# AmandineBtto/NeRAF

Measured on AMD Instinct MI355X. Metric: field-samples/sec (rays + RIR STFT bins), higher is better.
Workload: dtype f16; 1 GPU; RAF FurnishedRoom joint training step (BASELINE configs[2]): 4096 rays + 2048 RIR slices x 513 bins per GPU; radiance + grid refresh + ResNet3D + NAcF + STFT loss, backward, GradScaler + fused Adam...; rays_per_gpu=4096, slices_per_gpu=2048, global_rays=4096, global_slices=2048, parallelism=dp1, distinct_resident_batches=16, deterministic=True

## Files before the change

neraf_amd/csrc/field_bwd.hip:

```cpp
#include "field_common.h"

namespace {

constexpr int NFRAG = 24;
constexpr int NFRAG_B = 28;

struct RenderLossArgs {
  const float* density; const float* rgb_s; const float* e_bins; const float* s_bins; const float* gt;
  int R, S; float dist_mult;
  const float* up;
  float* d_rgb_s; float* d_density;
  float* d_density_dist;
  float* sums;
};

__global__ __launch_bounds__(256) void render_loss_kernel(RenderLossArgs a) {
  const int lane = threadIdx.x & 63;
  int ray = blockIdx.x * 4 + (threadIdx.x >> 6);
  const bool active = ray < a.R;
  if (!active) ray = a.R - 1;
  const int S = a.S;
  const bool on = lane < S;
  const float* eb = a.e_bins + (size_t)ray * (S + 1);
  const float* sb = a.s_bins + (size_t)ray * (S + 1);
// ... 214 lines not shown
  __syncthreads();
  const int lane = threadIdx.x & 63, wv = threadIdx.x >> 6;
  const long N = (long)a.R * a.S;
  const long nchunks = (N + 255) / 256;
  float tmass[8] = {0.f, 0.f, 0.f, 0.f, 0.f, 0.f, 0.f, 0.f};
  if (a.d32 && blockIdx.x == 0 && threadIdx.x < 2) a.one2[threadIdx.x] = 1.f;
  for (long chunk = blockIdx.x; chunk < nchunks; chunk += gridDim.x) {
    const long idx = chunk * 256 + threadIdx.x;
    const bool valid = idx < N;
    float enc[16], hpre[16], dh[16];
#pragma unroll
    for (int k = 0; k < 16; ++k) { enc[k] = 0.f; dh[k] = 0.f; hpre[k] = 0.f; }
    float x = 0.f, y = 0.f, z = 0.f, gs = 0.f;
    float xr = 0.f, yr = 0.f, zr = 0.f, tmid = 0.f; int ray_id = -1; bool sel_pt = false;
    float rgx = 0.f, rgy = 0.f, rgz = 0.f;
    if (valid) {
      const int ray = (int)(idx / a.S), s = (int)(idx % a.S);
      const float t = 0.5f * (a.e_bins[(size_t)ray * (a.S + 1) + s] + a.e_bins[(size_t)ray * (a.S + 1) + s + 1]);
      x = fmaf(a.dirs[ray * 3 + 0], t, a.origins[ray * 3 + 0]);
      y = fmaf(a.dirs[ray * 3 + 1], t, a.origins[ray * 3 + 1]);
      z = fmaf(a.dirs[ray * 3 + 2], t, a.origins[ray * 3 + 2]);
      xr = x; yr = y; zr = z; tmid = t; ray_id = ray;
      const bool sel = map_position(x, y, z, 0, nullptr);
      sel_pt = sel;
#pragma unroll
      for (int l = 0; l < 8; ++l)
        if (l < a.g.n_levels) {
          float f0, f1;
          encode_level(a.table, x, y, z, a.g.scale[l], a.g.res[l], a.g.size[l], a.g.offset[l], a.g.hashed[l], f0, f1);
          enc[2 * l] = (float)(half_t)f0; enc[2 * l + 1] = (float)(half_t)f1;
        }
      float out = 0.f;
#pragma unroll
      for (int j = 0; j < 16; ++j) {
        float h = 0.f;
#pragma unroll
        for (int k = 0; k < 16; ++k) h = fmaf(w0[j][k], enc[k], h);
        hpre[j] = h;
        out = fmaf(w1[j], fmaxf(h, 0.f), out);
      }
      gs = sel ? a.d_density[idx] * a.avg_density * __expf(fminf(fmaxf(out, -15.f), 15.f)) : 0.f;
#pragma unroll
      for (int j = 0; j < 16; ++j) dh[j] = hpre[j] > 0.f ? gs * w1[j] : 0.f;
    }
#pragma unroll
    for (int l = 0; l < 8; ++l)
      if (l < a.g.n_levels) {
        float g0 = 0.f, g1 = 0.f;
#pragma unroll
        for (int j = 0; j < 16; ++j) { g0 = fmaf(dh[j], w0[j][2 * l], g0); g1 = fmaf(dh[j], w0[j][2 * l + 1], g1); }
        if (a.d_ray && valid && sel_pt)
          encode_level_dpos(a.table, x, y, z, a.g.scale[l], a.g.res[l], a.g.size[l], a.g.offset[l], a.g.hashed[l], g0, g1, rgx, rgy, rgz);
        if (a.d32) {
          if (valid) { a.d32[(long)l * a.npad + idx] = make_float2(g0, g1); tmass[l] += fmaxf(fabsf(g0), fabsf(g1)); }
        } else {
          scatter_level_seg<64>(a.table_grad, x, y, z, a.g.scale[l], a.g.res[l], a.g.size[l], a.g.offset[l], a.g.hashed[l], g0, g1, lane);
        }
      }
    if (a.d_ray) {
      map_position_jt(xr, yr, zr, rgx, rgy, rgz);
      float g6[6] = {rgx, rgy, rgz, tmid * rgx, tmid * rgy, tmid * rgz};
      const int ray0 = __shfl(ray_id, 0);
      if (a.g6_out) {
        if (valid) {
#pragma unroll
          for (int k = 0; k < 6; ++k) a.g6_out[(size_t)idx * 6 + k] = g6[k];
        }
      } else if (__all(ray_id == ray0 || !valid)) {
#pragma unroll
        for (int k = 0; k < 6; ++k) {
          float v = valid ? g6[k] : 0.f;
#pragma unroll
          for (int o = 32; o > 0; o >>= 1) v += __shfl_xor(v, o);
          if (lane == 0 && v != 0.f && ray0 >= 0) atomicAdd(a.d_ray + (size_t)ray0 * 6 + k, v);
        }
      } else if (valid) {
#pragma unroll
        for (int k = 0; k < 6; ++k) if (g6[k] != 0.f) atomicAdd(a.d_ray + (size_t)ray_id * 6 + k, g6[k]);
      }
    }
#pragma unroll
    for (int k = 0; k < 16; ++k) { s_dh[wv][lane][k] = dh[k]; s_enc[wv][lane][k] = enc[k]; s_hr[wv][lane][k] = gs * fmaxf(hpre[k], 0.f); }
    __builtin_amdgcn_wave_barrier();
    __syncthreads();
    {
      const int j = lane >> 2, k0 = (lane & 3) * 4;
      float s[4] = {0.f, 0.f, 0.f, 0.f};
      for (int p = 0; p < 64; ++p) {
        const float d = s_dh[wv][p][j];
#pragma unroll
        for (int q = 0; q < 4; ++q) s[q] = fmaf(d, s_enc[wv][p][k0 + q], s[q]);
      }
#pragma unroll
      for (int q = 0; q < 4; ++q) acc[wv][j * 16 + k0 + q] += s[q];
      if (lane < 16) {
        float t = 0.f;
        for (int p = 0; p < 64; ++p) t += s_hr[wv][p][lane];
        acc[wv][256 + lane] += t;
      }
    }
    __syncthreads();
  }
  for (int i = threadIdx.x; i < 272; i += 256) {
    const float v = (acc[0][i] + acc[1][i]) + (acc[2][i] + acc[3][i]);
    if (a.w_part) a.w_part[(size_t)blockIdx.x * 272 + i] = v;
    else atomicAdd(a.w_grad + i, v);
  }
  if (a.d32) {
    __syncthreads();
    float* red = &s_dh[0][0][0];
#pragma unroll
    for (int l = 0; l < 8; ++l) {
      float v = tmass[l];
#pragma unroll
      for (int o = 32; o > 0; o >>= 1) v += __shfl_xor(v, o);
      if (lane == 0) red[wv * 8 + l] = v;
    }
    __syncthreads();
    if (threadIdx.x < 16)
      a.t_part[(size_t)blockIdx.x * 16 + threadIdx.x] = threadIdx.x < 8 ? (red[threadIdx.x] + red[8 + threadIdx.x]) + (red[16 + threadIdx.x] + red[24 + threadIdx.x]) : 0.f;
  }
}

__global__ __launch_bounds__(256) void prop_wgrad_fold_kernel(const float* __restrict__ part, int nblocks, float* __restrict__ w_grad,
                                                             float* __restrict__ w0_out, float* __restrict__ w1_out) {
  __shared__ float red[32][9];
  const int o = threadIdx.x & 7, sl = threadIdx.x >> 3;
  const int i = blockIdx.x * 8 + o;
  float t = 0.f, t1 = 0.f;
  if (i < 272) {
    int b = sl;
    for (; b + 32 < nblocks; b += 64) { t += part[(size_t)b * 272 + i]; t1 += part[(size_t)(b + 32) * 272 + i]; }
    for (; b < nblocks; b += 32) t += part[(size_t)b * 272 + i];
  }
  red[sl][o] = t + t1;
  __syncthreads();
  if (threadIdx.x < 8 && i < 272) {
    float s = 0.f;
#pragma unroll
    for (int r = 0; r < 32; ++r) s += red[r][threadIdx.x];
    const int k = blockIdx.x * 8 + threadIdx.x;
    if (w0_out) { if (k < 256) w0_out[k] = s; else w1_out[k - 256] = s; }
    else w_grad[k] += s;
  }
  if (w1_out && blockIdx.x == 0 && threadIdx.x >= 16) w1_out[threadIdx.x] = 0.f;
}

struct FieldBwdArgs {
  GridLayout g;
  const unsigned* table; const half8* wfrag; const half8* wfrag_b; const half_t* emb;
  const float* origins; const float* dirs; const float* e_bins; const int* cam_idx;
  int R, S; int mode; float aabb[6]; float avg_density; int avg_row;
  const float* d_rgb; const float* d_density;
  const float* scale;
  float* emb_grad;
  half_t* dump; long npad;
  unsigned* d_enc;
  float* t_part;
  int emb_det;
  float* e_part; int* e_part_row;
  float* pos;
  float* d_ray;
  float* g6_out;
  const half_t* enc_in;
  const half_t* denc_in;
};

__device__ __forceinline__ void dump_block(half_t* base, long npad, long n, int row0, const f32x4& v, float m) {
#pragma unroll
  for (int r = 0; r < 4; ++r) base[(long)(row0 + r) * npad + n] = (half_t)(v[r] * m);
}

template <bool RAYGRAD, bool SAVED>
__global__ __launch_bounds__(256) void field_backward_kernel(FieldBwdArgs a) {
  __shared__ float l_scale[MAX_LEVELS];
  __shared__ int l_res[MAX_LEVELS];
  __shared__ unsigned l_size[MAX_LEVELS], l_off[MAX_LEVELS];
  __shared__ int l_hash[MAX_LEVELS];
  if (threadIdx.x < MAX_LEVELS) {
    const int l = threadIdx.x;
    l_scale[l] = a.g.scale[l]; l_res[l] = a.g.res[l]; l_size[l] = a.g.size[l]; l_off[l] = a.g.offset[l]; l_hash[l] = a.g.hashed[l];
  }
  __syncthreads();
  __shared__ float t_sum[4][16];
  __shared__ float e_acc[32];
  __shared__ int e_blk_s;
  if (threadIdx.x < 32) e_acc[threadIdx.x] = 0.f;
  if (threadIdx.x == 0) {
    long n0 = (long)blockIdx.x * 64; const long Nn = (long)a.R * a.S;
    if (n0 >= Nn) n0 = Nn - 1;
    e_blk_s = (a.avg_row < 0 && a.cam_idx) ? a.cam_idx[n0 / a.S] : -1;
  }
  __syncthreads();
  const int e_blk = e_blk_s;
  const int lane = threadIdx.x & 63;
  const int p = lane & 15, q = lane >> 4;
  __shared__ half8 wf_s[NFRAG * 64];
  for (int i = threadIdx.x; i < NFRAG * 64; i += 256) wf_s[i] = a.wfrag[i];
  const half8* wfp = wf_s + lane;
#define wf(f) wfp[(f) * 64]
  __shared__ half8 wb_s[NFRAG_B * 64];
  for (int i = threadIdx.x; i < NFRAG_B * 64; i += 256) wb_s[i] = a.wfrag_b[i];
  __syncthreads();
  const half8* wb = wb_s + lane;
  const float gscale = a.scale[0], inv_gscale = a.scale[1];
  float tl[4] = {0.f, 0.f, 0.f, 0.f};
  const f32x4 zero = {0.f, 0.f, 0.f, 0.f};
  const long N = (long)a.R * a.S;
  const long ngroups = a.npad / 16;
  const long gstride = (long)gridDim.x * 4;
  const long MAT = 128 * a.npad;
  for (long grp = (long)blockIdx.x * 4 + (threadIdx.x >> 6); grp < ngroups; grp += gstride) {
    const long ncol = grp * 16 + p;
    long n = ncol;
    const bool valid = n < N;
    if (!valid) n = N - 1;
    const float vm = valid ? 1.f : 0.f;
    const int ray = (int)(n / a.S), s = (int)(n % a.S);
    const float t = 0.5f * (a.e_bins[(size_t)ray * (a.S + 1) + s] + a.e_bins[(size_t)ray * (a.S + 1) + s + 1]);
    const float dx = a.dirs[ray * 3 + 0], dy = a.dirs[ray * 3 + 1], dz = a.dirs[ray * 3 + 2];
    float x = fmaf(dx, t, a.origins[ray * 3 + 0]);
    float y = fmaf(dy, t, a.origins[ray * 3 + 1]);
    float z = fmaf(dz, t, a.origins[ray * 3 + 2]);
    const float xr = x, yr = y, zr = z;
    const bool sel = map_position(x, y, z, a.mode, a.aabb);
    if (a.pos && q == 0) { a.pos[ncol] = x; a.pos[a.npad + ncol] = y; a.pos[2 * a.npad + ncol] = z; }
    half8 xin;
    float dfe[RAYGRAD ? 4 : 1][2][3];
    if (SAVED) {
      xin = *reinterpret_cast<const half8*>(a.enc_in + ((size_t)n * 4 + q) * 8);
      if (RAYGRAD) {
        half8 dh[3];
        const half8* src = reinterpret_cast<const half8*>(a.denc_in + ((size_t)n * 4 + q) * 24);
        dh[0] = src[0]; dh[1] = src[1]; dh[2] = src[2];
        const half_t* dp = reinterpret_cast<const half_t*>(dh);
#pragma unroll
        for (int li = 0; li < 4; ++li)
#pragma unroll
          for (int k = 0; k < 3; ++k) { dfe[RAYGRAD ? li : 0][0][k] = (float)dp[li * 6 + k]; dfe[RAYGRAD ? li : 0][1][k] = (float)dp[li * 6 + 3 + k]; }
      }
    } else {
#pragma unroll
      for (int li = 0; li < 4; ++li) {
        const int l = 4 * q + li;
        float f0, f1;
        if (RAYGRAD) encode_level_grad(a.table, x, y, z, l_scale[l], l_res[l], l_size[l], l_off[l], l_hash[l], f0, f1, dfe[RAYGRAD ? li : 0][0], dfe[RAYGRAD ? li : 0][1]);
        else encode_level(a.table, x, y, z, l_scale[l], l_res[l], l_size[l], l_off[l], l_hash[l], f0, f1);
        xin[2 * li] = (half_t)f0; xin[2 * li + 1] = (half_t)f1;
      }
    }
    f32x4 d1[4];
#pragma unroll
    for (int ob = 0; ob < 4; ++ob) d1[ob] = __builtin_amdgcn_mfma_f32_16x16x32_f16(wf(ob), xin, zero, 0, 0, 0);
    f32x4 d2 = __builtin_amdgcn_mfma_f32_16x16x32_f16(wf(4), pack_relu(d1[0], d1[1], true), zero, 0, 0, 0);
    d2 = __builtin_amdgcn_mfma_f32_16x16x32_f16(wf(5), pack_relu(d1[2], d1[3], true), d2, 0, 0, 0);
    float sh[4];
    sh4_quarter(q, dx, dy, dz, sh);
    half8 h0;
#pragma unroll
    for (int r = 0; r < 4; ++r) { h0[r] = (half_t)d2[r]; h0[4 + r] = (half_t)sh[r]; }
    const float logit = d2[0];
    if (q == 0) h0[0] = (half_t)0.f;
    const int erow = a.avg_row >= 0 ? a.avg_row : a.cam_idx[ray];
    const half8 h1 = *reinterpret_cast<const half8*>(a.emb + (size_t)erow * 32 + 8 * q);
    f32x4 d3[4], d4[4];
#pragma unroll
    for (int ob = 0; ob < 4; ++ob) {
      d3[ob] = __builtin_amdgcn_mfma_f32_16x16x32_f16(wf(6 + ob * 2), h0, zero, 0, 0, 0);
      d3[ob] = __builtin_amdgcn_mfma_f32_16x16x32_f16(wf(7 + ob * 2), h1, d3[ob], 0, 0, 0);
    }
    const half8 a0 = pack_relu(d3[0], d3[1], true), a1 = pack_relu(d3[2], d3[3], true);
#pragma unroll
    for (int ob = 0; ob < 4; ++ob) {
      d4[ob] = __builtin_amdgcn_mfma_f32_16x16x32_f16(wf(14 + ob * 2), a0, zero, 0, 0, 0);
      d4[ob] = __builtin_amdgcn_mfma_f32_16x16x32_f16(wf(15 + ob * 2), a1, d4[ob], 0, 0, 0);
    }
    f32x4 d5 = __builtin_amdgcn_mfma_f32_16x16x32_f16(wf(22), pack_relu(d4[0], d4[1], true), zero, 0, 0, 0);
    d5 = __builtin_amdgcn_mfma_f32_16x16x32_f16(wf(23), pack_relu(d4[2], d4[3], true), d5, 0, 0, 0);
    f32x4 dy5 = zero;
    if (q == 0 && valid) {
#pragma unroll
      for (int c = 0; c < 3; ++c) {
        const float o = __builtin_amdgcn_rcpf(1.f + __expf(-d5[c]));
        dy5[c] = a.d_rgb[(size_t)n * 3 + c] * o * (1.f - o) * gscale;
      }
    }
    half_t* D = a.dump;
#pragma unroll
    for (int ob = 0; ob < 4; ++ob) {
      f32x4 r4; for (int r = 0; r < 4; ++r) r4[r] = fmaxf(d4[ob][r], 0.f);
      dump_block(D + 8 * MAT, a.npad, ncol, 16 * ob + 4 * q, r4, vm);
    }
    dump_block(D + 9 * MAT, a.npad, ncol, 4 * q, dy5, 1.f);
    f32x4 dy4[4];
    {
      const half8 b5 = pack_relu(dy5, zero, false);
#pragma unroll
      for (int ib = 0; ib < 4; ++ib) {
        dy4[ib] = __builtin_amdgcn_mfma_f32_16x16x32_f16(wb[(0 + ib) * 64], b5, zero, 0, 0, 0);
#pragma unroll
        for (int r = 0; r < 4; ++r) dy4[ib][r] = d4[ib][r] > 0.f ? dy4[ib][r] : 0.f;
      }
    }
#pragma unroll
    for (int ob = 0; ob < 4; ++ob) {
      f32x4 r3; for (int r = 0; r < 4; ++r) r3[r] = fmaxf(d3[ob][r], 0.f);
      dump_block(D + 6 * MAT, a.npad, ncol, 16 * ob + 4 * q, r3, vm);
      dump_block(D + 7 * MAT, a.npad, ncol, 16 * ob + 4 * q, dy4[ob], 1.f);
    }
    f32x4 dy3[4];
    {
      const half8 b0 = pack_relu(dy4[0], dy4[1], false), b1 = pack_relu(dy4[2], dy4[3], false);
#pragma unroll
      for (int ib = 0; ib < 4; ++ib) {
        dy3[ib] = __builtin_amdgcn_mfma_f32_16x16x32_f16(wb[(4 + ib * 2) * 64], b0, zero, 0, 0, 0);
        dy3[ib] = __builtin_amdgcn_mfma_f32_16x16x32_f16(wb[(5 + ib * 2) * 64], b1, dy3[ib], 0, 0, 0);
#pragma unroll
        for (int r = 0; r < 4; ++r) dy3[ib][r] = d3[ib][r] > 0.f ? dy3[ib][r] : 0.f;
      }
    }
    {
#pragma unroll
      for (int r = 0; r < 4; ++r) {
        D[4 * MAT + (long)(4 * q + r) * a.npad + ncol] = (half_t)(sh[r] * vm);
        const int tt = 4 * q + r;
        if (tt >= 1) D[4 * MAT + (long)(15 + tt) * a.npad + ncol] = (half_t)(d2[r] * vm);
      }
#pragma unroll
      for (int j = 0; j < 8; ++j) D[4 * MAT + (long)(31 + 8 * q + j) * a.npad + ncol] = (half_t)((float)h1[j] * vm);
      if (q == 0) D[4 * MAT + (long)63 * a.npad + ncol] = (half_t)0.f;
#pragma unroll
      for (int ob = 0; ob < 4; ++ob) dump_block(D + 5 * MAT, a.npad, ncol, 16 * ob + 4 * q, dy3[ob], 1.f);
    }
    f32x4 dbase, demb[2], dsh = zero;
    {
      const half8 b0 = pack_relu(dy3[0], dy3[1], false), b1 = pack_relu(dy3[2], dy3[3], false);
      dbase = __builtin_amdgcn_mfma_f32_16x16x32_f16(wb[12 * 64], b0, zero, 0, 0, 0);
      dbase = __builtin_amdgcn_mfma_f32_16x16x32_f16(wb[13 * 64], b1, dbase, 0, 0, 0);
      if (RAYGRAD) {
        dsh = __builtin_amdgcn_mfma_f32_16x16x32_f16(wb[26 * 64], b0, zero, 0, 0, 0);
        dsh = __builtin_amdgcn_mfma_f32_16x16x32_f16(wb[27 * 64], b1, dsh, 0, 0, 0);
      }
#pragma unroll
      for (int ib = 0; ib < 2; ++ib) {
        demb[ib] = __builtin_amdgcn_mfma_f32_16x16x32_f16(wb[(14 + ib * 2) * 64], b0, zero, 0, 0, 0);
        demb[ib] = __builtin_amdgcn_mfma_f32_16x16x32_f16(wb[(15 + ib * 2) * 64], b1, demb[ib], 0, 0, 0);
      }
    }
    if (a.emb_grad && a.avg_row < 0) {
      const int e0 = __shfl(erow, lane & 48);
      const bool uniform = __all(e0 == erow || !valid);
      const bool to_lds = uniform && __all(e0 == e_blk);
      const bool det_store = a.emb_det && uniform;
      if (a.emb_det && lane == 0) a.e_part_row[grp] = (uniform && __shfl(valid ? 1 : 0, 0)) ? e0 : -1;
#pragma unroll
      for (int ib = 0; ib < 2; ++ib)
#pragma unroll
        for (int r = 0; r < 4; ++r) {
          float v = valid ? demb[ib][r] * inv_gscale : 0.f;
          if (uniform) {
#pragma unroll
            for (int o = 1; o < 16; o <<= 1) v += __shfl_xor(v, o);
            if (det_store) {
              if (p == 0) a.e_part[grp * 32 + 16 * ib + 4 * q + r] = v;
            } else if (p == 0 && v != 0.f) {
              if (to_lds) atomicAdd(&e_acc[16 * ib + 4 * q + r], v);
              else atomicAdd(a.emb_grad + (size_t)e0 * 32 + 16 * ib + 4 * q + r, v);
            }
          } else if (valid && v != 0.f) {
            atomicAdd(a.emb_grad + (size_t)erow * 32 + 16 * ib + 4 * q + r, v);
          }
        }
    }
    f32x4 dy2 = dbase;
    if (q == 0) dy2[0] = (valid && sel) ? a.d_density[n] * a.avg_density * __expf(fminf(fmaxf(logit, -15.f), 15.f)) * gscale : 0.f;
#pragma unroll
    for (int ob = 0; ob < 4; ++ob) {
      f32x4 r1; for (int r = 0; r < 4; ++r) r1[r] = fmaxf(d1[ob][r], 0.f);
      dump_block(D + 2 * MAT, a.npad, ncol, 16 * ob + 4 * q, r1, vm);
    }
    dump_block(D + 3 * MAT, a.npad, ncol, 4 * q, dy2, vm);
    f32x4 dy1[4];
    {
      const half8 b2 = pack_relu(dy2, zero, false);
#pragma unroll
      for (int ib = 0; ib < 4; ++ib) {
        dy1[ib] = __builtin_amdgcn_mfma_f32_16x16x32_f16(wb[(18 + ib) * 64], b2, zero, 0, 0, 0);
#pragma unroll
        for (int r = 0; r < 4; ++r) dy1[ib][r] = (d1[ib][r] > 0.f && valid) ? dy1[ib][r] : 0.f;
      }
    }
#pragma unroll
    for (int j = 0; j < 8; ++j) D[0 * MAT + (long)(8 * q + j) * a.npad + ncol] = (half_t)((float)xin[j] * vm);
#pragma unroll
    for (int ob = 0; ob < 4; ++ob) dump_block(D + 1 * MAT, a.npad, ncol, 16 * ob + 4 * q, dy1[ob], 1.f);
    f32x4 de[2];
    {
      const half8 b0 = pack_relu(dy1[0], dy1[1], false), b1 = pack_relu(dy1[2], dy1[3], false);
#pragma unroll
      for (int rb = 0; rb < 2; ++rb) {
        de[rb] = __builtin_amdgcn_mfma_f32_16x16x32_f16(wb[(22 + rb * 2) * 64], b0, zero, 0, 0, 0);
        de[rb] = __builtin_amdgcn_mfma_f32_16x16x32_f16(wb[(23 + rb * 2) * 64], b1, de[rb], 0, 0, 0);
      }
    }
#pragma unroll
    for (int li = 0; li < 4; ++li) {
      const int l = 4 * q + li;
      half2v gh;
      gh[0] = (half_t)(valid ? de[li >> 1][2 * (li & 1)] : 0.f);
      gh[1] = (half_t)(valid ? de[li >> 1][2 * (li & 1) + 1] : 0.f);
      a.d_enc[(long)l * a.npad + ncol] = *reinterpret_cast<const unsigned*>(&gh);
      tl[li] += fmaxf(fabsf((float)gh[0]), fabsf((float)gh[1]));
    }
    if (RAYGRAD) {
      float px = 0.f, py = 0.f, pz = 0.f;
      if (valid && sel && a.mode == 0) {
#pragma unroll
        for (int li = 0; li < 4; ++li) {
          const float g0 = de[li >> 1][2 * (li & 1)], g1 = de[li >> 1][2 * (li & 1) + 1];
          px = fmaf(g0, dfe[RAYGRAD ? li : 0][0][0], fmaf(g1, dfe[RAYGRAD ? li : 0][1][0], px));
          py = fmaf(g0, dfe[RAYGRAD ? li : 0][0][1], fmaf(g1, dfe[RAYGRAD ? li : 0][1][1], py));
          pz = fmaf(g0, dfe[RAYGRAD ? li : 0][0][2], fmaf(g1, dfe[RAYGRAD ? li : 0][1][2], pz));
        }
      }
      px += __shfl_xor(px, 16); py += __shfl_xor(py, 16); pz += __shfl_xor(pz, 16);
      px += __shfl_xor(px, 32); py += __shfl_xor(py, 32); pz += __shfl_xor(pz, 32);
      map_position_jt(xr, yr, zr, px, py, pz);
      float sx = 0.f, sy = 0.f, sz = 0.f;
      if (valid) {
        const float g4[4] = {dsh[0], dsh[1], dsh[2], dsh[3]};
        sh4_quarter_dpos(q, dx, dy, dz, g4, sx, sy, sz);
      }
      sx += __shfl_xor(sx, 16); sy += __shfl_xor(sy, 16); sz += __shfl_xor(sz, 16);
      sx += __shfl_xor(sx, 32); sy += __shfl_xor(sy, 32); sz += __shfl_xor(sz, 32);
      float g6[6] = {px * inv_gscale, py * inv_gscale, pz * inv_gscale,
                     fmaf(t, px, sx) * inv_gscale, fmaf(t, py, sy) * inv_gscale, fmaf(t, pz, sz) * inv_gscale};
      const int ray0 = __shfl(ray, lane & 48);
      const bool one_ray = __all(ray == ray0 || !valid);
      if (a.g6_out) {
        if (valid && q == 0) {
#pragma unroll
          for (int k = 0; k < 6; ++k) a.g6_out[(size_t)n * 6 + k] = g6[k];
        }
      } else if (one_ray) {
#pragma unroll
        for (int k = 0; k < 6; ++k) {
          float v = valid ? g6[k] : 0.f;
#pragma unroll
          for (int o = 1; o < 16; o <<= 1) v += __shfl_xor(v, o);
          g6[k] = v;
        }
        if (p == 0 && q == 0) {
#pragma unroll
          for (int k = 0; k < 6; ++k) if (g6[k] != 0.f) atomicAdd(a.d_ray + (size_t)ray0 * 6 + k, g6[k]);
        }
      } else if (valid && q == 0) {
#pragma unroll
        for (int k = 0; k < 6; ++k) if (g6[k] != 0.f) atomicAdd(a.d_ray + (size_t)ray * 6 + k, g6[k]);
      }
    }
  }
#pragma unroll
  for (int li = 0; li < 4; ++li) {
    float v = tl[li];
#pragma unroll
    for (int o = 1; o < 16; o <<= 1) v += __shfl_xor(v, o);
    if (p == 0) t_sum[threadIdx.x >> 6][4 * q + li] = v;
  }
  __syncthreads();
  if (threadIdx.x < 16)
    a.t_part[(long)blockIdx.x * 16 + threadIdx.x] = t_sum[0][threadIdx.x] + t_sum[1][threadIdx.x] + t_sum[2][threadIdx.x] + t_sum[3][threadIdx.x];
  if (!a.emb_det) {
    if (threadIdx.x < 32) a.e_part[(long)blockIdx.x * 32 + threadIdx.x] = e_acc[threadIdx.x];
    if (threadIdx.x == 0) a.e_part_row[blockIdx.x] = e_blk;
  }
#undef wf
}

__global__ __launch_bounds__(256) void field_finalize_kernel(const float* __restrict__ t_part, int nblocks, float* __restrict__ lvl,
                                                            const float* __restrict__ e_part, const int* __restrict__ e_part_row,
                                                            float* __restrict__ emb_grad) {
  __shared__ float red[4];
  if (blockIdx.x < 16) {
    const int l = blockIdx.x;
    float v = 0.f;
    for (int b = threadIdx.x; b < nblocks; b += 256) v += t_part[(long)b * 16 + l];
#pragma unroll
    for (int o = 32; o > 0; o >>= 1) v += __shfl_xor(v, o);
    if ((threadIdx.x & 63) == 0) red[threadIdx.x >> 6] = v;
    __syncthreads();
    if (threadIdx.x == 0) {
      const float T = red[0] + red[1] + red[2] + red[3];
      float F = 1.f;
      if (T > 0.f && T < 3.0e38f) {
        int e = 29 - (int)ceilf(log2f(T));
        e = e > 100 ? 100 : (e < -100 ? -100 : e);
        F = exp2f((float)e);
      }
      lvl[l] = F; lvl[16 + l] = 1.f / F;
    }
    return;
  }
  if (!emb_grad) return;
  const int c = threadIdx.x & 31, sl = threadIdx.x >> 5;
  const int b0 = (blockIdx.x - 16) * 64 + sl * 8;
  int rows[8]; float vals[8];
#pragma unroll
  for (int i = 0; i < 8; ++i) {
    const int b = b0 + i;
    rows[i] = b < nblocks ? e_part_row[b] : -1;
    vals[i] = b < nblocks ? e_part[(long)b * 32 + c] : 0.f;
  }
  int cur = -1; float acc = 0.f;
#pragma unroll
  for (int i = 0; i < 8; ++i) {
    if (rows[i] != cur) {
      if (cur >= 0 && acc != 0.f) atomicAdd(emb_grad + (size_t)cur * 32 + c, acc);
      cur = rows[i]; acc = 0.f;
    }
    acc += vals[i];
  }
  if (cur >= 0 && acc != 0.f) atomicAdd(emb_grad + (size_t)cur * 32 + c, acc);
}

__global__ __launch_bounds__(256) void field_emb_fold_det_kernel(const float* __restrict__ e_part, const int* __restrict__ e_part_row,
                                                                long ngroups, float* __restrict__ emb_grad, int beta) {
  __shared__ float part[8][32];
  const int row = blockIdx.x, c = threadIdx.x & 31, q = threadIdx.x >> 5;
  float acc = 0.f;
  for (long g = q; g < ngroups; g += 8)
    if (e_part_row[g] == row) acc += e_part[g * 32 + c];
  part[q][c] = acc;
  __syncthreads();
  if (threadIdx.x < 32) {
    const float v = ((part[0][c] + part[1][c]) + (part[2][c] + part[3][c])) + ((part[4][c] + part[5][c]) + (part[6][c] + part[7][c]));
    float* dst = emb_grad + (size_t)row * 32 + c;
    *dst = beta ? *dst + v : v;
  }
}

struct FieldScatterArgs {
  GridLayout g;
  const float* origins; const float* dirs; const float* e_bins;
  int R, S; int mode; float aabb[6];
  const unsigned* d_enc; long npad;
  const float* lvl;
  unsigned long long* acc;
  int l_end;
  const float2* d_red; int run;
  long npad_r;
  const float2* d32;
};

__global__ __launch_bounds__(256) void field_runsum_kernel(const unsigned* __restrict__ d_enc, long npad, long nruns, int run,
                                                          float2* __restrict__ d_red, long npad_r) {
  const int l = blockIdx.y;
  for (long k = (long)blockIdx.x * 256 + threadIdx.x; k < nruns; k += (long)gridDim.x * 256) {
    float s0 = 0.f, s1 = 0.f;
    for (int j = 0; j < run; ++j) {
      const unsigned raw = d_enc[(long)l * npad + k * run + j];
      const half2v gh = *reinterpret_cast<const half2v*>(&raw);
      s0 += (float)gh[0]; s1 += (float)gh[1];
    }
    d_red[(long)l * npad_r + k] = make_float2(s0, s1);
  }
}

__device__ __forceinline__ long long shfl_up_i64(long long v, int o) {
  const int lo = __shfl_up((int)(v & 0xffffffffll), o), hi = __shfl_up((int)(v >> 32), o);
  return ((long long)hi << 32) | (unsigned)lo;
}

__global__ __launch_bounds__(256) void field_scatter_kernel(FieldScatterArgs a) {
  __shared__ float l_scale[MAX_LEVELS], l_fix[MAX_LEVELS];
  __shared__ int l_res[MAX_LEVELS];
  __shared__ unsigned l_size[MAX_LEVELS], l_off[MAX_LEVELS];
  __shared__ int l_hash[MAX_LEVELS];
  if (threadIdx.x < 16) {
    const int l = threadIdx.x;
    l_scale[l] = a.g.scale[l]; l_res[l] = a.g.res[l]; l_size[l] = a.g.size[l]; l_off[l] = a.g.offset[l]; l_hash[l] = a.g.hashed[l];
    l_fix[l] = a.lvl[l];
  }
  __syncthreads();
  const int lane = threadIdx.x & 63;
  const long N = a.run > 1 ? (long)a.R / a.run : (long)a.R * a.S;
  const long nwave = (N + 63) / 64;
  for (long wv = (long)blockIdx.x * 4 + (threadIdx.x >> 6); wv < nwave; wv += (long)gridDim.x * 4) {
    long n = wv * 64 + lane;
    const bool valid = n < N;
    if (!valid) n = N - 1;
    const int ray = a.run > 1 ? (int)(n * a.run) : (int)(n / a.S), sidx = a.run > 1 ? 0 : (int)(n % a.S);
    const float t = 0.5f * (a.e_bins[(size_t)ray * (a.S + 1) + sidx] + a.e_bins[(size_t)ray * (a.S + 1) + sidx + 1]);
    float x = fmaf(a.dirs[ray * 3 + 0], t, a.origins[ray * 3 + 0]);
    float y = fmaf(a.dirs[ray * 3 + 1], t, a.origins[ray * 3 + 1]);
    float z = fmaf(a.dirs[ray * 3 + 2], t, a.origins[ray * 3 + 2]);
    map_position(x, y, z, a.mode, a.aabb);
    const int l_first = gridDim.y > 1 ? (int)blockIdx.y : 0, l_last = gridDim.y > 1 ? l_first + 1 : a.l_end;
    for (int l = l_first; l < l_last; ++l) {
      const float F = l_fix[l];
      float g0, g1;
      if (a.run > 1) {
        const float2 gr = valid ? a.d_red[(long)l * a.npad_r + n] : make_float2(0.f, 0.f);
        g0 = gr.x * F; g1 = gr.y * F;
      } else if (a.d32) {
        const float2 gr = valid ? a.d32[(long)l * a.npad + n] : make_float2(0.f, 0.f);
        g0 = gr.x * F; g1 = gr.y * F;
      } else {
        const unsigned raw = valid ? a.d_enc[(long)l * a.npad + n] : 0u;
        const half2v gh = *reinterpret_cast<const half2v*>(&raw);
        g0 = (float)gh[0] * F; g1 = (float)gh[1] * F;
      }
      const float scale = l_scale[l];
      const int res = l_res[l]; const unsigned size = l_size[l], offset = l_off[l]; const int hashed = l_hash[l];
      const float px = fmaf(scale, x, 0.5f), py = fmaf(scale, y, 0.5f), pz = fmaf(scale, z, 0.5f);
      const float flx = floorf(px), fly = floorf(py), flz = floorf(pz);
      const float wx = px - flx, wy = py - fly, wz = pz - flz;
      const unsigned ix = (unsigned)(int)flx, iy = (unsigned)(int)fly, iz = (unsigned)(int)flz;
#pragma unroll
      for (int c = 0; c < 8; ++c) {
        const unsigned cx = ix + (c & 1), cy = iy + ((c >> 1) & 1), cz = iz + ((c >> 2) & 1);
        const float w = ((c & 1) ? wx : 1.f - wx) * ((c & 2) ? wy : 1.f - wy) * ((c & 4) ? wz : 1.f - wz);
        unsigned idx;
        if (hashed) idx = (cx ^ (cy * 2654435761u) ^ (cz * 805459861u)) & (size - 1u);
        else {
          idx = cx + cy * (unsigned)res + cz * (unsigned)res * (unsigned)res;
          if (idx >= size) idx -= size;
        }
        const int q0 = __float2int_rn(w * g0), q1 = __float2int_rn(w * g1);
        long long v = ((long long)q1 << 32) + (long long)q0;
        const unsigned prev = __shfl_up(idx, 1);
        const unsigned next = __shfl_down(idx, 1);
        int head = (lane == 0 || prev != idx) ? 1 : 0;
        const bool tail = (lane == 63) || next != idx;
        if (__any(!head)) {
#pragma unroll
// ... 78 lines not shown
  for (unsigned i = tid; i < NENT; i += OWN_THREADS) own[i] = 0ull;
  __syncthreads();
  const float scale = a.g.scale[l], F = a.lvl[l];
  const int res = a.g.res[l]; const unsigned size = a.g.size[l]; const int hashed = a.g.hashed[l];
  const unsigned mask = size - 1u;
  const unsigned nsl_mask = (size >> OWN_SLICE_LOG2) - 1u;
  const uint4* ids = reinterpret_cast<const uint4*>(a.ids + (long)l * a.npad);
  const unsigned* genc = a.d_enc + (long)l * a.npad;
  const float* xs = a.pos; const float* ys = a.pos + a.npad; const float* zs = a.pos + 2 * a.npad;

  auto expand = [&](unsigned head, int cnt) {
    if (lane < cnt) {
      const long n = (long)queue[(head + lane) & (OWN_QUEUE - 1)];
      const unsigned raw = genc[n];
      const float x = xs[n], y = ys[n], z = zs[n];
      const half2v gh = *reinterpret_cast<const half2v*>(&raw);
      const float g0 = (float)gh[0] * F, g1 = (float)gh[1] * F;
      const float px = fmaf(scale, x, 0.5f), py = fmaf(scale, y, 0.5f), pz = fmaf(scale, z, 0.5f);
      const float flx = floorf(px), fly = floorf(py), flz = floorf(pz);
      const float wx = px - flx, wy = py - fly, wz = pz - flz;
      const unsigned ix = (unsigned)(int)flx, iy = (unsigned)(int)fly, iz = (unsigned)(int)flz;
      auto add = [&](unsigned idx, float w) {
        const int q0 = __float2int_rn(w * g0), q1 = __float2int_rn(w * g1);
        const long long v = ((long long)q1 << 32) + (long long)q0;
        if (v != 0) atomicAdd(&own[idx & (NENT - 1u)], (unsigned long long)v);
      };
      if (hashed) {
        unsigned m4 = 0u;
#pragma unroll
        for (int k = 0; k < 4; ++k) {
          const unsigned t = ((iy + (k & 1)) * HASH_P1) ^ ((iz + (k >> 1)) * HASH_P2);
          if (((t >> OWN_SLICE_LOG2) & nsl_mask) == slice) m4 |= 1u << k;
        }
        while (m4) {
          const int k = __builtin_ctz(m4);
          m4 &= m4 - 1u;
          const int kb = k & 1, kc = k >> 1;
          const unsigned t = ((iy + kb) * HASH_P1) ^ ((iz + kc) * HASH_P2);
          const float wyv = kb ? wy : 1.f - wy, wzv = kc ? wz : 1.f - wz;
#pragma unroll
          for (int ka = 0; ka < 2; ++ka)
            add(((ix + ka) ^ t) & mask, ((ka ? wx : 1.f - wx) * wyv) * wzv);
        }
      } else {
#pragma unroll
        for (int c = 0; c < 8; ++c) {
          const unsigned idx = corner_index(ix + (c & 1), iy + ((c >> 1) & 1), iz + ((c >> 2) & 1), res, size, 0);
          if ((idx >> OWN_SLICE_LOG2) != slice) continue;
          add(idx, ((c & 1) ? wx : 1.f - wx) * ((c & 2) ? wy : 1.f - wy) * ((c & 4) ? wz : 1.f - wz));
        }
      }
    }
  };

  unsigned head = 0; int qcount = 0;
  const long step = (long)(OWN_THREADS / 64) * 256;
  long base = n_begin + (long)wave * 256;
  const uint4 none = make_uint4(0u, 0u, 0u, 0u);
  uint4 cur = (base < n_end && base + lane * 4 < a.npad) ? ids[(base >> 2) + lane] : none;
  for (; base < n_end; base += step) {
    const long nb = base + step;
    const uint4 nxt = (nb < n_end && nb + lane * 4 < a.npad) ? ids[(nb >> 2) + lane] : none;
    const unsigned wv[4] = {cur.x, cur.y, cur.z, cur.w};
#pragma unroll
    for (int j = 0; j < 4; ++j) {
      const bool has = (wv[j] >> slice) & 1u;
      const unsigned long long b = __ballot(has);
      if (b == 0ull) continue;
      if (has) {
        const int at = qcount + __builtin_amdgcn_mbcnt_hi((unsigned)(b >> 32), __builtin_amdgcn_mbcnt_lo((unsigned)b, 0));
        queue[(head + at) & (OWN_QUEUE - 1)] = (unsigned)(base + lane * 4 + j);
      }
      qcount += __popcll(b);
      __builtin_amdgcn_wave_barrier();
      if (qcount >= 64) { expand(head, 64); head += 64; qcount -= 64; __builtin_amdgcn_wave_barrier(); }
    }
    cur = nxt;
  }
  if (qcount > 0) expand(head, qcount);
  __syncthreads();
  const size_t e0 = (size_t)slice * NENT;
  unsigned long long* dst = a.acc + a.g.offset[l] + e0;
  if (nrep == 1 && a.dst) {
    const float m = a.lvl[16 + l] * a.scale[1];
    float2* out = a.dst + a.g.offset[l] + e0;
    for (unsigned i = tid; i < NENT; i += OWN_THREADS) {
      if (e0 + i >= size) continue;
      const long long v = (long long)own[i];
      if (v == 0) {
        if (!a.beta) out[i] = make_float2(0.f, 0.f);
        continue;
      }
      const int lo = (int)(v & 0xffffffffll);
      const int hi = (int)((v - (long long)lo) >> 32);
      float2 o = make_float2((float)lo * m, (float)hi * m);
      if (a.beta) { const float2 old = out[i]; o.x += old.x; o.y += old.y; }
      out[i] = o;
    }
  } else if (nrep == 1) {
    for (unsigned i = tid; i < NENT; i += OWN_THREADS)
      if (e0 + i < size) dst[i] = own[i];
  } else {
    for (unsigned i = tid; i < NENT; i += OWN_THREADS) {
      const unsigned long long v = own[i];
      if (v != 0ull && e0 + i < size) atomicAdd(dst + i, v);
    }
  }
}

__global__ __launch_bounds__(256) void field_unpack_grad_kernel(GridLayout g, const float* __restrict__ lvl, const float* __restrict__ scale,
                                                               unsigned long long* __restrict__ acc, float2* __restrict__ dst, int beta,
                                                               unsigned skip_levels = 0u) {
  const int l = blockIdx.y;
  if ((skip_levels >> l) & 1u) return;
  const float m = lvl[16 + l] * scale[1];
  const unsigned size = g.size[l], off = g.offset[l];
  const bool inplace = reinterpret_cast<void*>(dst) == reinterpret_cast<void*>(acc);
  for (unsigned i = blockIdx.x * 256 + threadIdx.x; i < size; i += gridDim.x * 256) {
    const long long v = (long long)acc[off + i];
    if (v == 0) {
      if (!inplace && !beta) dst[off + i] = make_float2(0.f, 0.f);
      continue;
    }
    const int lo = (int)(v & 0xffffffffll);
    const int hi = (int)((v - (long long)lo) >> 32);
    float2 o = make_float2((float)lo * m, (float)hi * m);
    if (!inplace) {
      acc[off + i] = 0ull;
      if (beta) { const float2 old = dst[off + i]; o.x += old.x; o.y += old.y; }
    }
    dst[off + i] = o;
  }
}

__global__ __launch_bounds__(256) void field_amax_kernel(const float* __restrict__ d_rgb, const float* __restrict__ d_density,
                                                        const float* __restrict__ density, long N, float avg_density,
                                                        unsigned* __restrict__ amax_bits, float* __restrict__ zero_p, long zero_n) {
  for (long i = (long)blockIdx.x * 256 + threadIdx.x; i < zero_n; i += (long)gridDim.x * 256) zero_p[i] = 0.f;
  const float dlo = avg_density * 3.0590232e-7f, dhi = avg_density * 3269017.4f;
  float m = 0.f;
  for (long i = (long)blockIdx.x * 256 + threadIdx.x; i < N; i += (long)gridDim.x * 256) {
    float v = fmaxf(fabsf(d_rgb[i * 3]), fmaxf(fabsf(d_rgb[i * 3 + 1]), fabsf(d_rgb[i * 3 + 2]))) * 0.25f;
    v = fmaxf(v, fabsf(d_density[i]) * fminf(fmaxf(density[i], dlo), dhi));
    m = (v == v && v > m) ? v : m;
  }
#pragma unroll
  for (int o = 32; o > 0; o >>= 1) m = fmaxf(m, __shfl_xor(m, o));
  __shared__ float sh[4];
  if ((threadIdx.x & 63) == 0) sh[threadIdx.x >> 6] = m;
  __syncthreads();
  if (threadIdx.x == 0) atomicMax(amax_bits, __float_as_uint(fmaxf(fmaxf(sh[0], sh[1]), fmaxf(sh[2], sh[3]))));
}

__global__ void field_make_scale_kernel(float* __restrict__ scale) {
  if (threadIdx.x == 0 && blockIdx.x == 0) {
    const float amax = __uint_as_float(reinterpret_cast<unsigned*>(scale)[2]);
    reinterpret_cast<unsigned*>(scale)[2] = 0u;
    float S = 1.f;
    if (amax > 0.f && amax < 3.0e38f) {
      int e = 6 - (int)floorf(log2f(amax));
      e = e > 100 ? 100 : (e < -100 ? -100 : e);
      S = exp2f((float)e);
    }
    scale[0] = S; scale[1] = 1.f / S;
  }
}

}

extern "C" int neraf_render_loss(neraf_ctx* ctx, const float* density, const float* rgb_s, const float* e_bins,
                                 const float* s_bins, const float* gt_rgb, int R, int S, float distortion_mult, const float* up3,
                                 float* d_rgb_s, float* d_density, float* d_density_dist, float* sums, neraf_stream_t stream) {
  if (R <= 0 || S <= 0 || S > 64 || !density || !rgb_s || !e_bins || !s_bins || !gt_rgb || !sums || (up3 && (!d_rgb_s || !d_density)) ||
      (!up3 && d_rgb_s && (!d_density || !d_density_dist)))
    return neraf_fail(ctx, NERAF_EINVAL, "render_loss: bad arguments (S <= 64)");
  RenderLossArgs a{density, rgb_s, e_bins, s_bins, gt_rgb, R, S, distortion_mult, up3, d_rgb_s, d_density, d_density_dist, sums};
  hipLaunchKernelGGL(render_loss_kernel, dim3((R + 3) / 4), dim3(256), 0, (hipStream_t)stream, a);
  NERAF_HIP_CHECK(ctx, hipGetLastError());
  return NERAF_OK;
}

extern "C" int neraf_interlevel_loss(neraf_ctx* ctx, const float* c_bins, const float* w_fine, int S2, const float* p_bins,
                                     const float* p_ebins, const float* p_density, int Sp, int R, float mult, const float* up3,
                                     float* d_density, float* sums, neraf_stream_t stream) {
  if (R <= 0 || S2 <= 0 || S2 > IL_MAX_S2 || Sp <= 0 || Sp > IL_MAX_SP || !c_bins || !w_fine || !p_bins || !p_ebins || !p_density ||
      !sums || (up3 && !d_density))
    return neraf_fail(ctx, NERAF_EINVAL, "interlevel_loss: bad arguments (S2 <= 64, Sp <= 256)");
  InterlevelArgs a{c_bins, w_fine, S2, p_bins, p_ebins, p_density, Sp, R, mult, up3, d_density, sums};
  hipLaunchKernelGGL(interlevel_kernel, dim3((R + 3) / 4), dim3(256), 0, (hipStream_t)stream, a);
  NERAF_HIP_CHECK(ctx, hipGetLastError());
  return NERAF_OK;
}

static int proposal_backward_impl(neraf_ctx* ctx, const neraf_grid_desc* g, const void* table_f16, const void* mlp_f16,
                                  const float* origins, const float* dirs, const float* e_bins, const float* d_density,
                                  int R, int S, float avg_density, float* table_grad, float* w_grad, void* scratch,
                                  size_t scratch_bytes, float* d_rays, float* w0_out, float* w1_out, void* acc_scratch,
                                  neraf_stream_t stream);

extern "C" size_t neraf_proposal_backward_scratch_bytes(int R, int S, int n_levels) {
  const size_t npad = ((size_t)R * S + 63) / 64 * 64;
  return (size_t)2048 * 272 * sizeof(float) + (size_t)2048 * 16 * sizeof(float) + 64 * sizeof(float) + (size_t)n_levels * npad * sizeof(float2) +
         (neraf_deterministic() ? npad * 6 * sizeof(float) : 0);
}

extern "C" int neraf_proposal_backward(neraf_ctx* ctx, const neraf_grid_desc* g, const void* table_f16, const void* mlp_f16,
                                       const float* origins, const float* dirs, const float* e_bins, const float* d_density,
                                       int R, int S, float avg_density, float* table_grad, float* w_grad, void* scratch,
                                       size_t scratch_bytes, neraf_stream_t stream) {
  return proposal_backward_impl(ctx, g, table_f16, mlp_f16, origins, dirs, e_bins, d_density, R, S, avg_density, table_grad, w_grad,
                                scratch, scratch_bytes, nullptr, nullptr, nullptr, nullptr, stream);
}

extern "C" int neraf_proposal_backward_ex(neraf_ctx* ctx, const neraf_grid_desc* g, const void* table_f16, const void* mlp_f16,
                                          const float* origins, const float* dirs, const float* e_bins, const float* d_density,
                                          int R, int S, float avg_density, float* table_grad, float* w0_grad, float* w1_grad,
                                          void* scratch, size_t scratch_bytes, void* acc_scratch, float* d_rays,
                                          neraf_stream_t stream) {
  if (!w0_grad || !w1_grad || !acc_scratch || !scratch || scratch_bytes < neraf_proposal_backward_scratch_bytes(R, S, g ? g->n_levels : 0))
    return neraf_fail(ctx, NERAF_EINVAL, "proposal_backward_ex: w0_grad, w1_grad, acc_scratch and the full scratch are required");
  return proposal_backward_impl(ctx, g, table_f16, mlp_f16, origins, dirs, e_bins, d_density, R, S, avg_density, table_grad, w0_grad,
                                scratch, scratch_bytes, d_rays, w0_grad, w1_grad, acc_scratch, stream);
}

extern "C" int neraf_proposal_backward_rays(neraf_ctx* ctx, const neraf_grid_desc* g, const void* table_f16, const void* mlp_f16,
                                            const float* origins, const float* dirs, const float* e_bins, const float* d_density,
                                            int R, int S, float avg_density, float* table_grad, float* w_grad, void* scratch,
                                            size_t scratch_bytes, float* d_rays, neraf_stream_t stream) {
  if (!d_rays) return neraf_fail(ctx, NERAF_EINVAL, "proposal_backward_rays: d_rays required");
  return proposal_backward_impl(ctx, g, table_f16, mlp_f16, origins, dirs, e_bins, d_density, R, S, avg_density, table_grad, w_grad,
                                scratch, scratch_bytes, d_rays, nullptr, nullptr, nullptr, stream);
}

static int proposal_backward_impl(neraf_ctx* ctx, const neraf_grid_desc* g, const void* table_f16, const void* mlp_f16,
                                  const float* origins, const float* dirs, const float* e_bins, const float* d_density,
                                  int R, int S, float avg_density, float* table_grad, float* w_grad, void* scratch,
                                  size_t scratch_bytes, float* d_rays, float* w0_out, float* w1_out, void* acc_scratch,
                                  neraf_stream_t stream) {
  PropBwdArgs a{};
  if (make_grid_layout(g, &a.g) || a.g.n_levels > 8) return neraf_fail(ctx, NERAF_EINVAL, "proposal_backward: bad grid (<= 8 levels)");
  if (R <= 0 || S <= 0 || !table_f16 || !mlp_f16 || !origins || !dirs || !e_bins || !d_density || !table_grad || !w_grad)
    return neraf_fail(ctx, NERAF_EINVAL, "proposal_backward: bad arguments");
  a.table = (const unsigned*)table_f16; a.w = (const half_t*)mlp_f16; a.origins = origins; a.dirs = dirs; a.e_bins = e_bins;
  a.d_density = d_density; a.R = R; a.S = S; a.avg_density = avg_density; a.table_grad = table_grad; a.w_grad = w_grad; a.d_ray = d_rays;
  const long n = (long)R * S;
  long blocks = (n + 255) / 256;
  if (blocks > 2048) blocks = 2048;
  a.w_part = (scratch && scratch_bytes >= (size_t)blocks * 272 * sizeof(float)) ? (float*)scratch : nullptr;
  constexpr int packed_on = 1;
  const long npad = (n + 63) / 64 * 64;
  float* lvl = nullptr;
  if (packed_on && a.w_part && scratch_bytes >= neraf_proposal_backward_scratch_bytes(R, S, a.g.n_levels)) {
    char* sp = (char*)scratch + (size_t)2048 * 272 * sizeof(float);
    a.t_part = (float*)sp; sp += (size_t)2048 * 16 * sizeof(float);
    lvl = (float*)sp; sp += 32 * sizeof(float);
    a.one2 = (float*)sp; sp += 32 * sizeof(float);
    a.d32 = (float2*)sp; a.npad = npad;
    sp += (size_t)a.g.n_levels * npad * sizeof(float2);
    if (neraf_deterministic() && d_rays) a.g6_out = (float*)sp;
  }
  hipStream_t st = (hipStream_t)stream;
  {
    ProfScope prof(ctx, st, PROF_PROP_BWD, (double)n * a.g.n_levels * 8 * 8);
    hipLaunchKernelGGL(proposal_backward_kernel, dim3((unsigned)blocks), dim3(256), 0, st, a);
    if (a.g6_out) hipLaunchKernelGGL(ray_fold_kernel, dim3((R + 3) / 4), dim3(256), 0, st, a.g6_out, R, S, d_rays);
    if (a.d32) {
      hipLaunchKernelGGL(field_finalize_kernel, dim3(16), dim3(256), 0, st, a.t_part, (int)blocks, lvl, nullptr, nullptr, nullptr);
      FieldScatterArgs sa{};
      sa.g = a.g; sa.origins = origins; sa.dirs = dirs; sa.e_bins = e_bins; sa.R = R; sa.S = S; sa.mode = 0;
      sa.npad = npad; sa.lvl = lvl; sa.acc = reinterpret_cast<unsigned long long*>(acc_scratch ? acc_scratch : (void*)table_grad);
      sa.l_end = a.g.n_levels; sa.run = 1;
      sa.d32 = a.d32;
      long sblocks = ((n + 63) / 64 + 3) / 4;
      const long cap = (long)(ctx ? ctx->num_cus : 256) * 8;
      if (sblocks > cap) sblocks = cap;
      hipLaunchKernelGGL(field_scatter_kernel, dim3((unsigned)sblocks, 1), dim3(256), 0, st, sa);
      unsigned maxsize = 0;
      for (int l = 0; l < a.g.n_levels; ++l) maxsize = a.g.size[l] > maxsize ? a.g.size[l] : maxsize;
      hipLaunchKernelGGL(field_unpack_grad_kernel, dim3((maxsize + 1023) / 1024, a.g.n_levels), dim3(256), 0, st, a.g, lvl, a.one2,
                         sa.acc, reinterpret_cast<float2*>(table_grad), 0);
    } else if (acc_scratch) return neraf_fail(ctx, NERAF_EINVAL, "proposal_backward_ex: packed table gradient unavailable");
  }
  if (a.w_part) hipLaunchKernelGGL(prop_wgrad_fold_kernel, dim3(34), dim3(256), 0, st, a.w_part, (int)blocks, w_grad, w0_out, w1_out);
  NERAF_HIP_CHECK(ctx, hipGetLastError());
  return NERAF_OK;
}

extern "C" size_t neraf_field_backward_dump_bytes(int R, int S) {
  const long npad = ((long)R * S + 63) / 64 * 64;
  return (size_t)10 * 128 * npad * 2 + 256 + (neraf_deterministic() ? (size_t)npad * 6 * sizeof(float) : 0);
}

static int field_backward_impl(neraf_ctx* ctx, const neraf_grid_desc* g, const void* table_f16, const void* wfrag_f16,
                               const void* wfrag_bwd_f16, const void* emb_f16, const float* origins, const float* dirs,
                               const float* e_bins, const int32_t* cam_idx, int R, int S, int mode, const float* aabb_host,
                               float avg_density, int avg_row, const float* density, const float* d_rgb,
                               const float* d_density, float* table_grad, float* emb_grad, float* const* w_grads, void* dump,
                               void* splitk_ws, size_t splitk_bytes, int pos_run, float* d_rays, const void* enc_in, const void* denc_in,
                               void* acc_scratch, int accumulate, int emb_rows, neraf_stream_t stream);

extern "C" int neraf_field_backward(neraf_ctx* ctx, const neraf_grid_desc* g, const void* table_f16, const void* wfrag_f16,
                                    const void* wfrag_bwd_f16, const void* emb_f16, const float* origins, const float* dirs,
                                    const float* e_bins, const int32_t* cam_idx, int R, int S, int mode, const float* aabb_host,
                                    float avg_density, int avg_row, const float* density, const float* d_rgb, const float* d_density,
                                    float* table_grad, float* emb_grad, float* const* w_grads, void* dump, void* splitk_ws,
                                    size_t splitk_bytes, neraf_stream_t stream) {
  return field_backward_impl(ctx, g, table_f16, wfrag_f16, wfrag_bwd_f16, emb_f16, origins, dirs, e_bins, cam_idx, R, S, mode,
                             aabb_host, avg_density, avg_row, density, d_rgb, d_density, table_grad, emb_grad, w_grads, dump,
                             splitk_ws, splitk_bytes, 1, nullptr, nullptr, nullptr, nullptr, 0, 0, stream);
}

extern "C" int neraf_field_backward_runs(neraf_ctx* ctx, const neraf_grid_desc* g, const void* table_f16, const void* wfrag_f16,
                                         const void* wfrag_bwd_f16, const void* emb_f16, const float* origins, const float* dirs,
                                         const float* e_bins, const int32_t* cam_idx, int R, int S, int mode, const float* aabb_host,
                                         float avg_density, int avg_row, const float* density, const float* d_rgb,
                                         const float* d_density, float* table_grad, float* emb_grad, float* const* w_grads, void* dump,
                                         void* splitk_ws, size_t splitk_bytes, int pos_run, neraf_stream_t stream) {
  return field_backward_impl(ctx, g, table_f16, wfrag_f16, wfrag_bwd_f16, emb_f16, origins, dirs, e_bins, cam_idx, R, S, mode,
                             aabb_host, avg_density, avg_row, density, d_rgb, d_density, table_grad, emb_grad, w_grads, dump,
                             splitk_ws, splitk_bytes, pos_run, nullptr, nullptr, nullptr, nullptr, 0, 0, stream);
}

extern "C" int neraf_field_backward_rays(neraf_ctx* ctx, const neraf_grid_desc* g, const void* table_f16, const void* wfrag_f16,
                                         const void* wfrag_bwd_f16, const void* emb_f16, const float* origins, const float* dirs,
                                         const float* e_bins, const int32_t* cam_idx, int R, int S, int mode, const float* aabb_host,
                                         float avg_density, int avg_row, const float* density, const float* d_rgb,
                                         const float* d_density, float* table_grad, float* emb_grad, float* const* w_grads, void* dump,
                                         void* splitk_ws, size_t splitk_bytes, float* d_rays, neraf_stream_t stream) {
  if (!d_rays) return neraf_fail(ctx, NERAF_EINVAL, "field_backward_rays: d_rays required");
  return field_backward_impl(ctx, g, table_f16, wfrag_f16, wfrag_bwd_f16, emb_f16, origins, dirs, e_bins, cam_idx, R, S, mode,
                             aabb_host, avg_density, avg_row, density, d_rgb, d_density, table_grad, emb_grad, w_grads, dump,
                             splitk_ws, splitk_bytes, 1, d_rays, nullptr, nullptr, nullptr, 0, 0, stream);
}

extern "C" int neraf_field_backward_ex(neraf_ctx* ctx, const neraf_grid_desc* g, const void* table_f16, const void* wfrag_f16,
                                      const void* wfrag_bwd_f16, const void* emb_f16, const float* origins, const float* dirs,
                                      const float* e_bins, const int32_t* cam_idx, int R, int S, int mode, const float* aabb_host,
                                      float avg_density, int avg_row, const float* density, const float* d_rgb,
                                      const float* d_density, float* table_grad, float* emb_grad, float* const* w_grads, void* dump,
                                      void* splitk_ws, size_t splitk_bytes, int pos_run, float* d_rays, const void* enc_saved,
                                      const void* denc_saved, void* acc_scratch, int accumulate, int emb_rows, neraf_stream_t stream) {
  if (d_rays && pos_run != 1) return neraf_fail(ctx, NERAF_EINVAL, "field_backward_ex: ray gradients need pos_run == 1");
  return field_backward_impl(ctx, g, table_f16, wfrag_f16, wfrag_bwd_f16, emb_f16, origins, dirs, e_bins, cam_idx, R, S, mode,
                             aabb_host, avg_density, avg_row, density, d_rgb, d_density, table_grad, emb_grad, w_grads, dump,
                             splitk_ws, splitk_bytes, pos_run, d_rays, enc_saved, denc_saved, acc_scratch, accumulate, emb_rows, stream);
}

static int field_backward_impl(neraf_ctx* ctx, const neraf_grid_desc* g, const void* table_f16, const void* wfrag_f16,
                               const void* wfrag_bwd_f16, const void* emb_f16, const float* origins, const float* dirs,
                               const float* e_bins, const int32_t* cam_idx, int R, int S, int mode, const float* aabb_host,
                               float avg_density, int avg_row, const float* density, const float* d_rgb,
                               const float* d_density, float* table_grad, float* emb_grad, float* const* w_grads, void* dump,
                               void* splitk_ws, size_t splitk_bytes, int pos_run, float* d_rays, const void* enc_in, const void* denc_in,
                               void* acc_scratch, int accumulate, int emb_rows, neraf_stream_t stream) {
  if (accumulate && !acc_scratch)
    return neraf_fail(ctx, NERAF_EINVAL, "field_backward: accumulate needs acc_scratch (the gradient buffer cannot double as the accumulator)");
  if (pos_run < 1 || (pos_run > 1 && (S != 1 || R % pos_run != 0)))
    return neraf_fail(ctx, NERAF_EINVAL, "field_backward_runs: pos_run > 1 needs S == 1 and R a multiple of pos_run");
  FieldBwdArgs a{};
  if (make_grid_layout(g, &a.g) || a.g.n_levels != 16) return neraf_fail(ctx, NERAF_EINVAL, "field_backward: grid must have 16 levels");
  if (R <= 0 || S <= 0 || !table_f16 || !wfrag_f16 || !wfrag_bwd_f16 || !emb_f16 || !origins || !dirs || !e_bins || !density ||
      !d_rgb || !d_density || !table_grad || !w_grads || !dump || (avg_row < 0 && !cam_idx) || (mode != 0 && !aabb_host))
    return neraf_fail(ctx, NERAF_EINVAL, "field_backward: bad arguments");
  hipStream_t st = (hipStream_t)stream;
  const long N = (long)R * S;
  const long npad = (N + 63) / 64 * 64;
  a.table = (const unsigned*)table_f16; a.wfrag = (const half8*)wfrag_f16; a.wfrag_b = (const half8*)wfrag_bwd_f16;
  a.emb = (const half_t*)emb_f16; a.origins = origins; a.dirs = dirs; a.e_bins = e_bins; a.cam_idx = cam_idx;
  a.R = R; a.S = S; a.mode = mode;
  for (int i = 0; i < 6; ++i) a.aabb[i] = aabb_host ? aabb_host[i] : 0.f;
  a.avg_density = avg_density; a.avg_row = avg_row; a.d_rgb = d_rgb; a.d_density = d_density;
  a.emb_grad = emb_grad;
  a.dump = (half_t*)dump; a.npad = npad;
  a.d_enc = reinterpret_cast<unsigned*>((half_t*)dump + (size_t)64 * npad);
  a.t_part = reinterpret_cast<float*>((half_t*)dump + (size_t)128 * npad + (size_t)64 * npad);
  a.e_part = reinterpret_cast<float*>((half_t*)dump + (size_t)2 * 128 * npad + (size_t)64 * npad);
  a.e_part_row = reinterpret_cast<int*>((half_t*)dump + (size_t)3 * 128 * npad + (size_t)64 * npad);
  float* scale = (float*)((char*)dump + (size_t)10 * 128 * npad * 2);
  a.scale = scale;
  if (neraf_deterministic() && d_rays) a.g6_out = (float*)((char*)dump + (size_t)10 * 128 * npad * 2 + 256);
  constexpr int kOwnLds = (1 << OWN_SLICE_LOG2) * 8 + (OWN_THREADS / 64) * OWN_QUEUE * 4;
  const char* own_e = getenv("NERAF_FIELD_OWNER_SCATTER");
  const int own_env = own_e ? atoi(own_e) : 1;
  bool use_owner = own_env && pos_run == 1 && (N >= 131072 || own_env == 2) && N < (1l << 30);
  int own_blk[MAX_LEVELS + 1] = {0};
  unsigned char own_rep[MAX_LEVELS] = {0};
  for (int l = 0; l < 16 && use_owner; ++l) {
    const unsigned sz = a.g.size[l];
    const unsigned nsl = (sz + (1u << OWN_SLICE_LOG2) - 1u) >> OWN_SLICE_LOG2;
    use_owner = nsl <= 32 && a.g.res[l] + 1 < (1 << OWN_SLICE_LOG2) &&
                (!a.g.hashed[l] || ((sz & (sz - 1)) == 0 && sz >= (2u << OWN_SLICE_LOG2)));
    int rep = a.g.hashed[l] ? 1 : (int)((10 + nsl / 2) / nsl);
    rep = rep < 1 ? 1 : (rep > 12 ? 12 : rep);
    own_rep[l] = (unsigned char)rep;
    own_blk[l + 1] = own_blk[l] + (int)nsl * rep;
  }
  if (use_owner) {
    static bool attr_set = false;
    if (!attr_set) {
      NERAF_HIP_CHECK(ctx, hipFuncSetAttribute(reinterpret_cast<const void*>(&field_scatter_owner_kernel),
                                               hipFuncAttributeMaxDynamicSharedMemorySize, kOwnLds));
      attr_set = true;
    }
    a.pos = reinterpret_cast<float*>((half_t*)dump + (size_t)4 * 128 * npad + (size_t)64 * npad);
  }
  {
    long blocks = (N + 1023) / 1024; if (blocks > 256) blocks = 256;
    a.emb_det = (neraf_deterministic() && acc_scratch && emb_grad && avg_row < 0 && emb_rows > 0) ? 1 : 0;
    const bool zero_emb = acc_scratch && !accumulate && emb_grad && avg_row < 0 && emb_rows > 0;
    hipLaunchKernelGGL(field_amax_kernel, dim3((unsigned)blocks), dim3(256), 0, st, d_rgb, d_density, density, N, avg_density,
                       reinterpret_cast<unsigned*>(scale) + 2, zero_emb ? emb_grad : nullptr, zero_emb ? (long)emb_rows * 32 : 0l);
    hipLaunchKernelGGL(field_make_scale_kernel, dim3(1), dim3(64), 0, st, scale);
  }
  {
    const long groups = npad / 16;
    long blocks = (groups + 3) / 4;
    const long cap = (long)(ctx ? ctx->num_cus : 256) * 8;
    if (blocks > cap) blocks = cap;
    {
      ProfScope prof(ctx, st, PROF_FIELD_BWD, (double)N * 16 * 8 * 4);
      a.d_ray = d_rays; a.enc_in = (const half_t*)enc_in; a.denc_in = (const half_t*)denc_in;
      if (d_rays && enc_in && denc_in) hipLaunchKernelGGL((field_backward_kernel<true, true>), dim3((unsigned)blocks), dim3(256), 0, st, a);
      else if (d_rays) hipLaunchKernelGGL((field_backward_kernel<true, false>), dim3((unsigned)blocks), dim3(256), 0, st, a);
      else if (enc_in) hipLaunchKernelGGL((field_backward_kernel<false, true>), dim3((unsigned)blocks), dim3(256), 0, st, a);
      else hipLaunchKernelGGL((field_backward_kernel<false, false>), dim3((unsigned)blocks), dim3(256), 0, st, a);
      if (a.g6_out) hipLaunchKernelGGL(ray_fold_kernel, dim3((R + 3) / 4), dim3(256), 0, st, a.g6_out, R, S, d_rays);
    }
    NERAF_HIP_CHECK(ctx, hipGetLastError());
    float* lvl = scale + 8;
    const bool fold_emb = avg_row < 0 && emb_grad && !a.emb_det;
    if (a.emb_det)
      hipLaunchKernelGGL(field_emb_fold_det_kernel, dim3((unsigned)emb_rows), dim3(256), 0, st, a.e_part, a.e_part_row, npad / 16, emb_grad, 1);
    hipLaunchKernelGGL(field_finalize_kernel, dim3(16 + (fold_emb ? (unsigned)((blocks + 63) / 64) : 0u)), dim3(256), 0, st, a.t_part,
                       (int)blocks, lvl, a.e_part, a.e_part_row, fold_emb ? emb_grad : nullptr);
    FieldScatterArgs sa{};
    sa.g = a.g; sa.origins = origins; sa.dirs = dirs; sa.e_bins = e_bins; sa.R = R; sa.S = S; sa.mode = mode;
    for (int i = 0; i < 6; ++i) sa.aabb[i] = a.aabb[i];
    sa.d_enc = a.d_enc; sa.npad = npad; sa.lvl = lvl;
    sa.acc = reinterpret_cast<unsigned long long*>(acc_scratch ? acc_scratch : (void*)table_grad);
    sa.l_end = 16;
    sa.run = pos_run;
    long sblocks = ((N + 63) / 64 + 3) / 4;
    if (pos_run > 1) {
      const long nruns = N / pos_run;
      sa.npad_r = (nruns + 63) / 64 * 64;
      float2* d_red = reinterpret_cast<float2*>((half_t*)dump + (size_t)5 * 128 * npad + (size_t)64 * npad);
      sa.d_red = d_red;
      long rb = (nruns + 255) / 256; if (rb > 256) rb = 256;
      hipLaunchKernelGGL(field_runsum_kernel, dim3((unsigned)rb, 16), dim3(256), 0, st, a.d_enc, npad, nruns, pos_run, d_red, sa.npad_r);
      sblocks = ((nruns + 63) / 64 + 3) / 4;
    }
    if (sblocks > cap) sblocks = cap;
    unsigned direct_levels = 0u;
    {
      ProfScope prof(ctx, st, PROF_FIELD_SCATTER, (double)N * 16 * 8 * 8);
      if (!use_owner) hipLaunchKernelGGL(field_scatter_kernel, dim3((unsigned)sblocks, pos_run > 1 ? 16 : 1), dim3(256), 0, st, sa);
      else {
        FieldOwnerArgs oa{};
        oa.g = a.g; oa.pos = a.pos; oa.npad = npad; oa.N = N; oa.d_enc = a.d_enc; oa.lvl = lvl; oa.acc = sa.acc;
        oa.ids = reinterpret_cast<unsigned*>(a.pos + 3 * npad);
        for (int l = 0; l <= 16; ++l) oa.blk_begin[l] = own_blk[l];
        for (int l = 0; l < 16; ++l) oa.rep[l] = own_rep[l];
        static const int direct_on = [] { const char* e = getenv("NERAF_OWNER_DIRECT"); return e ? atoi(e) : 1; }();
        if (acc_scratch && direct_on) {
          oa.dst = reinterpret_cast<float2*>(table_grad); oa.beta = accumulate; oa.scale = scale;
          for (int l = 0; l < 16; ++l) if (own_rep[l] == 1) direct_levels |= 1u << l;
        }
        long iblocks = (npad + 255) / 256; if (iblocks > 512) iblocks = 512;
        hipLaunchKernelGGL(field_slice_ids_kernel, dim3((unsigned)iblocks, 16), dim3(256), 0, st, oa);
        hipLaunchKernelGGL(field_scatter_owner_kernel, dim3(own_blk[16]), dim3(OWN_THREADS), kOwnLds, st, oa);
      }
    }
    unsigned maxsize = 0;
    for (int l = 0; l < 16; ++l) maxsize = a.g.size[l] > maxsize ? a.g.size[l] : maxsize;
    hipLaunchKernelGGL(field_unpack_grad_kernel, dim3((maxsize + 1023) / 1024, 16), dim3(256), 0, st, a.g, lvl, scale,
                       sa.acc, reinterpret_cast<float2*>(table_grad), accumulate, direct_levels);
    NERAF_HIP_CHECK(ctx, hipGetLastError());
  }
  const int outs[5] = {64, 16, 64, 64, 16}, ins[5] = {32, 64, 64, 64, 64};
  GemmParams gp{};
  gp.lda = (int)npad; gp.ldb = (int)npad; gp.K = (int)npad; gp.Mpad = 64; gp.Npad = 64; gp.alpha = 1.f; gp.alpha_dev = scale + 1;
  gp.splitk_ws = (float*)splitk_ws; gp.splitk_ws_bytes = splitk_bytes;
  gp.ngroups = 5;
  gp.c32_beta = accumulate;
  for (int l = 0; l < 5; ++l) {
    gp.grp[l].A = (const half_t*)dump + (size_t)(2 * l + 1) * 128 * npad;
    gp.grp[l].B = (const half_t*)dump + (size_t)(2 * l) * 128 * npad;
    gp.grp[l].M = outs[l]; gp.grp[l].N = ins[l]; gp.grp[l].C32 = w_grads[l]; gp.grp[l].ldc32 = ins[l];
  }
  gp.A = gp.grp[0].A; gp.B = gp.grp[0].B; gp.M = 64; gp.N = 64; gp.C32 = w_grads[0]; gp.ldc32 = ins[0];
  if (int e = launch_gemm_f16(ctx, gp, st)) return e;
  return NERAF_OK;
}
```

neraf_amd/csrc/nacf.hip:

```cpp
#include "common.h"
#include <algorithm>

namespace {

constexpr int TRUNK[5] = {5096, 2048, 1024, 1024, 0};
constexpr int KQ_PAD = 192;
constexpr int QT_ROWS = 256;

struct Dims {
  int n[6];
  int np[6];
  int k[6];
  int kp[6];
  int kdense, kdense_p;
};

Dims make_dims(const neraf_nacf_desc* d) {
  Dims D{};
  for (int i = 0; i < 4; ++i) D.n[i] = TRUNK[i];
  D.n[4] = d->W;
  D.n[5] = d->C * d->F;
  for (int i = 0; i < 6; ++i) D.np[i] = round_up(D.n[i], 128);
  D.k[0] = d->n_query; D.kp[0] = KQ_PAD;
  for (int i = 1; i < 6; ++i) { D.k[i] = D.n[i - 1]; D.kp[i] = D.np[i - 1]; }
  D.kdense = d->n_feat + d->n_query;
  D.kdense_p = round_up(D.kdense, 128);
  return D;
}

struct PackLayout {
  size_t w[6], wt[6];
  size_t w0d, w0dt;
  size_t bias[6];
  size_t total;
};

PackLayout make_pack_layout(const neraf_nacf_desc* d, const Dims& D) {
  PackLayout L{};
  size_t off = 0;
  auto take = [&](size_t bytes) { size_t o = off; off += round_up_sz(bytes, 256); return o; };
  for (int l = 0; l < 6; ++l) {
    L.w[l] = take((size_t)D.np[l] * D.kp[l] * 2);
    L.wt[l] = (l == 0) ? 0 : take((size_t)round_up(D.kp[l], 128) * D.np[l] * 2);
  }
  if (d->dense_l0) {
    L.w0d = take((size_t)D.np[0] * D.kdense_p * 2);
    L.w0dt = take((size_t)D.kdense_p * D.np[0] * 2);
  }
  for (int l = 0; l < 6; ++l) L.bias[l] = take((size_t)D.np[l] * 4);
  L.total = off;
  return L;
}

struct WsLayout {
  int Mpad;
  size_t q, qT;
  size_t hd, hdT;
  size_t h[5], hT[5];
  size_t bias0;
  size_t dz[2], dzT[2];
  size_t colsum[6];
  size_t scale;
  size_t dfeat_part;
  int col_slots;
  size_t total;
};

WsLayout make_ws_layout(const neraf_nacf_desc* d, const Dims& D, int B, int training) {
  WsLayout L{};
  static const int kAlign = [] { const char* e = getenv("NERAF_NACF_MALIGN"); const int v = e ? atoi(e) : 128; return (v == 256 || v == 512) ? v : 128; }();
  L.Mpad = round_up(B, kAlign);
  size_t off = 0;
  auto take = [&](size_t bytes) { size_t o = off; off += round_up_sz(bytes, 256); return o; };
  const size_t M = L.Mpad;
  L.q = take(M * KQ_PAD * 2);
  L.qT = take((size_t)QT_ROWS * M * 2);
  if (d->dense_l0) {
    L.hd = take(M * D.kdense_p * 2);
    L.hdT = take((size_t)D.kdense_p * M * 2);
  }
  for (int l = 0; l < 5; ++l) {
    L.h[l] = take(M * D.np[l] * 2);
    L.hT[l] = training ? take((size_t)D.np[l] * M * 2) : 0;
  }
  L.bias0 = take((size_t)D.np[0] * 4);
  if (training) {
    int maxw = 0;
    for (int l = 0; l < 6; ++l) maxw = D.np[l] > maxw ? D.np[l] : maxw;
    for (int i = 0; i < 2; ++i) {
      L.dz[i] = take(M * maxw * 2);
      L.dzT[i] = take((size_t)(maxw + 128) * M * 2);
    }
    L.col_slots = neraf_deterministic() ? L.Mpad / 32 : 1;
    for (int l = 0; l < 6; ++l) L.colsum[l] = take((size_t)L.col_slots * D.np[l] * 4);
    L.scale = take(256);
    if (neraf_deterministic()) L.dfeat_part = take((size_t)64 * (d->n_feat > 0 ? d->n_feat : 1) * 4);
  }
  L.total = off;
  return L;
}


__global__ __launch_bounds__(256) void cvt_pad_transpose_kernel(
    const float* __restrict__ src, const float* __restrict__ aux, const float* __restrict__ scale, int ld, int R, int Cc,
    int mode, half_t* __restrict__ dst, int ld_dst, int Rpad, int Cpad,
    half_t* __restrict__ dstT, int ld_dstT, int RpadT, int CpadT, float* __restrict__ colsum, int colsum_slot_stride) {
  __shared__ float tile[32][33];
  const int tx = threadIdx.x & 31, ty = threadIdx.x >> 5;
  const int c0 = blockIdx.x * 32, r0 = blockIdx.y * 32;
  const float sc = scale ? scale[0] : 1.f;
#pragma unroll
  for (int i = 0; i < 4; ++i) {
    const int r = r0 + ty + i * 8, c = c0 + tx;
    float v = 0.f;
    if (r < R && c < Cc) {
      v = src[(size_t)r * ld + c];
      if (mode == 1) {
        const float o = aux[(size_t)r * ld + c];
        v *= (10.f - o * o * 0.1f) * sc;
      }
    }
    tile[ty + i * 8][tx] = v;
    if (dst && r < Rpad && c < Cpad) dst[(size_t)r * ld_dst + c] = (half_t)v;
  }
  __syncthreads();
  if (dstT) {
#pragma unroll
    for (int i = 0; i < 4; ++i) {
      const int c = c0 + ty + i * 8, r = r0 + tx;
      if (c < CpadT && r < RpadT) dstT[(size_t)c * ld_dstT + r] = (half_t)tile[tx][ty + i * 8];
    }
  }
  if (colsum && ty == 0) {
    float s = 0.f;
#pragma unroll 8
    for (int i = 0; i < 32; ++i) s += (float)(half_t)tile[i][tx];
    const int c = c0 + tx;
    if (c < Cpad) {
      if (colsum_slot_stride > 0) colsum[(size_t)blockIdx.y * colsum_slot_stride + c] = s;
      else atomicAdd(colsum + c, s);
    }
  }
}

__global__ void pad_copy_f32_kernel(const float* __restrict__ src, int n, float* __restrict__ dst, int npad) {
  const int i = blockIdx.x * blockDim.x + threadIdx.x;
  if (i < npad) dst[i] = (i < n) ? src[i] : 0.f;
}

struct CvtJob {
  const float* src; half_t* dst; half_t* dstT;
  int ld, R, Cc, ld_dst, Rpad, Cpad, ld_dstT, RpadT, CpadT;
  int tiles_x, tile_begin;
};
constexpr int kMaxCvtJobs = 10;
struct CvtTable { int n; int total; CvtJob j[kMaxCvtJobs]; };

__global__ __launch_bounds__(256) void cvt_pad_transpose_grouped_kernel(CvtTable t) {
  __shared__ float tile[32][33];
  int ji = 0;
  while (ji + 1 < t.n && (int)blockIdx.x >= t.j[ji + 1].tile_begin) ++ji;
  const CvtJob& J = t.j[ji];
  const int b = blockIdx.x - J.tile_begin;
  const int tx = threadIdx.x & 31, ty = threadIdx.x >> 5;
  const int c0 = (b % J.tiles_x) * 32, r0 = (b / J.tiles_x) * 32;
#pragma unroll
  for (int i = 0; i < 4; ++i) {
    const int r = r0 + ty + i * 8, c = c0 + tx;
    float v = 0.f;
    if (r < J.R && c < J.Cc) v = J.src[(size_t)r * J.ld + c];
    tile[ty + i * 8][tx] = v;
    if (J.dst && r < J.Rpad && c < J.Cpad) J.dst[(size_t)r * J.ld_dst + c] = (half_t)v;
  }
  __syncthreads();
  if (J.dstT) {
#pragma unroll
    for (int i = 0; i < 4; ++i) {
      const int c = c0 + ty + i * 8, r = r0 + tx;
      if (c < J.CpadT && r < J.RpadT) J.dstT[(size_t)c * J.ld_dstT + r] = (half_t)tile[tx][ty + i * 8];
    }
  }
}

struct SegCopyTable { int n; int begin[17]; const float* src[16]; float* dst[16]; int len[16]; int npad[16]; int stride[16]; const float* mul;
                      int nslots; };

__global__ __launch_bounds__(256) void seg_copy_kernel(SegCopyTable t) {
  int si = 0;
  while (si + 1 < t.n && (int)blockIdx.x >= t.begin[si + 1]) ++si;
  const int i = (blockIdx.x - t.begin[si]) * 256 + threadIdx.x;
  if (i >= t.npad[si]) return;
  float v = 0.f;
  if (i < t.len[si]) {
    if (t.nslots > 1) {
      float a = 0.f, b = 0.f, c = 0.f, e = 0.f;
      int sl = 0;
      for (; sl + 4 <= t.nslots; sl += 4) {
        a += t.src[si][(size_t)sl * t.stride[si] + i]; b += t.src[si][(size_t)(sl + 1) * t.stride[si] + i];
        c += t.src[si][(size_t)(sl + 2) * t.stride[si] + i]; e += t.src[si][(size_t)(sl + 3) * t.stride[si] + i];
      }
      for (; sl < t.nslots; ++sl) a += t.src[si][(size_t)sl * t.stride[si] + i];
      v = (a + b) + (c + e);
    } else {
      v = t.src[si][i];
    }
    v *= t.mul ? t.mul[0] : 1.f;
  }
  t.dst[si][i] = v;
}

static void seg_copy_add(SegCopyTable& t, float* dst, const float* src, int n, int npad, int stride = 0) {
  const int k = t.n++;
  t.src[k] = src; t.dst[k] = dst; t.len[k] = n; t.npad[k] = npad; t.stride[k] = stride;
  t.begin[k + 1] = t.begin[k] + (npad + 255) / 256;
}

__global__ __launch_bounds__(256) void feat_gemv_kernel(const float* __restrict__ W0, int ldw, const float* __restrict__ b0,
                                                       const float* __restrict__ feat, int n_feat, int N, int Npad,
                                                       float* __restrict__ out) {
  const int lane = threadIdx.x & 63;
  const int n = blockIdx.x * 4 + (threadIdx.x >> 6);
  if (n >= Npad) return;
  float s = 0.f;
  if (n < N) {
    const float* w = W0 + (size_t)n * ldw;
    for (int k = lane; k < n_feat; k += 64) s += w[k] * feat[k];
  }
#pragma unroll
  for (int o = 32; o > 0; o >>= 1) s += __shfl_xor(s, o);
  if (lane == 0) out[n] = (n < N) ? s + b0[n] : 0.f;
}

__global__ __launch_bounds__(256) void dfeat_kernel(const float* __restrict__ W0, int ldw, const float* __restrict__ db0,
                                                   int N, int n_feat, float* __restrict__ dfeat, float* __restrict__ part) {
  const int k = blockIdx.x * 256 + threadIdx.x;
  const int per = (N + gridDim.y - 1) / gridDim.y;
  const int n0 = blockIdx.y * per, n1 = min(N, n0 + per);
  if (k >= n_feat) return;
  float s = 0.f, s1 = 0.f, s2 = 0.f, s3 = 0.f;
  int n = n0;
  for (; n + 8 <= n1; n += 8) {
    float w[8];
#pragma unroll
    for (int u = 0; u < 8; ++u) w[u] = W0[(size_t)(n + u) * ldw + k];
    s += db0[n] * w[0] + db0[n + 4] * w[4]; s1 += db0[n + 1] * w[1] + db0[n + 5] * w[5];
    s2 += db0[n + 2] * w[2] + db0[n + 6] * w[6]; s3 += db0[n + 3] * w[3] + db0[n + 7] * w[7];
  }
  for (; n < n1; ++n) s += db0[n] * W0[(size_t)n * ldw + k];
  if (part) part[(size_t)blockIdx.y * n_feat + k] = (s + s1) + (s2 + s3);
  else atomicAdd(dfeat + k, (s + s1) + (s2 + s3));
}

__global__ __launch_bounds__(256) void dfeat_fold_kernel(const float* __restrict__ part, int nsplit, int n_feat, float* __restrict__ dfeat) {
  const int k = blockIdx.x * 256 + threadIdx.x;
  if (k >= n_feat) return;
  float a = 0.f, b = 0.f, c = 0.f, e = 0.f;
  int sl = 0;
  for (; sl + 4 <= nsplit; sl += 4) {
    a += part[(size_t)sl * n_feat + k]; b += part[(size_t)(sl + 1) * n_feat + k];
    c += part[(size_t)(sl + 2) * n_feat + k]; e += part[(size_t)(sl + 3) * n_feat + k];
  }
  for (; sl < nsplit; ++sl) a += part[(size_t)sl * n_feat + k];
  dfeat[k] = (a + b) + (c + e);
}

__global__ __launch_bounds__(256) void outer_kernel(const float* __restrict__ db0, const float* __restrict__ feat, int N,
                                                   int n_feat, float* __restrict__ dW0, int ldw, float* __restrict__ zero_nfeat) {
  const int k = blockIdx.x * 256 + threadIdx.x;
  const int n = blockIdx.y;
  if (k < n_feat && n < N) dW0[(size_t)n * ldw + k] = db0[n] * feat[k];
  if (zero_nfeat && n == 0 && k < n_feat) zero_nfeat[k] = 0.f;
}

struct EncodeArgs {
  const int64_t* tq; const double* mic; const double* src; const double* rot;
  float aabb[6]; float inv_tmax; int B, Mpad;
  half_t* q; half_t* qT;
  int pstride;
};

__global__ __launch_bounds__(256) void encode_queries_kernel(EncodeArgs a, int tmajor) {
  const long idx = (long)blockIdx.x * 256 + threadIdx.x;
  int row, col;
  if (tmajor) {
    if (idx >= (long)QT_ROWS * a.Mpad) return;
    col = (int)(idx / a.Mpad); row = (int)(idx % a.Mpad);
  } else {
    if (idx >= (long)a.Mpad * KQ_PAD) return;
    row = (int)(idx / KQ_PAD); col = (int)(idx % KQ_PAD);
  }
  float v = 0.f;
  if (row < a.B && col < 163) {
    const double TWO_PI = 6.283185307179586476925286766559;
    const double HALF_PI = 1.5707963267948966192313216916398;
    if (col < 21) {
      const float t = (float)a.tq[row] * a.inv_tmax;
      if (col == 20) v = t;
      else {
        const int k = col % 10;
        const float f = exp2f((float)k * (8.0f / 9.0f));
        const float s = (6.283185307179586f * t) * f;
        v = (col < 10) ? (float)sin((double)s) : (float)sin((double)(s + 1.5707963267948966f));
      }
    } else if (col < 147) {
      const bool is_mic = col < 84;
      const double* P = (is_mic ? a.mic : a.src) + (size_t)row * a.pstride;
      const int c = is_mic ? col - 21 : col - 84;
      double xn[3];
      bool inside = true;
#pragma unroll
      for (int d = 0; d < 3; ++d) {
        xn[d] = (P[d] - (double)a.aabb[d]) / ((double)a.aabb[3 + d] - (double)a.aabb[d]);
        inside = inside && (xn[d] > 0.0) && (xn[d] < 1.0);
      }
      if (!inside) { xn[0] = xn[1] = xn[2] = 0.0; }
      if (c >= 60) v = (float)xn[c - 60];
      else {
        const int cc = c < 30 ? c : c - 30;
        const int d = cc / 10, k = cc % 10;
        const double f = (double)exp2f((float)k * (8.0f / 9.0f));
        const double s = TWO_PI * xn[d] * f;
        v = (float)sin(c < 30 ? s : s + HALF_PI);
      }
    } else {
      const double* R = a.rot + (size_t)row * a.pstride;
      const float x = (float)R[0] * 2.f - 1.f, y = (float)R[1] * 2.f - 1.f, z = (float)R[2] * 2.f - 1.f;
      const float xy = x * y, xz = x * z, yz = y * z, x2 = x * x, y2 = y * y, z2 = z * z;
      switch (col - 147) {
        case 0: v = 0.28209479177387814f; break;
        case 1: v = -0.48860251190291987f * y; break;
        case 2: v = 0.48860251190291987f * z; break;
        case 3: v = -0.48860251190291987f * x; break;
        case 4: v = 1.0925484305920792f * xy; break;
        case 5: v = -1.0925484305920792f * yz; break;
        case 6: v = 0.94617469575755997f * z2 - 0.31539156525251999f; break;
        case 7: v = -1.0925484305920792f * xz; break;
        case 8: v = 0.54627421529603959f * x2 - 0.54627421529603959f * y2; break;
        case 9: v = 0.59004358992664352f * y * (-3.0f * x2 + y2); break;
        case 10: v = 2.8906114426405538f * xy * z; break;
        case 11: v = 0.45704579946446572f * y * (1.0f - 5.0f * z2); break;
        case 12: v = 0.3731763325901154f * z * (5.0f * z2 - 3.0f); break;
        case 13: v = 0.45704579946446572f * x * (1.0f - 5.0f * z2); break;
        case 14: v = 1.4453057213202769f * z * (x2 - y2); break;
        default: v = 0.59004358992664352f * x * (-x2 + 3.0f * y2); break;
      }
    }
  }
  if (tmajor) a.qT[(size_t)col * a.Mpad + row] = (half_t)v;
  else a.q[(size_t)row * KQ_PAD + col] = (half_t)v;
}

__global__ __launch_bounds__(256) void amax_dz5_kernel(const float* __restrict__ dout, const float* __restrict__ out, size_t n,
                                                      unsigned* __restrict__ amax_bits) {
  float m = 0.f;
  for (size_t i = (size_t)blockIdx.x * 256 + threadIdx.x; i < n; i += (size_t)gridDim.x * 256) {
    const float o = out[i];
    const float v = fabsf(dout[i] * (10.f - o * o * 0.1f));
    m = (v == v && v > m) ? v : m;
  }
#pragma unroll
  for (int o = 32; o > 0; o >>= 1) m = fmaxf(m, __shfl_xor(m, o));
  __shared__ float sh[4];
  if ((threadIdx.x & 63) == 0) sh[threadIdx.x >> 6] = m;
  __syncthreads();
  if (threadIdx.x == 0) atomicMax(amax_bits, __float_as_uint(fmaxf(fmaxf(sh[0], sh[1]), fmaxf(sh[2], sh[3]))));
}

__global__ void make_scale_kernel(float* __restrict__ scale) {
  if (threadIdx.x == 0 && blockIdx.x == 0) {
    const float amax = __uint_as_float(reinterpret_cast<unsigned*>(scale)[2]);
    float S = 1.f;
    if (amax > 0.f && amax < 3.0e38f) {
      int e = 8 - (int)floorf(log2f(amax));
      e = e > 100 ? 100 : (e < -100 ? -100 : e);
      S = exp2f((float)e);
    }
    scale[0] = S;
    scale[1] = 1.f / S;
  }
}

__global__ void scale_copy_kernel(float* __restrict__ dst, const float* __restrict__ src, int n, const float* __restrict__ mul) {
  const int i = blockIdx.x * blockDim.x + threadIdx.x;
  if (i < n) dst[i] = src[i] * mul[0];
}

__global__ __launch_bounds__(256) void stft_loss_sums_kernel(const float* __restrict__ x, const float* __restrict__ y,
                                                            size_t n, int l1, float* __restrict__ part) {
  float s0 = 0.f, s1 = 0.f, s2 = 0.f;
  for (size_t i = (size_t)blockIdx.x * 256 + threadIdx.x; i < n; i += (size_t)gridDim.x * 256) {
    const float xv = x[i], yv = y[i];
    const float xm = expf(xv) - 1e-3f, ym = expf(yv) - 1e-3f;
    const float dm = ym - xm, dl = xv - yv;
    s0 += dm * dm; s1 += ym * ym; s2 += l1 ? fabsf(dl) : dl * dl;
  }
#pragma unroll
  for (int o = 32; o > 0; o >>= 1) { s0 += __shfl_xor(s0, o); s1 += __shfl_xor(s1, o); s2 += __shfl_xor(s2, o); }
  __shared__ float sh[3][4];
  const int lane = threadIdx.x & 63, w = threadIdx.x >> 6;
  if (lane == 0) { sh[0][w] = s0; sh[1][w] = s1; sh[2][w] = s2; }
  __syncthreads();
  if (threadIdx.x < 3) part[(size_t)blockIdx.x * 4 + threadIdx.x] = (sh[threadIdx.x][0] + sh[threadIdx.x][1]) + (sh[threadIdx.x][2] + sh[threadIdx.x][3]);
}

__global__ __launch_bounds__(64) void stft_sums_fold_kernel(const float* __restrict__ part, int nblocks, float* __restrict__ sums) {
  const int lane = threadIdx.x;
  float v[3] = {0.f, 0.f, 0.f};
  for (int b = lane; b < nblocks; b += 64)
#pragma unroll
    for (int k = 0; k < 3; ++k) v[k] += part[(size_t)b * 4 + k];
#pragma unroll
  for (int k = 0; k < 3; ++k) {
#pragma unroll
    for (int o = 32; o > 0; o >>= 1) v[k] += __shfl_xor(v[k], o);
  }
  if (lane < 3) sums[lane] = v[lane];
  if (lane == 3) sums[3] = 0.f;
}

__global__ void stft_loss_final_kernel(const float* __restrict__ sums, float inv_n, const float* __restrict__ weights,
                                       float* __restrict__ losses) {
  if (threadIdx.x == 0 && blockIdx.x == 0) {
    const float sc = sqrtf(sums[0]) / sqrtf(sums[1]);
    const float mag = sums[2] * inv_n;
    losses[0] = weights ? sc * weights[0] : sc;
    losses[1] = weights ? mag * weights[1] : mag;
  }
}

__global__ __launch_bounds__(256) void stft_loss_bwd_kernel(const float* __restrict__ x, const float* __restrict__ y, size_t n,
                                                           size_t n_total, int l1, const float* __restrict__ sums, const float* g_sc,
                                                           const float* g_mag, const float* __restrict__ weights, float extra,
                                                           float* __restrict__ dx) {
  const float w0 = (g_sc ? *g_sc : 0.f) * (weights ? weights[0] : 1.f) * extra;
  const float w1 = (g_mag ? *g_mag : 0.f) * (weights ? weights[1] : 1.f) * extra;
  const float inv_den = w0 / (sqrtf(sums[0]) * sqrtf(sums[1]));
  const float wm = w1 / (float)n_total;
  for (size_t i = (size_t)blockIdx.x * 256 + threadIdx.x; i < n; i += (size_t)gridDim.x * 256) {
    const float xv = x[i], yv = y[i];
    const float ex = expf(xv);
    const float xm = ex - 1e-3f, ym = expf(yv) - 1e-3f;
    const float dl = xv - yv;
    const float gm = l1 ? (dl > 0.f ? 1.f : (dl < 0.f ? -1.f : 0.f)) : 2.f * dl;
    dx[i] = (xm - ym) * ex * inv_den + gm * wm;
  }
}

int cvt_pad_transpose(neraf_ctx* ctx, hipStream_t st, const float* src, const float* aux, const float* scale, int ld, int R,
                      int Cc, int mode,
                      half_t* dst, int ld_dst, int Rpad, int Cpad, half_t* dstT, int ld_dstT, int RpadT, int CpadT,
                      float* colsum, int colsum_slot_stride = 0) {
  int rmax = Rpad, cmax = Cpad;
  if (dstT) { rmax = RpadT > rmax ? RpadT : rmax; cmax = CpadT > cmax ? CpadT : cmax; }
  if (!dst) { rmax = RpadT; cmax = CpadT; }
  dim3 grid((cmax + 31) / 32, (rmax + 31) / 32);
  hipLaunchKernelGGL(cvt_pad_transpose_kernel, grid, dim3(256), 0, st, src, aux, scale, ld, R, Cc, mode, dst, ld_dst,
                     dst ? Rpad : 0, dst ? Cpad : 0, dstT, ld_dstT, RpadT, CpadT, colsum, colsum_slot_stride);
  NERAF_HIP_CHECK(ctx, hipGetLastError());
  return NERAF_OK;
}

inline const float* Wptr(const float* const* w, int l) { return w[2 * l]; }
inline const float* Bptr(const float* const* w, int l) { return w[2 * l + 1]; }

}

extern "C" size_t neraf_nacf_packed_bytes(const neraf_nacf_desc* d) {
  const Dims D = make_dims(d);
  return make_pack_layout(d, D).total;
}

extern "C" size_t neraf_nacf_workspace_bytes(const neraf_nacf_desc* d, int B, int training) {
  const Dims D = make_dims(d);
  return make_ws_layout(d, D, B, training).total;
}

static int check_desc(neraf_ctx* ctx, const neraf_nacf_desc* d) {
  if (!d || d->n_query != 163 || d->W <= 0 || d->C < 1 || d->C > 8 || d->F <= 0 || d->n_feat < 0)
    return neraf_fail(ctx, NERAF_EINVAL, "nacf: unsupported descriptor (n_query must be 163)");
  return NERAF_OK;
}

extern "C" int neraf_nacf_pack_weights(neraf_ctx* ctx, const neraf_nacf_desc* d, const float* const* w, void* packed,
                                       neraf_stream_t stream) {
  if (int e = check_desc(ctx, d)) return e;
  if (d->C + 6 > kMaxCvtJobs || d->C + 5 > 16) return neraf_fail(ctx, NERAF_EINVAL, "nacf_pack_weights: too many heads");
  hipStream_t st = (hipStream_t)stream;
  const Dims D = make_dims(d);
  const PackLayout L = make_pack_layout(d, D);
  char* P = (char*)packed;
  const int ld0 = D.kdense;
  CvtTable t{};
  auto add = [&](const float* src, int ld, int R, int Cc, half_t* dst, int ld_dst, int Rpad, int Cpad, half_t* dstT, int ld_dstT,
                 int RpadT, int CpadT) {
    CvtJob& J = t.j[t.n++];
    J.src = src; J.dst = dst; J.dstT = dstT; J.ld = ld; J.R = R; J.Cc = Cc; J.ld_dst = ld_dst; J.Rpad = Rpad; J.Cpad = Cpad;
    J.ld_dstT = ld_dstT; J.RpadT = RpadT; J.CpadT = CpadT;
    const int rows = std::max(dst ? Rpad : 0, dstT ? RpadT : 0), cols = std::max(dst ? Cpad : 0, dstT ? CpadT : 0);
    J.tiles_x = (cols + 31) / 32;
    J.tile_begin = t.total;
    t.total += J.tiles_x * ((rows + 31) / 32);
  };
  add(Wptr(w, 0) + d->n_feat, ld0, D.n[0], D.k[0], (half_t*)(P + L.w[0]), D.kp[0], D.np[0], D.kp[0], nullptr, 0, 0, 0);
  if (d->dense_l0)
    add(Wptr(w, 0), ld0, D.n[0], D.kdense, (half_t*)(P + L.w0d), D.kdense_p, D.np[0], D.kdense_p, (half_t*)(P + L.w0dt), D.np[0], D.np[0],
        D.kdense_p);
  for (int l = 1; l < 5; ++l)
    add(Wptr(w, l), D.k[l], D.n[l], D.k[l], (half_t*)(P + L.w[l]), D.kp[l], D.np[l], D.kp[l], (half_t*)(P + L.wt[l]), D.np[l], D.np[l],
        round_up(D.kp[l], 128));
  const int kt5 = round_up(D.kp[5], 128);
  for (int c = 0; c < d->C; ++c) {
    const bool last = c == d->C - 1;
    const int rows = last ? D.np[5] - c * d->F : d->F;
    add(w[2 * (5 + c)], d->W, d->F, d->W, (half_t*)(P + L.w[5]) + (size_t)c * d->F * D.kp[5], D.kp[5], rows, D.kp[5],
        (half_t*)(P + L.wt[5]) + (size_t)c * d->F, D.np[5], rows, kt5);
  }
  hipLaunchKernelGGL(cvt_pad_transpose_grouped_kernel, dim3(t.total), dim3(256), 0, st, t);
  SegCopyTable sc{};
  for (int c = 0; c < d->C; ++c) {
    const bool last = c == d->C - 1;
    seg_copy_add(sc, (float*)(P + L.bias[5]) + (size_t)c * d->F, w[2 * (5 + c) + 1], d->F, last ? D.np[5] - c * d->F : d->F);
  }
  for (int l = 0; l < 5; ++l) seg_copy_add(sc, (float*)(P + L.bias[l]), Bptr(w, l), D.n[l], D.np[l]);
  hipLaunchKernelGGL(seg_copy_kernel, dim3(sc.begin[sc.n]), dim3(256), 0, st, sc);
  NERAF_HIP_CHECK(ctx, hipGetLastError());
  return NERAF_OK;
}

extern "C" int neraf_nacf_encode_queries(neraf_ctx* ctx, const neraf_nacf_desc* d, const int64_t* time_query,
                                         const double* mic_pose, const double* source_pose, const double* rot,
                                         const float* aabb_host, int max_len, int B, void* workspace, int training,
                                         neraf_stream_t stream) {
  return neraf_nacf_encode_queries_ex(ctx, d, time_query, mic_pose, source_pose, rot, B, aabb_host, max_len, B, workspace, training, stream);
}

extern "C" int neraf_nacf_encode_queries_ex(neraf_ctx* ctx, const neraf_nacf_desc* d, const int64_t* time_query,
                                            const double* mic_pose, const double* source_pose, const double* rot, int pose_rows,
                                            const float* aabb_host, int max_len, int B, void* workspace, int training,
                                            neraf_stream_t stream) {
  if (int e = check_desc(ctx, d)) return e;
  if (B <= 0 || max_len < 2) return neraf_fail(ctx, NERAF_EINVAL, "encode_queries: B>0 and max_len>=2 required");
  if (pose_rows != B && pose_rows != 1) return neraf_fail(ctx, NERAF_EINVAL, "encode_queries: pose_rows is B or 1");
  const Dims D = make_dims(d);
  const WsLayout L = make_ws_layout(d, D, B, training);
  EncodeArgs a{};
  a.tq = time_query; a.mic = mic_pose; a.src = source_pose; a.rot = rot;
  for (int i = 0; i < 6; ++i) a.aabb[i] = aabb_host[i];
  a.inv_tmax = 1.0f / (float)(max_len - 1.0);
  a.B = B; a.Mpad = L.Mpad; a.pstride = pose_rows == B ? 3 : 0;
  a.q = (half_t*)((char*)workspace + L.q);
  a.qT = (half_t*)((char*)workspace + L.qT);
  hipStream_t st = (hipStream_t)stream;
  long n = (long)L.Mpad * KQ_PAD;
  hipLaunchKernelGGL(encode_queries_kernel, dim3((unsigned)((n + 255) / 256)), dim3(256), 0, st, a, 0);
  if (training) {
    n = (long)QT_ROWS * L.Mpad;
    hipLaunchKernelGGL(encode_queries_kernel, dim3((unsigned)((n + 255) / 256)), dim3(256), 0, st, a, 1);
  }
  NERAF_HIP_CHECK(ctx, hipGetLastError());
  return NERAF_OK;
}

static int nacf_fwd_tail(neraf_ctx* ctx, const neraf_nacf_desc* d, const Dims& D, const PackLayout& PL, const WsLayout& WL,
                         const char* P, char* ws, int B, float* out, int training, hipStream_t st) {
  for (int l = 1; l < 5; ++l) {
    GemmParams g{};
    g.A = (const half_t*)(ws + WL.h[l - 1]); g.lda = D.np[l - 1];
    g.B = (const half_t*)(P + PL.w[l]); g.ldb = D.kp[l];
    g.M = B; g.N = D.n[l]; g.K = D.kp[l]; g.Mpad = WL.Mpad; g.Npad = D.np[l]; g.alpha = 1.f;
    g.bias = (const float*)(P + PL.bias[l]); g.act = ACT_LEAKY;
    g.C16 = (half_t*)(ws + WL.h[l]); g.ldc16 = D.np[l];
    if (training) { g.C16T = (half_t*)(ws + WL.hT[l]); g.ldc16t = WL.Mpad; }
    if (int e = launch_gemm_f16(ctx, g, st)) return e;
  }
  GemmParams g{};
  g.A = (const half_t*)(ws + WL.h[4]); g.lda = D.np[4];
  g.B = (const half_t*)(P + PL.w[5]); g.ldb = D.kp[5];
  g.M = B; g.N = D.n[5]; g.K = D.kp[5]; g.Mpad = WL.Mpad; g.Npad = D.np[5]; g.alpha = 1.f;
  g.bias = (const float*)(P + PL.bias[5]); g.act = ACT_TANH10;
  g.C32 = out; g.ldc32 = D.n[5];
  return launch_gemm_f16(ctx, g, st);
}

extern "C" int neraf_nacf_fwd(neraf_ctx* ctx, const neraf_nacf_desc* d, const void* packed, const float* const* w,
                              const float* feat, int B, float* out, void* workspace, int training,
                              neraf_stream_t stream) {
  if (int e = check_desc(ctx, d)) return e;
  if (B <= 0) return neraf_fail(ctx, NERAF_EINVAL, "nacf_fwd: B must be positive");
  if (d->n_feat > 0 && !feat) return neraf_fail(ctx, NERAF_EINVAL, "nacf_fwd: feat is null");
  hipStream_t st = (hipStream_t)stream;
  const Dims D = make_dims(d);
  const PackLayout PL = make_pack_layout(d, D);
  const WsLayout WL = make_ws_layout(d, D, B, training);
  const char* P = (const char*)packed;
  char* ws = (char*)workspace;
  float* bias0 = (float*)(ws + WL.bias0);
  hipLaunchKernelGGL(feat_gemv_kernel, dim3(D.np[0] / 4), dim3(256), 0, st, Wptr(w, 0), D.kdense, Bptr(w, 0), feat,
                     d->n_feat, D.n[0], D.np[0], bias0);
  NERAF_HIP_CHECK(ctx, hipGetLastError());
  GemmParams g{};
  g.A = (const half_t*)(ws + WL.q); g.lda = KQ_PAD;
  g.B = (const half_t*)(P + PL.w[0]); g.ldb = D.kp[0];
  g.M = B; g.N = D.n[0]; g.K = D.kp[0]; g.Mpad = WL.Mpad; g.Npad = D.np[0]; g.alpha = 1.f;
  g.bias = bias0; g.act = ACT_LEAKY;
  g.C16 = (half_t*)(ws + WL.h[0]); g.ldc16 = D.np[0];
  if (training) { g.C16T = (half_t*)(ws + WL.hT[0]); g.ldc16t = WL.Mpad; }
  if (int e = launch_gemm_f16(ctx, g, st)) return e;
  return nacf_fwd_tail(ctx, d, D, PL, WL, P, ws, B, out, training, st);
}

extern "C" int neraf_nacf_fwd_dense(neraf_ctx* ctx, const neraf_nacf_desc* d, const void* packed, const float* h, int B,
                                    float* out, void* workspace, int training, neraf_stream_t stream) {
  if (int e = check_desc(ctx, d)) return e;
  if (!d->dense_l0) return neraf_fail(ctx, NERAF_EINVAL, "nacf_fwd_dense: descriptor was created without dense_l0");
  if (B <= 0) return neraf_fail(ctx, NERAF_EINVAL, "nacf_fwd_dense: B must be positive");
  hipStream_t st = (hipStream_t)stream;
  const Dims D = make_dims(d);
  const PackLayout PL = make_pack_layout(d, D);
  const WsLayout WL = make_ws_layout(d, D, B, training);
  const char* P = (const char*)packed;
  char* ws = (char*)workspace;
  if (int e = cvt_pad_transpose(ctx, st, h, nullptr, nullptr, D.kdense, B, D.kdense, 0, (half_t*)(ws + WL.hd), D.kdense_p, WL.Mpad,
                                D.kdense_p, training ? (half_t*)(ws + WL.hdT) : nullptr, WL.Mpad, WL.Mpad, D.kdense_p,
                                nullptr))
    return e;
  GemmParams g{};
  g.A = (const half_t*)(ws + WL.hd); g.lda = D.kdense_p;
  g.B = (const half_t*)(P + PL.w0d); g.ldb = D.kdense_p;
  g.M = B; g.N = D.n[0]; g.K = D.kdense_p; g.Mpad = WL.Mpad; g.Npad = D.np[0]; g.alpha = 1.f;
  g.bias = (const float*)(P + PL.bias[0]); g.act = ACT_LEAKY;
  g.C16 = (half_t*)(ws + WL.h[0]); g.ldc16 = D.np[0];
  if (training) { g.C16T = (half_t*)(ws + WL.hT[0]); g.ldc16t = WL.Mpad; }
  if (int e = launch_gemm_f16(ctx, g, st)) return e;
  return nacf_fwd_tail(ctx, d, D, PL, WL, P, ws, B, out, training, st);
}

static int nacf_bwd_body(neraf_ctx* ctx, const neraf_nacf_desc* d, const Dims& D, const PackLayout& PL, const WsLayout& WL,
                         const char* P, char* ws, int B, const float* out, const float* dout, float* const* grads,
                         int* slot0, hipStream_t st) {
  const int M = WL.Mpad;
  neraf_zero_async(st, ws + WL.colsum[0], WL.scale + 256 - WL.colsum[0]);
  float* scale = (float*)(ws + WL.scale);
  const float* inv_scale = scale + 1;
  {
    const size_t n = (size_t)B * D.n[5];
    int blocks = (int)((n + 1023) / 1024);
    if (blocks > 256) blocks = 256;
    hipLaunchKernelGGL(amax_dz5_kernel, dim3(blocks), dim3(256), 0, st, dout, out, n, reinterpret_cast<unsigned*>(scale) + 2);
    hipLaunchKernelGGL(make_scale_kernel, dim3(1), dim3(64), 0, st, scale);
  }
  SegCopyTable outs{};
  outs.mul = inv_scale;
  const bool det = WL.col_slots > 1;
  outs.nslots = WL.col_slots;
  auto copy_out = [&](float* dst, const float* src, int n, int np) { seg_copy_add(outs, dst, src, n, n, np); };
  int cur = 0;
  half_t* dz = (half_t*)(ws + WL.dz[cur]);
  half_t* dzT = (half_t*)(ws + WL.dzT[cur]);
  if (int e = cvt_pad_transpose(ctx, st, dout, out, scale, D.n[5], B, D.n[5], 1, dz, D.np[5], M, D.np[5], dzT, M, M, D.np[5] + 128,
                                (float*)(ws + WL.colsum[5]), det ? D.np[5] : 0))
    return e;
  for (int c = 0; c < d->C; ++c) {
    GemmParams g{};
    g.A = dzT + (size_t)c * d->F * M; g.lda = M;
    g.B = (const half_t*)(ws + WL.hT[4]); g.ldb = M;
    g.M = d->F; g.N = D.n[4]; g.K = M; g.Mpad = round_up(d->F, 128); g.Npad = D.np[4]; g.alpha = 1.f;
    g.alpha_dev = inv_scale;
    g.C32 = grads[2 * (5 + c)]; g.ldc32 = D.n[4];
    if (int e = launch_gemm_f16(ctx, g, st)) return e;
    copy_out(grads[2 * (5 + c) + 1], (const float*)(ws + WL.colsum[5]) + (size_t)c * d->F, d->F, D.np[5]);
  }
  for (int l = 5; l >= 1; --l) {
    const int nxt = cur ^ 1;
    half_t* dzn = (half_t*)(ws + WL.dz[nxt]);
    half_t* dznT = (half_t*)(ws + WL.dzT[nxt]);
    GemmParams g{};
    g.A = (const half_t*)(ws + WL.dz[cur]); g.lda = D.np[l];
    g.B = (const half_t*)(P + PL.wt[l]); g.ldb = D.np[l];
    g.M = B; g.N = D.n[l - 1]; g.K = D.np[l]; g.Mpad = M; g.Npad = D.np[l - 1]; g.alpha = 1.f;
    g.lmask = (const half_t*)(ws + WL.h[l - 1]); g.ldmask = D.np[l - 1]; g.mask_slope = 0.1f;
    g.C16 = dzn; g.ldc16 = D.np[l - 1];
    g.C16T = dznT; g.ldc16t = M;
    g.colsum = (float*)(ws + WL.colsum[l - 1]);
    if (det) { g.stat_det = 1; g.stat_stride = D.np[l - 1]; }
    if (int e = launch_gemm_f16(ctx, g, st)) return e;
    cur = nxt;
    if (l - 1 >= 1) {
      GemmParams w{};
      w.A = dznT; w.lda = M;
      w.B = (const half_t*)(ws + WL.hT[l - 2]); w.ldb = M;
      w.M = D.n[l - 1]; w.N = D.k[l - 1]; w.K = M; w.Mpad = D.np[l - 1]; w.Npad = D.kp[l - 1]; w.alpha = 1.f;
      w.alpha_dev = inv_scale;
      w.C32 = grads[2 * (l - 1)]; w.ldc32 = D.k[l - 1];
      if (int e = launch_gemm_f16(ctx, w, st)) return e;
      copy_out(grads[2 * (l - 1) + 1], (const float*)(ws + WL.colsum[l - 1]), D.n[l - 1], D.np[l - 1]);
    }
  }
  copy_out(grads[1], (const float*)(ws + WL.colsum[0]), D.n[0], D.np[0]);
  hipLaunchKernelGGL(seg_copy_kernel, dim3(outs.begin[outs.n]), dim3(256), 0, st, outs);
  NERAF_HIP_CHECK(ctx, hipGetLastError());
  *slot0 = cur;
  return NERAF_OK;
}

extern "C" int neraf_nacf_bwd(neraf_ctx* ctx, const neraf_nacf_desc* d, const void* packed, const float* const* w,
                              const float* feat, int B, const float* out, const float* dout, float* const* grads,
                              float* dfeat, void* workspace, neraf_stream_t stream) {
  if (int e = check_desc(ctx, d)) return e;
  if (B <= 0 || !out || !dout || !grads) return neraf_fail(ctx, NERAF_EINVAL, "nacf_bwd: bad arguments");
  hipStream_t st = (hipStream_t)stream;
  const Dims D = make_dims(d);
  const PackLayout PL = make_pack_layout(d, D);
  const WsLayout WL = make_ws_layout(d, D, B, 1);
  const char* P = (const char*)packed;
  char* ws = (char*)workspace;
  int s0 = 0;
  if (int e = nacf_bwd_body(ctx, d, D, PL, WL, P, ws, B, out, dout, grads, &s0, st)) return e;
  const int M = WL.Mpad;
  GemmParams g{};
  g.A = (const half_t*)(ws + WL.dzT[s0]); g.lda = M;
  g.B = (const half_t*)(ws + WL.qT); g.ldb = M;
  g.M = D.n[0]; g.N = D.k[0]; g.K = M; g.Mpad = D.np[0]; g.Npad = QT_ROWS; g.alpha = 1.f;
  g.alpha_dev = (const float*)(ws + WL.scale) + 1;
  g.C32 = grads[0] + d->n_feat; g.ldc32 = D.kdense;
  if (int e = launch_gemm_f16(ctx, g, st)) return e;
  const float* db0 = grads[1];
  if (d->n_feat > 0) {
    hipLaunchKernelGGL(outer_kernel, dim3((d->n_feat + 255) / 256, D.n[0]), dim3(256), 0, st, db0, feat, D.n[0], d->n_feat,
                       grads[0], D.kdense, dfeat);
    if (dfeat) {
      float* part = WL.col_slots > 1 ? (float*)(ws + WL.dfeat_part) : nullptr;
      hipLaunchKernelGGL(dfeat_kernel, dim3((d->n_feat + 255) / 256, 64), dim3(256), 0, st, Wptr(w, 0), D.kdense, db0,
                         D.n[0], d->n_feat, dfeat, part);
      if (part) hipLaunchKernelGGL(dfeat_fold_kernel, dim3((d->n_feat + 255) / 256), dim3(256), 0, st, part, 64, d->n_feat, dfeat);
    }
  }
  NERAF_HIP_CHECK(ctx, hipGetLastError());
  return NERAF_OK;
}

extern "C" int neraf_nacf_bwd_dense(neraf_ctx* ctx, const neraf_nacf_desc* d, const void* packed, int B, const float* out,
                                    const float* dout, float* const* grads, float* dh, void* workspace,
                                    neraf_stream_t stream) {
  if (int e = check_desc(ctx, d)) return e;
  if (!d->dense_l0) return neraf_fail(ctx, NERAF_EINVAL, "nacf_bwd_dense: descriptor was created without dense_l0");
  if (B <= 0 || !out || !dout || !grads) return neraf_fail(ctx, NERAF_EINVAL, "nacf_bwd_dense: bad arguments");
  hipStream_t st = (hipStream_t)stream;
  const Dims D = make_dims(d);
  const PackLayout PL = make_pack_layout(d, D);
  const WsLayout WL = make_ws_layout(d, D, B, 1);
  const char* P = (const char*)packed;
  char* ws = (char*)workspace;
  int s0 = 0;
  if (int e = nacf_bwd_body(ctx, d, D, PL, WL, P, ws, B, out, dout, grads, &s0, st)) return e;
  const int M = WL.Mpad;
  GemmParams g{};
  g.A = (const half_t*)(ws + WL.dzT[s0]); g.lda = M;
  g.B = (const half_t*)(ws + WL.hdT); g.ldb = M;
  g.M = D.n[0]; g.N = D.kdense; g.K = M; g.Mpad = D.np[0]; g.Npad = D.kdense_p; g.alpha = 1.f;
  g.alpha_dev = (const float*)(ws + WL.scale) + 1;
  g.C32 = grads[0]; g.ldc32 = D.kdense;
  if (int e = launch_gemm_f16(ctx, g, st)) return e;
  if (dh) {
    GemmParams x{};
    x.A = (const half_t*)(ws + WL.dz[s0]); x.lda = D.np[0];
    x.B = (const half_t*)(P + PL.w0dt); x.ldb = D.np[0];
    x.M = B; x.N = D.kdense; x.K = D.np[0]; x.Mpad = M; x.Npad = D.kdense_p; x.alpha = 1.f;
    x.alpha_dev = (const float*)(ws + WL.scale) + 1;
    x.C32 = dh; x.ldc32 = D.kdense;
    if (int e = launch_gemm_f16(ctx, x, st)) return e;
  }
  return NERAF_OK;
}

extern "C" int neraf_stft_loss_sums(neraf_ctx* ctx, const float* pred, const float* gt, size_t n, int loss_type,
                                    float* sums, neraf_stream_t stream) {
  if (!pred || !gt || !sums || n == 0) return neraf_fail(ctx, NERAF_EINVAL, "stft_loss_sums: bad arguments");
  hipStream_t st = (hipStream_t)stream;
  int blocks = (int)((n + 1023) / 1024);
  if (blocks > 256) blocks = 256;
  hipLaunchKernelGGL(stft_loss_sums_kernel, dim3(blocks), dim3(256), 0, st, pred, gt, n, loss_type, sums + 4);
  hipLaunchKernelGGL(stft_sums_fold_kernel, dim3(1), dim3(64), 0, st, sums + 4, blocks, sums);
  NERAF_HIP_CHECK(ctx, hipGetLastError());
  return NERAF_OK;
}

extern "C" int neraf_stft_loss_finalize(neraf_ctx* ctx, const float* sums, size_t n_total, const float* weights, float* losses,
                                        neraf_stream_t stream) {
  if (!sums || !losses || n_total == 0) return neraf_fail(ctx, NERAF_EINVAL, "stft_loss_finalize: bad arguments");
  hipLaunchKernelGGL(stft_loss_final_kernel, dim3(1), dim3(64), 0, (hipStream_t)stream, sums, 1.0f / (float)n_total, weights, losses);
  NERAF_HIP_CHECK(ctx, hipGetLastError());
  return NERAF_OK;
}

extern "C" int neraf_stft_loss_fwd(neraf_ctx* ctx, const float* pred, const float* gt, size_t n, int loss_type,
                                   float* sums, float* losses, neraf_stream_t stream) {
  if (int e = neraf_stft_loss_sums(ctx, pred, gt, n, loss_type, sums, stream)) return e;
  return neraf_stft_loss_finalize(ctx, sums, n, nullptr, losses, stream);
}

extern "C" int neraf_stft_loss_bwd(neraf_ctx* ctx, const float* pred, const float* gt, size_t n, size_t n_total,
                                   int loss_type, const float* sums, const float* g_sc, const float* g_mag, const float* weights,
                                   float extra, float* dpred, neraf_stream_t stream) {
  if (!pred || !gt || !sums || !dpred || n == 0 || n_total < n)
    return neraf_fail(ctx, NERAF_EINVAL, "stft_loss_bwd: bad arguments");
  hipStream_t st = (hipStream_t)stream;
  int blocks = (int)((n + 255) / 256);
  if (blocks > 2048) blocks = 2048;
  hipLaunchKernelGGL(stft_loss_bwd_kernel, dim3(blocks), dim3(256), 0, st, pred, gt, n, n_total, loss_type, sums, g_sc, g_mag, weights, extra, dpred);
  NERAF_HIP_CHECK(ctx, hipGetLastError());
  return NERAF_OK;
}
```

neraf_amd/csrc/resnet3d.hip:

```cpp
#include "resnet3d_common.h"
#include <algorithm>

namespace {

__global__ __launch_bounds__(256) void grid_to_ndhwc8_kernel(const float* __restrict__ grid, size_t nvox, half_t* __restrict__ out) {
  const size_t v = (size_t)blockIdx.x * 256 + threadIdx.x;
  if (v >= nvox) return;
  half8 h;
#pragma unroll
  for (int c = 0; c < 7; ++c) h[c] = (half_t)grid[c * nvox + v];
  h[7] = (half_t)0.f;
  reinterpret_cast<half8*>(out)[v] = h;
}

__global__ __launch_bounds__(256) void grid_window_to_ndhwc8_kernel(const float* __restrict__ grid, size_t nvox, const unsigned long long* start,
                                                                   int n, half_t* __restrict__ out) {
  const int t = blockIdx.x * 256 + threadIdx.x;
  if (t >= n) return;
  const size_t v = (size_t)*start + t;
  if (v >= nvox) return;
  half8 h;
#pragma unroll
  for (int c = 0; c < 7; ++c) h[c] = (half_t)grid[c * nvox + v];
  h[7] = (half_t)0.f;
  reinterpret_cast<half8*>(out)[v] = h;
}

__global__ void set_u64_fwd_kernel(unsigned long long* p, unsigned long long v) { if (threadIdx.x == 0 && blockIdx.x == 0) p[0] = v; }

struct RunTable {
  int n;
  int begin[kMaxConv + 1];
  unsigned long long stat_off[kMaxConv];
  int cpad[kMaxConv];
  float unbias[kMaxConv];
  float* rmean[kMaxConv]; float* rvar[kMaxConv];
  long long* nbt[kMaxConv];
};

__global__ __launch_bounds__(256) void bn_update_running_all_kernel(RunTable t, const char* __restrict__ ws, float mom) {
  if (blockIdx.x == 0 && (int)threadIdx.x < t.n && t.nbt[threadIdx.x]) *t.nbt[threadIdx.x] += 1;
  const int idx = blockIdx.x * 256 + threadIdx.x;
  if (idx >= t.begin[t.n]) return;
  int lo = 0, hi = t.n - 1;
  while (lo < hi) { const int mid = (lo + hi + 1) >> 1; if (t.begin[mid] <= idx) lo = mid; else hi = mid - 1; }
  const int i = lo, c = idx - t.begin[i];
  const float* fin = reinterpret_cast<const float*>(ws + t.stat_off[i]);
  const float mean = fin[c], var = fin[t.cpad[i] + c];
  t.rmean[i][c] = (1.f - mom) * t.rmean[i][c] + mom * mean;
  t.rvar[i][c] = (1.f - mom) * t.rvar[i][c] + mom * var * t.unbias[i];
}

__global__ __launch_bounds__(256) void bn_relu_maxpool_kernel(BnSrc s, int din, int dout, size_t m_in, half_t* __restrict__ out,
                                                             unsigned char* __restrict__ arg) {
  __shared__ float sc[64], sh[64];
  if (threadIdx.x < 64) bn_scale_shift(s, threadIdx.x, 1.f / (float)m_in, sc[threadIdx.x], sh[threadIdx.x]);
  __syncthreads();
  const size_t total = cube(dout) * 8;
  const size_t idx = (size_t)blockIdx.x * 256 + threadIdx.x;
  if (idx >= total) return;
  const size_t vox = idx >> 3; const int c0 = (int)(idx & 7) * 8;
  const int x = (int)(vox % dout), y = (int)((vox / dout) % dout), z = (int)(vox / ((size_t)dout * dout));
  float best[8]; int at[8];
#pragma unroll
  for (int j = 0; j < 8; ++j) { best[j] = -3.0e38f; at[j] = 255; }
  for (int dz = -1; dz <= 1; ++dz) {
    const int iz = 2 * z + dz; if ((unsigned)iz >= (unsigned)din) continue;
    for (int dy = -1; dy <= 1; ++dy) {
      const int iy = 2 * y + dy; if ((unsigned)iy >= (unsigned)din) continue;
      for (int dx = -1; dx <= 1; ++dx) {
        const int ix = 2 * x + dx; if ((unsigned)ix >= (unsigned)din) continue;
        const half8 v = *reinterpret_cast<const half8*>(s.x + (((size_t)iz * din + iy) * din + ix) * 64 + c0);
        const int tap = (dz + 1) * 9 + (dy + 1) * 3 + (dx + 1);
#pragma unroll
        for (int j = 0; j < 8; ++j) {
          const float a = fmaxf(fmaf((float)v[j], sc[c0 + j], sh[c0 + j]), 0.f);
          if (a > best[j]) { best[j] = a; at[j] = tap; }
        }
      }
    }
  }
  if (arg) {
    unsigned long long packed = 0ull;
#pragma unroll
    for (int j = 0; j < 8; ++j) packed |= (unsigned long long)(best[j] > 0.f ? at[j] : 255) << (8 * j);
    *reinterpret_cast<unsigned long long*>(arg + vox * 64 + c0) = packed;
  }
  half8 o;
#pragma unroll
  for (int j = 0; j < 8; ++j) o[j] = (half_t)best[j];
  *reinterpret_cast<half8*>(out + vox * 64 + c0) = o;
}

__global__ __launch_bounds__(256) void avgpool_kernel(const half_t* __restrict__ x, int M, int C, float* __restrict__ feat) {
  __shared__ float part[32][65];
  const int chunk = threadIdx.x & 7, grp = threadIdx.x >> 3;
  const int c0 = blockIdx.x * 64 + chunk * 8;
  float s[8] = {0.f, 0.f, 0.f, 0.f, 0.f, 0.f, 0.f, 0.f};
  for (int r = grp; r < M; r += 32) {
    const half8 v = *reinterpret_cast<const half8*>(x + (size_t)r * C + c0);
#pragma unroll
    for (int j = 0; j < 8; ++j) s[j] += (float)v[j];
  }
#pragma unroll
  for (int j = 0; j < 8; ++j) part[grp][chunk * 8 + j] = s[j];
  __syncthreads();
  if (threadIdx.x < 64) {
    float v[32];
#pragma unroll
    for (int k = 0; k < 32; ++k) v[k] = part[k][threadIdx.x];
#pragma unroll
    for (int w = 1; w < 32; w <<= 1)
#pragma unroll
      for (int k = 0; k < 32; k += 2 * w) v[k] += v[k + w];
    feat[blockIdx.x * 64 + threadIdx.x] = v[0] * (1.f / (float)M);
  }
}

}

extern "C" int neraf_resnet3d_num_convs(const neraf_resnet3d_desc* d) {
  Arch A;
  if (make_arch(d, &A)) return -1;
  return A.nconv;
}

extern "C" size_t neraf_resnet3d_packed_bytes(const neraf_resnet3d_desc* d) {
  Arch A; Layout L;
  if (make_arch(d, &A)) return 0;
  make_layout(A, &L);
  return L.packed_total;
}

extern "C" size_t neraf_resnet3d_workspace_bytes(const neraf_resnet3d_desc* d) {
  Arch A; Layout L;
  if (make_arch(d, &A)) return 0;
  make_layout(A, &L);
  return L.total;
}

extern "C" double neraf_resnet3d_forward_flops(const neraf_resnet3d_desc* d) {
  Arch A;
  if (make_arch(d, &A)) return -1.0;
  double f = 0.0;
  for (int i = 0; i < A.nconv; ++i) {
    const ConvSpec& c = A.conv[i];
    f += 2.0 * (double)cube(c.dout) * (c.k * c.k * c.k) * c.cin_real * c.cout;
  }
  return f;
}

extern "C" int neraf_resnet3d_debug_locate(const neraf_resnet3d_desc* d, int kind, int index, size_t* offset, int* rows, int* cols) {
  Arch A; Layout L;
  if (make_arch(d, &A) || !offset || !rows || !cols) return NERAF_EINVAL;
  make_layout(A, &L);
  if (kind >= 0 && kind <= 2) {
    if (index < 0 || index >= A.nblock) return NERAF_EINVAL;
    const ConvSpec& c = A.conv[A.block[index].conv[kind]];
    *offset = kind == 0 ? L.a1[index] : kind == 1 ? L.a2[index] : L.out[index];
    *rows = (int)cube(c.dout); *cols = c.cout;
    return NERAF_OK;
  }
  if (kind == 7) { *offset = L.x0; *rows = (int)cube(A.S); *cols = 8; return NERAF_OK; }
  if (kind == 3) { *offset = L.act_pool; *rows = (int)cube(A.pooled); *cols = 64; return NERAF_OK; }
  if (kind == 4) { *offset = L.pool_arg; *rows = (int)cube(A.pooled); *cols = 64; return NERAF_OK; }
  if (kind == 5 || kind == 6) {
    if (index < 0 || index >= A.nconv) return NERAF_EINVAL;
    const ConvSpec& c = A.conv[index];
    if (kind == 5) { *offset = L.pre[index]; *rows = (int)cube(c.dout); *cols = c.cout; }
    else { *offset = L.fin[index]; *rows = 2; *cols = round_up(c.cout, 128); }
    return NERAF_OK;
  }
  return NERAF_EINVAL;
}

extern "C" int neraf_resnet3d_pack_weights(neraf_ctx* ctx, const neraf_resnet3d_desc* d, const float* const* conv_w, void* packed,
                                           neraf_stream_t stream) {
  Arch A; Layout L;
  if (make_arch(d, &A) || !conv_w || !packed) return neraf_fail(ctx, NERAF_EINVAL, "resnet3d_pack_weights: bad arguments");
  make_layout(A, &L);
  hipStream_t st = (hipStream_t)stream;
  PackTable t{};
  BrickTable bt{};
  unsigned long long acc = 0;
  int tiles = 0, max_run = 0;
  for (int i = 0; i < A.nconv; ++i) {
    const ConvSpec& c = A.conv[i];
    const int taps = c.k * c.k * c.k;
    if (brick_packable(c) && conv_kpad(c) == taps * c.cin && conv_npad(c) == c.cout) {
      const int j = bt.n++;
      int cob, cib;
      brick_shape(c, 0, &cob, &cib);
      bt.src[j] = conv_w[i]; bt.tile_begin[j] = tiles; bt.dst_off[j] = L.w[i];
      bt.cout[j] = c.cout; bt.cin[j] = c.cin; bt.taps[j] = taps; bt.cib[j] = cib; bt.cob[j] = cob;
      tiles += (c.cout / cob) * (c.cin / cib);
      max_run = std::max(max_run, cob * (cib * taps + 2));
      continue;
    }
    const int j = t.n++;
    t.src[j] = conv_w[i]; t.begin[j] = acc; t.dst_off[j] = L.w[i];
    t.cout[j] = c.cout; t.cin_real[j] = c.cin_real; t.cin[j] = c.cin; t.taps[j] = taps;
    t.kpad[j] = conv_kpad(c);
    acc += (unsigned long long)conv_npad(c) * conv_kpad(c);
  }
  t.begin[t.n] = acc;
  bt.tile_begin[bt.n] = tiles;
  if (t.n > 0) hipLaunchKernelGGL(pack_all_conv_weights_kernel, dim3((unsigned)((acc + 255) / 256)), dim3(256), 0, st, t, (char*)packed);
  if (bt.n > 0) {
    const size_t lds = brick_lds_bytes(max_run);
    static size_t attr_lds = 0;
    if (lds > attr_lds) {
      NERAF_HIP_CHECK(ctx, hipFuncSetAttribute(reinterpret_cast<const void*>(&pack_bricks_kernel<0>),
                                               hipFuncAttributeMaxDynamicSharedMemorySize, (int)lds));
      attr_lds = lds;
    }
    hipLaunchKernelGGL(pack_bricks_kernel<0>, dim3((unsigned)tiles), dim3(256), lds, st, bt, (char*)packed);
  }
  NERAF_HIP_CHECK(ctx, hipGetLastError());
  return NERAF_OK;
}

static int resnet3d_fwd_body(neraf_ctx* ctx, const Arch& A, const Layout& L, const char* packed, const float* const* bn, const float* grid,
                             char* ws, float* feat, int use_batch_stats, int win_cells, hipStream_t st) {
  neraf_zero3_async(st, ws + L.zero_page, 256, ws + L.stats_begin, L.stats_bytes, feat, (size_t)A.n_features * sizeof(float));
  neraf_node(ctx, "neraf_zero3_kernel | statistics accumulators", 0.0, 0.0, 256.0 + (double)L.stats_bytes + 4096.0);
  const size_t nvox = cube(A.S);
  const bool training = use_batch_stats != 0;
  if (win_cells > 0) {
    hipLaunchKernelGGL(grid_window_to_ndhwc8_kernel, dim3((unsigned)((win_cells + 255) / 256)), dim3(256), 0, st, grid, nvox,
                       reinterpret_cast<const unsigned long long*>(ws + L.win), win_cells, (half_t*)(ws + L.x0));
    neraf_node(ctx, "grid_window_to_ndhwc8_kernel | refresh window -> fp16 channels-last", 0.0, win_cells * 28.0, win_cells * 16.0);
  } else {
    hipLaunchKernelGGL(grid_to_ndhwc8_kernel, dim3((unsigned)((nvox + 255) / 256)), dim3(256), 0, st, grid, nvox, (half_t*)(ws + L.x0));
    neraf_node(ctx, "grid_to_ndhwc8_kernel | grid -> fp16 channels-last", 0.0, (double)nvox * 28.0, (double)nvox * 16.0);
  }
  if (int e = run_conv(ctx, st, A, L, 0, packed, ws, (const half_t*)(ws + L.x0))) return e;
  {
    const ConvSpec& c = A.conv[0];
    BnSrc s = bn_src_fwd(A, L, ws, bn, 0, use_batch_stats);
    const size_t total = cube(A.pooled) * 8;
    hipLaunchKernelGGL(bn_relu_maxpool_kernel, dim3((unsigned)((total + 255) / 256)), dim3(256), 0, st, s, c.dout, A.pooled,
                       cube(c.dout), (half_t*)(ws + L.act_pool), training ? (unsigned char*)(ws + L.pool_arg) : nullptr);
    NERAF_HIP_CHECK(ctx, hipGetLastError());
    neraf_node(ctx, "bn_relu_maxpool_kernel | stem BatchNorm + ReLU + 3x3x3/2 max-pool", 0.0, (double)cube(c.dout) * 64 * 2.0,
               (double)cube(A.pooled) * 64 * (training ? 3.0 : 2.0));
  }
  const half_t* x = (const half_t*)(ws + L.act_pool);
  for (int b = 0; b < A.nblock; ++b) {
    const BlockSpec& B = A.block[b];
    const int i0 = B.conv[0], i1 = B.conv[1], i2 = B.conv[2];
    const ConvSpec &c0 = A.conv[i0], &c1 = A.conv[i1], &c2 = A.conv[i2];
    if (int e = run_conv(ctx, st, A, L, i0, packed, ws, x)) return e;
    BnApplyArgs a{};
    a.a = bn_src_fwd(A, L, ws, bn, i0, use_batch_stats);
    a.M = (int)cube(c0.dout); a.Mpad = (int)rows_pad(c0.dout); a.C = c0.cout; a.relu = 1; a.out = (half_t*)(ws + L.a1[b]);
    if (int e = run_bn_apply(ctx, st, a)) return e;
    if (int e = run_conv(ctx, st, A, L, i1, packed, ws, (const half_t*)(ws + L.a1[b]))) return e;
    BnApplyArgs a2{};
    a2.a = bn_src_fwd(A, L, ws, bn, i1, use_batch_stats);
    a2.M = (int)cube(c1.dout); a2.Mpad = (int)rows_pad(c1.dout); a2.C = c1.cout; a2.relu = 1; a2.out = (half_t*)(ws + L.a2[b]);
    static const int skip_small = [] { const char* e = getenv("NERAF_SKIP_SMALL_BN"); return e ? atoi(e) : 0; }();
    if (!(skip_small && cube(c1.dout) <= 4096))
    if (int e = run_bn_apply(ctx, st, a2)) return e;
    if (int e = run_conv(ctx, st, A, L, i2, packed, ws, (const half_t*)(ws + L.a2[b]))) return e;
    BnApplyArgs a3{};
    a3.a = bn_src_fwd(A, L, ws, bn, i2, use_batch_stats);
    if (B.ds >= 0) {
      if (int e = run_conv(ctx, st, A, L, B.ds, packed, ws, x)) return e;
      a3.r = bn_src_fwd(A, L, ws, bn, B.ds, use_batch_stats);
    } else {
      a3.res = x;
    }
    a3.M = (int)cube(c2.dout); a3.Mpad = (int)rows_pad(c2.dout); a3.C = c2.cout; a3.relu = 1; a3.out = (half_t*)(ws + L.out[b]);
    if (int e = run_bn_apply(ctx, st, a3)) return e;
    x = (const half_t*)(ws + L.out[b]);
  }
  {
    const int M = (int)cube(A.final_edge), C = A.n_features;
    hipLaunchKernelGGL(avgpool_kernel, dim3(C / 64), dim3(256), 0, st, x, M, C, feat);
    NERAF_HIP_CHECK(ctx, hipGetLastError());
    neraf_node(ctx, "avgpool_kernel | mean over the voxels", 0.0, (double)M * C * 2.0, C * 4.0);
  }
  return NERAF_OK;
}

extern "C" int neraf_resnet3d_fwd(neraf_ctx* ctx, const neraf_resnet3d_desc* d, const void* packed_, const float* const* bn,
                                  const float* grid, void* workspace, float* feat, int use_batch_stats, size_t win_start, int win_cells,
                                  neraf_stream_t stream) {
  Arch A; Layout L;
  if (make_arch(d, &A) || !packed_ || !bn || !grid || !workspace || !feat || win_cells < 0 ||
      (win_cells > 0 && win_start + (size_t)win_cells > cube(d->grid_size)))
    return neraf_fail(ctx, NERAF_EINVAL, "resnet3d_fwd: bad arguments (grid_size 64|128|256, in_channels 7, n_features 1024|2048, window inside the grid)");
  make_layout(A, &L);
  if (win_cells > 0)
    hipLaunchKernelGGL(set_u64_fwd_kernel, dim3(1), dim3(64), 0, (hipStream_t)stream,
                       reinterpret_cast<unsigned long long*>((char*)workspace + L.win), (unsigned long long)win_start);
  ArgHash k;
  k.add(0x66776431u); k.add(d->grid_size); k.add(packed_); k.ptrs((const void* const*)bn, 4 * A.nconv); k.add(grid); k.add(workspace);
  k.add(feat); k.add(use_batch_stats); k.add(win_cells);
  return neraf_run_graphed(ctx, (hipStream_t)stream, k.h, [&](hipStream_t st) {
    return resnet3d_fwd_body(ctx, A, L, (const char*)packed_, bn, grid, (char*)workspace, feat, use_batch_stats, win_cells, st);
  });
}

extern "C" int neraf_resnet3d_update_running_stats(neraf_ctx* ctx, const neraf_resnet3d_desc* d, const void* workspace,
                                                   float* const* bn, float momentum, int64_t* const* num_batches_tracked,
                                                   neraf_stream_t stream) {
  Arch A; Layout L;
  if (make_arch(d, &A) || !workspace || !bn) return neraf_fail(ctx, NERAF_EINVAL, "resnet3d_update_running_stats: bad arguments");
  make_layout(A, &L);
  const char* ws = (const char*)workspace;
  RunTable t{};
  t.n = A.nconv;
  int acc = 0;
  for (int i = 0; i < A.nconv; ++i) {
    const ConvSpec& c = A.conv[i];
    const float m = (float)cube(c.dout);
    t.begin[i] = acc; t.stat_off[i] = L.fin[i]; t.cpad[i] = round_up(c.cout, 128);
    t.unbias[i] = m / (m - 1.f);
    t.rmean[i] = bn[4 * i + 2]; t.rvar[i] = bn[4 * i + 3];
    t.nbt[i] = num_batches_tracked ? (long long*)num_batches_tracked[i] : nullptr;
    acc += c.cout;
  }
  t.begin[A.nconv] = acc;
  hipLaunchKernelGGL(bn_update_running_all_kernel, dim3((acc + 255) / 256), dim3(256), 0, (hipStream_t)stream, t, ws, momentum);
  NERAF_HIP_CHECK(ctx, hipGetLastError());
  return NERAF_OK;
}
```

neraf_amd/csrc/resnet3d_bwd.hip:

```cpp
#include "resnet3d_common.h"
#include <algorithm>
#include <mutex>
#include <stddef.h>
#include <stdlib.h>
#include <string.h>
#include <unordered_map>

namespace {

struct PackTTable {
  int n;
  const float* src[kMaxConv];
  int tile_begin[kMaxConv + 1];
  unsigned long long dst_off[kMaxConv];
  int cout[kMaxConv], cin[kMaxConv], taps[kMaxConv], kcols[kMaxConv], nrows[kMaxConv];
};

__global__ __launch_bounds__(256) void pack_dgrad_weights_kernel(PackTTable t, char* __restrict__ packed) {
  extern __shared__ half_t brick[];
  int lo = 0, hi = t.n - 1;
  const int bid = blockIdx.x;
  while (lo < hi) { const int mid = (lo + hi + 1) >> 1; if (t.tile_begin[mid] <= bid) lo = mid; else hi = mid - 1; }
  const int i = lo;
  const int tile = bid - t.tile_begin[i];
// ... 67 lines not shown
  r.x = *reinterpret_cast<const half8*>(p.s.x + off);
  if (p.g16) r.g16 = *reinterpret_cast<const half8*>(p.g16 + off);
  else { r.g0 = *reinterpret_cast<const f32x4*>(p.g32 + off); r.g1 = *reinterpret_cast<const f32x4*>(p.g32 + off + 4); }
  if (p.act) r.act = *reinterpret_cast<const half8*>(p.act + off);
}
__device__ __forceinline__ void bn_bwd_finish(const BnBwdArgs& p, const BnBwdRaw& r, float (&xv)[8], float (&g)[8]) {
#pragma unroll
  for (int j = 0; j < 8; ++j) xv[j] = (float)r.x[j];
  if (p.g16) {
#pragma unroll
    for (int j = 0; j < 8; ++j) g[j] = (float)r.g16[j];
  } else {
#pragma unroll
    for (int j = 0; j < 4; ++j) { g[j] = r.g0[j]; g[4 + j] = r.g1[j]; }
  }
  if (p.act) {
#pragma unroll
    for (int j = 0; j < 8; ++j) if (!((float)r.act[j] > 0.f)) g[j] = 0.f;
  }
}
__device__ __forceinline__ void bn_bwd_load(const BnBwdArgs& p, size_t off, float (&xv)[8], float (&g)[8]) {
  BnBwdRaw r;
  bn_bwd_issue(p, off, r);
  bn_bwd_finish(p, r, xv, g);
}

__global__ __launch_bounds__(256) void bn_bwd_reduce_kernel(BnBwdArgs p) {
  __shared__ float mean[64], rstd[64];
  __shared__ float red[2][32][65];
  const int c_base = blockIdx.y * 64;
  const int tid = threadIdx.x;
  const int ch = tid & 7, rsub = tid >> 3;
  const int r_begin = blockIdx.x * p.rows_per_block;
  const int r_end = min(p.M, r_begin + p.rows_per_block);
  BnBwdRaw first;
  const bool has_first = r_begin + rsub < r_end;
  if (has_first) bn_bwd_issue(p, (size_t)(r_begin + rsub) * p.C + c_base + ch * 8, first);
  if (tid < 64) { float m, v; bn_mean_var(p.s, c_base + tid, 0.f, m, v); mean[tid] = m; rstd[tid] = rsqrtf(v + 1e-5f); }
  __syncthreads();
  float s1[8], s2[8];
#pragma unroll
  for (int j = 0; j < 8; ++j) { s1[j] = 0.f; s2[j] = 0.f; }
  for (int row = r_begin + rsub; row < r_end; row += 32) {
    float xv[8], g[8];
    if (row == r_begin + rsub) bn_bwd_finish(p, first, xv, g);
    else bn_bwd_load(p, (size_t)row * p.C + c_base + ch * 8, xv, g);
#pragma unroll
    for (int j = 0; j < 8; ++j) {
      s1[j] += g[j];
      s2[j] += g[j] * (xv[j] - mean[ch * 8 + j]) * rstd[ch * 8 + j];
    }
  }
#pragma unroll
  for (int j = 0; j < 8; ++j) { red[0][rsub][ch * 8 + j] = s1[j]; red[1][rsub][ch * 8 + j] = s2[j]; }
  __syncthreads();
  if (tid < 128) {
    const int which = tid >> 6, col = tid & 63;
    float acc = 0.f;
#pragma unroll 8
    for (int r = 0; r < 32; ++r) acc += red[which][r][col];
    if (p.det) {
      p.sums[(size_t)(blockIdx.x * (p.rows_per_block >> 5)) * (2 * p.s.cpad) + which * p.s.cpad + c_base + col] = acc;
    } else {
      const int rep = p.rep > 1 ? (blockIdx.x & (p.rep - 1)) * kStatStride : 0;
      atomicAdd(p.sums + rep + which * p.s.cpad + c_base + col, acc);
    }
  }
}

__global__ __launch_bounds__(256) void bn_bwd_apply_kernel(BnBwdArgs p) {
  __shared__ float mean[64], rstd[64], k1[64], k2[64], k3[64];
  __shared__ float part[2][4][64];
  const int c_base = blockIdx.y * 64, m0 = blockIdx.x * 64;
  const int tid = threadIdx.x;
  const float inv_m = 1.f / (float)p.M;
  BnBwdRaw raw[2];
  size_t offs[2];
  bool in[2];
#pragma unroll
  for (int it = 0; it < 2; ++it) {
    const int e = it * 256 + tid, row = e >> 3, ch = e & 7;
    const int m = m0 + row;
    offs[it] = (size_t)m * p.C + c_base + ch * 8;
    in[it] = m < p.M;
    if (in[it]) bn_bwd_issue(p, offs[it], raw[it]);
  }
  float fm = 0.f, fv = 0.f, gam = 0.f;
  const float isc = p.isc ? p.isc[0] : 1.f;
  const float rsc = p.osc ? p.osc[0] / isc : 1.f, rmk = p.msc ? p.msc[0] / isc : 1.f;
  if (tid < 64) { bn_mean_var(p.s, c_base + tid, 0.f, fm, fv); gam = p.s.gamma[c_base + tid]; }
  {
    const int c = c_base + (tid & 63), q = tid >> 6;
    float db = 0.f, dg = 0.f;
    for (int r = q; r < p.rep; r += 4) {
      db += stat_ld(p.sums + r * kStatStride + c, p.s.read_mode); dg += stat_ld(p.sums + r * kStatStride + p.s.cpad + c, p.s.read_mode);
    }
    part[0][q][tid & 63] = db; part[1][q][tid & 63] = dg;
  }
  __syncthreads();
  if (tid < 64) {
    const int c = c_base + tid;
    const float rs = rsqrtf(fv + 1e-5f);
    const float dbeta = (part[0][0][tid] + part[0][1][tid]) + (part[0][2][tid] + part[0][3][tid]);
    const float dgamma = (part[1][0][tid] + part[1][1][tid]) + (part[1][2][tid] + part[1][3][tid]);
    mean[tid] = fm; rstd[tid] = rs;
    k1[tid] = gam * rs * rsc; k2[tid] = dbeta * inv_m; k3[tid] = dgamma * inv_m;
    if (blockIdx.x == 0 && p.dgamma) { p.dgamma[c] = dgamma * p.inv_scale[0]; p.dbeta[c] = dbeta * p.inv_scale[0]; }
  }
  __syncthreads();
  float am = 0.f, am_in = 0.f;
  half8 o[2], om[2];
#pragma unroll
  for (int it = 0; it < 2; ++it) {
    const int ch = (it * 256 + tid) & 7;
    if (in[it]) {
      float xv[8], g[8];
      bn_bwd_finish(p, raw[it], xv, g);
#pragma unroll
      for (int j = 0; j < 8; ++j) {
        const int c = ch * 8 + j;
        const float xh = (xv[j] - mean[c]) * rstd[c];
        const float v = k1[c] * (g[j] - k2[c] - xh * k3[c]);
        am = fmaxf(am, fabsf(v));
        am_in = fmaxf(am_in, fabsf(g[j]));
        o[it][j] = (half_t)v;
        om[it][j] = (half_t)(g[j] * rmk);
      }
    } else {
#pragma unroll
      for (int j = 0; j < 8; ++j) { o[it][j] = (half_t)0.f; om[it][j] = (half_t)0.f; }
    }
  }
  if (p.amax_out) {
    __shared__ float wmax[2][4];
#pragma unroll
    for (int o2 = 32; o2 > 0; o2 >>= 1) { am = fmaxf(am, __shfl_xor(am, o2)); am_in = fmaxf(am_in, __shfl_xor(am_in, o2)); }
    if ((tid & 63) == 0) { wmax[0][tid >> 6] = am; wmax[1][tid >> 6] = am_in; }
    __syncthreads();
    if (tid < 2) {
      const float m4 = fmaxf(fmaxf(wmax[tid][0], wmax[tid][1]), fmaxf(wmax[tid][2], wmax[tid][3]));
      unsigned* dst = tid == 0 ? p.amax_out : p.amax_in;
      if (dst && m4 > 0.f) atomicMax(dst + ((blockIdx.x * 3u + blockIdx.y) & (kAmaxRep - 1)) * kAmaxStride, __float_as_uint(m4));
    }
  }
#pragma unroll
  for (int it = 0; it < 2; ++it) {
    *reinterpret_cast<half8*>(p.dx + offs[it]) = o[it];
    if (p.dy_masked) *reinterpret_cast<half8*>(p.dy_masked + offs[it]) = om[it];
  }
}

__global__ __launch_bounds__(256) void bwd_prologue_kernel(const float* __restrict__ dfeat, float* __restrict__ scale, int target_log2, int M,
                                                          int Mpad, int C, half_t* __restrict__ g, ChainState* __restrict__ cs,
                                                          unsigned* __restrict__ amax, int n_groups, ChainParents par) {
  __shared__ float red[4];
  __shared__ unsigned s_am[kChainMax];
  __shared__ ChainParents s_par;
  constexpr int kWords = kChainMax * kAmaxRep / 256;
  unsigned v[kWords];
  unsigned magic = 0u, passes_in = 0u;
  int e_in = 0;
  if (blockIdx.x == 0) {
#pragma unroll
    for (int k = 0; k < kWords; ++k) {
      const int i = threadIdx.x + k * 256;
      v[k] = i < n_groups * kAmaxRep ? __hip_atomic_load(amax + (size_t)i * kAmaxStride, __ATOMIC_RELAXED, __HIP_MEMORY_SCOPE_SYSTEM) : 0u;
    }
    magic = cs->magic; passes_in = cs->passes;
    if ((int)threadIdx.x < n_groups) e_in = cs->e[threadIdx.x];
  }
  float df[8];
#pragma unroll
  for (int k = 0; k < 8; ++k) df[k] = (int)(threadIdx.x + k * 256) < C ? fabsf(dfeat[threadIdx.x + k * 256]) : 0.f;
  float m = 0.f;
  int nan_seen = 0;
#pragma unroll
  for (int k = 0; k < 8; ++k) { m = (df[k] == df[k] && df[k] > m) ? df[k] : m; nan_seen |= df[k] != df[k]; }
#pragma unroll
  for (int o = 32; o > 0; o >>= 1) m = fmaxf(m, __shfl_xor(m, o));
  if ((threadIdx.x & 63) == 0) red[threadIdx.x >> 6] = m;
  __syncthreads();
  const float amx = fmaxf(fmaxf(red[0], red[1]), fmaxf(red[2], red[3]));
  int es = 0;
  if (amx > 0.f && amx < 3.0e38f) {
    es = target_log2 - (int)floorf(log2f(amx));
    es = es > 100 ? 100 : (es < -100 ? -100 : es);
  }
  const float S = exp2f((float)es);
  if (blockIdx.x == 0) {
    const int dfeat_bad = __syncthreads_or(nan_seen) || !(amx < 3.0e38f);
    if (threadIdx.x == 0) { scale[0] = S; scale[1] = 1.f / S; }
    if ((int)threadIdx.x < kChainMax) { s_par.p[threadIdx.x] = par.p[threadIdx.x]; s_am[threadIdx.x] = 0u; }
    const bool valid = magic == kChainMagic;
    __syncthreads();
    bool any = false;
#pragma unroll
    for (int k = 0; k < kWords; ++k) {
      const int i = threadIdx.x + k * 256;
      if (i < n_groups * kAmaxRep && v[k]) { amax[(size_t)i * kAmaxStride] = 0u; if (valid) atomicMax(&s_am[i / kAmaxRep], v[k]); any = true; }
    }
    const int recorded = __syncthreads_or(any ? 1 : 0);
    if (threadIdx.x < 64) {
      const int lane = threadIdx.x;
      const bool in = lane < n_groups;
      const unsigned mx = in ? s_am[lane] : 0u;
      const int p = (in && lane > 0) ? s_par.p[lane] : 0;
      const int eo = (in && valid) ? e_in : 0;
      const int eo_p = __shfl(eo, p);
      int ok = (lane == 0 || !in) ? 1 : (mx < 0x477fe000u ? 1 : 0);
      int anc = p;
#pragma unroll
      for (int r = 0; r < 6; ++r) { ok &= __shfl(ok, anc); anc = __shfl(anc, anc); }
      const int okp = __shfl(ok, p);
      const bool measured = okp && mx > 0u && mx < 0x7f800000u;
      const bool blind = okp && in && lane > 0 && mx >= 0x7f800000u;
      int done = (lane == 0 || !in || measured || blind) ? 1 : 0;
      int acc = (lane == 0 || !in) ? 0 : (measured ? eo + kChainTarget - ((int)(mx >> 23) - 127) : (blind ? eo - kChainOverflowStep : eo - eo_p));
      int link = done ? lane : p;
#pragma unroll
      for (int r = 0; r < 6; ++r) {
        const int a2 = __shfl(acc, link), d2 = __shfl(done, link), l2 = __shfl(link, link);
        if (!done) { acc += a2; done = d2; link = l2; }
      }
      const int lim_lo = max(-100, -120 - es), lim_hi = min(100, 120 - es);
      const int e = acc < lim_lo ? lim_lo : (acc > lim_hi ? lim_hi : acc);
      const unsigned long long bad = __ballot(in && !ok);
      if (in) { cs->e[lane] = e; cs->pow2[lane] = exp2f((float)e); cs->inv[lane] = exp2f((float)(-es - e)); }
      if (lane == 0) {
        if (!valid) cs->unsettled = (unsigned)n_groups;
        else if (recorded) cs->unsettled = (unsigned)__popcll(bad);
        cs->passes = valid ? passes_in + 1u : 1u;
        cs->dfeat_bad = dfeat_bad ? 1u : 0u;
        cs->magic = kChainMagic;
      }
    }
  }
  const float k = S / (float)M;
  const size_t total = (size_t)Mpad * C;
  for (size_t idx = (size_t)blockIdx.x * 256 + threadIdx.x; idx < total; idx += (size_t)gridDim.x * 256) {
    const int row = (int)(idx / C), c = (int)(idx % C);
    g[idx] = (half_t)(row < M ? dfeat[c] * k : 0.f);
  }
}

__global__ __launch_bounds__(256) void maxpool_bwd_gather_kernel(const unsigned char* __restrict__ arg, int din, int dout,
                                                                const half_t* __restrict__ g, half_t* __restrict__ dpost, size_t rows_pad_in) {
  const size_t idx = (size_t)blockIdx.x * 256 + threadIdx.x;
  if (idx >= rows_pad_in * 8) return;
  const size_t vox = idx >> 3; const int c0 = (int)(idx & 7) * 8;
  float acc[8];
#pragma unroll
  for (int j = 0; j < 8; ++j) acc[j] = 0.f;
  if (vox < cube(din)) {
    const int ix = (int)(vox % din), iy = (int)((vox / din) % din), iz = (int)(vox / ((size_t)din * din));
    int oz[2], tz[2], oy[2], ty[2], ox[2], tx[2];
    auto wins = [&](int i, int (&o)[2], int (&tp)[2]) {
      if ((i & 1) == 0) { o[0] = i >> 1; tp[0] = 1; return 1; }
      o[0] = (i - 1) >> 1; tp[0] = 2;
      if (((i + 1) >> 1) < dout) { o[1] = (i + 1) >> 1; tp[1] = 0; return 2; }
      return 1;
    };
    const int nz = wins(iz, oz, tz), ny = wins(iy, oy, ty), nx = wins(ix, ox, tx);
    for (int a = 0; a < nz; ++a)
      for (int b = 0; b < ny; ++b)
        for (int c = 0; c < nx; ++c) {
          const size_t ov = ((size_t)oz[a] * dout + oy[b]) * dout + ox[c];
          const unsigned tap = (unsigned)(tz[a] * 9 + ty[b] * 3 + tx[c]);
          const unsigned long long am = *reinterpret_cast<const unsigned long long*>(arg + ov * 64 + c0);
          const half8 gv = *reinterpret_cast<const half8*>(g + ov * 64 + c0);
#pragma unroll
          for (int j = 0; j < 8; ++j)
            if (((am >> (8 * j)) & 0xffu) == tap) acc[j] += (float)gv[j];
        }
  }
  half8 o;
#pragma unroll
  for (int j = 0; j < 8; ++j) o[j] = (half_t)acc[j];
  *reinterpret_cast<half8*>(dpost + vox * 64 + c0) = o;
}

__global__ void set_f32x2_kernel(float* p, float a, float b) { if (threadIdx.x == 0 && blockIdx.x == 0) { p[0] = a; p[1] = b; } }
__global__ void set_u64_kernel(unsigned long long* p, unsigned long long v) { if (threadIdx.x == 0 && blockIdx.x == 0) p[0] = v; }

__global__ __launch_bounds__(256) void stem_w_relayout_kernel(const float* __restrict__ W, float* __restrict__ Wt) {
  const int idx = blockIdx.x * 256 + threadIdx.x;
  if (idx >= 125 * 8 * 64) return;
  const int co = idx & 63, c = (idx >> 6) & 7, tap = idx >> 9;
  Wt[idx] = c < 7 ? W[((size_t)co * 7 + c) * 125 + tap] : 0.f;
}

__global__ __launch_bounds__(256) void stem_dgrid_kernel(const half_t* __restrict__ dy, const float* __restrict__ Wt, int S, int dout,
                                                        const unsigned long long* __restrict__ start_dev, int n, int nch,
                                                        const float* __restrict__ inv_scale, float* __restrict__ dgrid) {
  const int lane = threadIdx.x & 63;
  const int i = blockIdx.x * 4 + (threadIdx.x >> 6);
  if (i >= n) return;
  const size_t cell = (size_t)start_dev[0] + i;
  const int x = (int)(cell % S), y = (int)((cell / S) % S), z = (int)(cell / ((size_t)S * S));
  float acc[7] = {0.f, 0.f, 0.f, 0.f, 0.f, 0.f, 0.f};
  for (int dz = 0; dz < 5; ++dz) {
    const int nz = z + 2 - dz; if (nz < 0 || (nz & 1) || (nz >> 1) >= dout) continue;
    for (int dyy = 0; dyy < 5; ++dyy) {
      const int ny = y + 2 - dyy; if (ny < 0 || (ny & 1) || (ny >> 1) >= dout) continue;
      for (int dx = 0; dx < 5; ++dx) {
        const int nx = x + 2 - dx; if (nx < 0 || (nx & 1) || (nx >> 1) >= dout) continue;
        const float d = (float)dy[((size_t)((nz >> 1) * dout + (ny >> 1)) * dout + (nx >> 1)) * 64 + lane];
        const float* w = Wt + (size_t)((dz * 5 + dyy) * 5 + dx) * 512 + lane;
#pragma unroll
        for (int c = 0; c < 7; ++c) if (c < nch) acc[c] = fmaf(d, w[c * 64], acc[c]);
      }
    }
  }
#pragma unroll
  for (int c = 0; c < 7; ++c) {
    if (c >= nch) break;
    float v = acc[c];
#pragma unroll
    for (int o = 32; o > 0; o >>= 1) v += __shfl_xor(v, o);
    if (lane == 0) dgrid[(size_t)c * n + i] = v * inv_scale[0];
  }
}

__global__ void f16_to_f32_kernel(const half_t* __restrict__ a, size_t n, const float* __restrict__ mul, float* __restrict__ o) {
  const size_t i = (size_t)blockIdx.x * blockDim.x + threadIdx.x;
  if (i < n) o[i] = (float)a[i] * mul[0];
}

struct BwdLayout {
  size_t wt[64];
  size_t packed_total;
  size_t scale;
  size_t chain, amax;
  size_t sums[64];
  size_t sums_fin[64];
  size_t sums_begin, sums_bytes;
  size_t g[2];
  size_t dy[64];
  size_t gm, da;
  size_t dpost;
  size_t wtmp;
  size_t splitk; size_t splitk_bytes;
  size_t total;
};

inline int bwd_rows_per_block(const ConvSpec& c) {
  static const int min_rows = [] { const char* e = getenv("NERAF_BN_BWD_MIN_ROWS"); return e ? atoi(e) : 32; }();
  static const int max_blocks = [] { const char* e = getenv("NERAF_BN_BWD_MAX_BLOCKS"); return e ? atoi(e) : 512; }();
  const int M = (int)cube(c.dout);
  return std::max(min_rows, round_up((M + max_blocks - 1) / max_blocks, 32));
}
inline int bwd_stat_rep(const ConvSpec& c) {
  if (2 * round_up(c.cout, 128) > kStatStride) return 1;
  const int M = (int)cube(c.dout), rpb = bwd_rows_per_block(c);
  const int nrb = (M + rpb - 1) / rpb;
  int r = 1;
  while (r < 16 && r * 8 < nrb) r <<= 1;
  return r;
}

void make_bwd_layout(const Arch& A, BwdLayout* L) {
  size_t off = 0;
  auto take = [&](size_t bytes) { size_t o = off; off += round_up_sz(bytes, 256); return o; };
  for (int i = 0; i < A.nconv; ++i) {
    const ConvSpec& c = A.conv[i];
    const int nrows = c.cin == 64 || c.cin == 8 ? 64 : round_up(c.cin, 128);
    L->wt[i] = take((size_t)nrows * c.k * c.k * c.k * c.cout * 2);
  }
  L->packed_total = off;
  off = 0;
  L->scale = take(256);
  L->chain = take(sizeof(ChainState));
  L->amax = take((size_t)kChainMax * kAmaxRep * kAmaxStride * 4);
  L->sums_begin = off;
  for (int i = 0; i < A.nconv; ++i) {
    const int rep = bwd_stat_rep(A.conv[i]);
    if (neraf_deterministic()) L->sums[i] = take(det_slots(A.conv[i]) * 2 * round_up(A.conv[i].cout, 128) * 4);
    else L->sums[i] = take(rep > 1 ? (size_t)rep * kStatStride * 4 : (size_t)2 * round_up(A.conv[i].cout, 128) * 4);
  }
  L->sums_bytes = off - L->sums_begin;
  for (int i = 0; i < A.nconv; ++i) L->sums_fin[i] = take((size_t)2 * round_up(A.conv[i].cout, 128) * 4);
  size_t max_act = 0, max_wtmp = 0;
  for (int i = 0; i < A.nconv; ++i) {
    const ConvSpec& c = A.conv[i];
    const size_t rows_out = rows_pad(c.dout), rows_in = rows_pad(c.din);
    if (i > 0) {
      max_act = std::max(max_act, rows_out * c.cout * 2);
      max_act = std::max(max_act, rows_in * c.cin * 2);
    }
    max_wtmp = std::max(max_wtmp, (size_t)125 * 8 * 64 * 4);
  }
  for (int i = 0; i < 2; ++i) L->g[i] = take(max_act);
  for (int i = 0; i < A.nconv; ++i) L->dy[i] = take(rows_pad(A.conv[i].dout) * A.conv[i].cout * 2);
  L->gm = take(max_act); L->da = take(max_act);
  L->dpost = take(cube(A.conv[0].dout) * 64 * 4);
  L->wtmp = take(max_wtmp);
  L->splitk_bytes = (size_t)192 << 20;
  L->splitk = take(L->splitk_bytes);
  L->total = off;
}

struct Ctx {
  neraf_ctx* ctx; hipStream_t st; const Arch* A; const Layout* L; const BwdLayout* B;
  const char* packed_t; char* ws; char* bws; const float* const* bn; float* const* w_grads; float* const* bn_grads;
  const float* pow2(int t) const { return reinterpret_cast<const ChainState*>(bws + B->chain)->pow2 + t; }
  const float* inv(int t) const { return reinterpret_cast<const ChainState*>(bws + B->chain)->inv + t; }
  const float* inv_base() const { return reinterpret_cast<const ChainState*>(bws + B->chain)->inv; }
  bool track = true;
  unsigned* amax(int t) const { return track ? reinterpret_cast<unsigned*>(bws + B->amax) + (size_t)t * kAmaxRep * kAmaxStride : nullptr; }
};

int bn_backward(const Ctx& c, int ci, const half_t* g16, const float* g32, const half_t* act, half_t* dx, half_t* dy_masked,
                int k_in, int k_out, int k_mask, bool sums_done = false) {
  const ConvSpec& cs = c.A->conv[ci];
  BnBwdArgs p{};
  p.s = bn_src_bwd(*c.A, *c.L, c.ws, c.bn, ci);
  p.g16 = g16; p.g32 = g32; p.act = act;
  p.M = (int)cube(cs.dout); p.Mpad = (int)rows_pad(cs.dout); p.C = cs.cout;
  p.rows_per_block = bwd_rows_per_block(cs);
  p.sums = (float*)(c.bws + c.B->sums[ci]); p.rep = bwd_stat_rep(cs);
  p.dx = dx; p.dy_masked = dy_masked;
  p.dgamma = c.bn_grads[2 * ci]; p.dbeta = c.bn_grads[2 * ci + 1]; p.inv_scale = c.inv(k_in);
  p.osc = c.pow2(k_out); p.isc = c.pow2(k_in); p.msc = dy_masked ? c.pow2(k_mask) : nullptr;
  p.amax_out = c.amax(k_out); p.amax_in = g16 ? c.amax(k_in) : nullptr;
  const int nrb = (p.M + p.rows_per_block - 1) / p.rows_per_block;
  p.det = neraf_deterministic() ? 1 : 0;
  if (!sums_done) hipLaunchKernelGGL(bn_bwd_reduce_kernel, dim3(nrb, p.C / 64), dim3(256), 0, c.st, p);
  if (c.ctx && c.ctx->manifest) {
    char nm[96];
    const double elems = (double)p.M * p.C;
    if (!sums_done) {
      snprintf(nm, sizeof(nm), "bn_bwd_reduce_kernel | M=%d C=%d", p.M, p.C);
      neraf_node(c.ctx, nm, 0.0, elems * (2.0 + (g16 ? 2.0 : 4.0) + (act ? 2.0 : 0.0)), 0.0);
    }
    snprintf(nm, sizeof(nm), "bn_bwd_apply_kernel | M=%d C=%d%s", p.M, p.C, dy_masked ? " + masked copy" : "");
    neraf_node(c.ctx, nm, 0.0, elems * (2.0 + (g16 ? 2.0 : 4.0) + (act ? 2.0 : 0.0)), (double)p.Mpad * p.C * 2.0 * (dy_masked ? 2 : 1));
  }
  static const int skip_small = [] { const char* e = getenv("NERAF_SKIP_SMALL_BN"); return e ? atoi(e) : 0; }();
  if (skip_small >= 2 && cube(cs.dout) <= 4096 && cs.k == 1) return NERAF_OK;
  if (p.det) {
    float* fin = (float*)(c.bws + c.B->sums_fin[ci]);
    run_slot_sum(c.st, p.sums, det_slots(cs), p.s.cpad, 0.f, 0, fin);
    p.sums = fin; p.rep = 1;
  }
  hipLaunchKernelGGL(bn_bwd_apply_kernel, dim3(p.Mpad / 64, p.C / 64), dim3(256), 0, c.st, p);
  NERAF_HIP_CHECK(c.ctx, hipGetLastError());
  return NERAF_OK;
}

inline WgradItem wgrad_item(const Ctx& c, int ci, const half_t* dy, const half_t* x_in, int t_dy) {
  const ConvSpec& cs = c.A->conv[ci];
  WgradItem it{};
  it.dy = dy; it.x = x_in; it.out = c.w_grads[ci];
  it.cout = cs.cout; it.cin = cs.cin; it.cin_real = cs.cin_real; it.ksize = cs.k; it.stride = cs.stride; it.pad = cs.pad;
  it.din = cs.din; it.dout = cs.dout; it.K = (int)rows_pad(cs.dout);
  it.alpha_idx = t_dy;
  return it;
}

int conv_wgrad(const Ctx& c, int ci, const half_t* dy, const half_t* x_in, int t_dy) {
  const WgradItem it = wgrad_item(c, ci, dy, x_in, t_dy);
  return launch_wgrad_grouped(c.ctx, &it, 1, (const half_t*)(c.ws + c.L->zero_page), (float*)(c.bws + c.B->splitk), c.B->splitk_bytes,
                              c.inv_base(), c.st);
}

inline bool fuse_bn_sums(const ConvSpec& bn_conv) {
  static const int on = [] { const char* e = getenv("NERAF_BN_FUSE_SUMS"); return e ? atoi(e) : 1; }();
  static const long max_vox = [] { const char* e = getenv("NERAF_BN_FUSE_MAX_VOX"); return e ? atol(e) : 4096l; }();
  return on && (long)cube(bn_conv.dout) <= max_vox && (bn_conv.cout % 64) == 0;
}

int conv_dgrad(const Ctx& c, int ci, const half_t* dy, const half_t* add16, half_t* dx, int bn_ci = -1, const half_t* bn_act = nullptr) {
  const ConvSpec& cs = c.A->conv[ci];
  GemmParams g{};
  const int taps = cs.k * cs.k * cs.k;
  g.A = (const half_t*)dy; g.lda = cs.cout;
  g.B = (const half_t*)(c.packed_t + c.B->wt[ci]); g.ldb = taps * cs.cout;
  g.M = (int)cube(cs.din); g.N = cs.cin; g.K = taps * cs.cout; g.Mpad = (int)rows_pad(cs.din);
  g.Npad = cs.cin == 64 ? 64 : round_up(cs.cin, 128); g.tile_n = cs.cin == 64 ? 64 : 0; g.alpha = 1.f;
  g.alg_flops = 2.0 * (double)cube(cs.dout) * taps * cs.cin_real * cs.cout;
  g.add16 = (const half_t*)add16; g.ldadd = cs.cin;
  g.C16 = (half_t*)dx; g.ldc16 = cs.cin;
  g.splitk_ws = (float*)(c.bws + c.B->splitk); g.splitk_ws_bytes = c.B->splitk_bytes;
  if (bn_ci >= 0) {
    const ConvSpec& bs = c.A->conv[bn_ci];
    float* sums = (float*)(c.bws + c.B->sums[bn_ci]);
    g.colsum = sums; g.colsumsq = sums + round_up(bs.cout, 128);
    g.stat_rep = bwd_stat_rep(bs); g.stat_stride = kStatStride;
    if (neraf_deterministic()) { g.stat_det = 1; g.stat_rep = 0; g.stat_stride = 2 * round_up(bs.cout, 128); }
    g.bnb_x = (const half_t*)(c.ws + c.L->pre[bn_ci]); g.ldbnb = bs.cout; g.bnb_mask = (const half_t*)bn_act;
    g.bnb_fin = (const float*)(c.ws + c.L->fin[bn_ci]); g.bnb_cpad = round_up(bs.cout, 128);
  }
  if (cs.k == 1 && cs.stride == 1) {
    g.conv.loader = 0;
  } else {
    g.conv.loader = 1; g.conv.cin = cs.cout; g.conv.din = cs.dout; g.conv.dout = cs.din; g.conv.stride = 1; g.conv.pad = -cs.pad;
    g.conv.ksize = cs.k; g.conv.tflip = 1; g.conv.tstride = cs.stride;
    g.conv.zero_page = (const half_t*)(c.ws + c.L->zero_page);
  }
  return launch_gemm_f16(c.ctx, g, c.st);
}

}

extern "C" size_t neraf_resnet3d_bwd_packed_bytes(const neraf_resnet3d_desc* d) {
  Arch A; BwdLayout B;
  if (make_arch(d, &A)) return 0;
  make_bwd_layout(A, &B);
  return B.packed_total;
}

extern "C" size_t neraf_resnet3d_bwd_workspace_bytes(const neraf_resnet3d_desc* d) {
  Arch A; BwdLayout B;
  if (make_arch(d, &A)) return 0;
  make_bwd_layout(A, &B);
  return B.total;
}

extern "C" int neraf_resnet3d_pack_weights_bwd(neraf_ctx* ctx, const neraf_resnet3d_desc* d, const float* const* conv_w, void* packed_t,
                                               neraf_stream_t stream) {
  Arch A; BwdLayout B;
  if (make_arch(d, &A) || !conv_w || !packed_t) return neraf_fail(ctx, NERAF_EINVAL, "resnet3d_pack_weights_bwd: bad arguments");
  make_bwd_layout(A, &B);
  hipStream_t st = (hipStream_t)stream;
  PackTTable t{};
  BrickTable bt{};
  int acc = 0, max_taps = 1, tiles = 0, max_run = 0;
  for (int i = 1; i < A.nconv; ++i) {
    const ConvSpec& c = A.conv[i];
    const int taps = c.k * c.k * c.k;
    const int nrows = c.cin == 64 || c.cin == 8 ? 64 : round_up(c.cin, 128);
    if (brick_packable(c) && nrows == c.cin) {
      const int j = bt.n++;
      int cob, cib;
      brick_shape(c, 1, &cob, &cib);
      bt.src[j] = conv_w[i]; bt.tile_begin[j] = tiles; bt.dst_off[j] = B.wt[i];
      bt.cout[j] = c.cout; bt.cin[j] = c.cin; bt.taps[j] = taps; bt.cib[j] = cib; bt.cob[j] = cob;
      tiles += (c.cout / cob) * (c.cin / cib);
      max_run = std::max(max_run, cob * (cib * taps + 2));
      continue;
    }
    const int j = t.n++;
    t.src[j] = conv_w[i]; t.tile_begin[j] = acc; t.dst_off[j] = B.wt[i];
    t.cout[j] = c.cout; t.cin[j] = c.cin_real; t.taps[j] = taps; t.kcols[j] = taps * c.cout; t.nrows[j] = nrows;
    acc += (c.cout / 32) * (nrows / 32);
    max_taps = std::max(max_taps, taps);
  }
  t.tile_begin[t.n] = acc;
  bt.tile_begin[bt.n] = tiles;
  if (t.n > 0)
    if (int e = launch_pack_dgrad(ctx, t, acc, max_taps, (char*)packed_t, st)) return e;
  if (bt.n > 0) {
    const size_t lds = brick_lds_bytes(max_run);
    static size_t attr_lds = 0;
    if (lds > attr_lds) {
      NERAF_HIP_CHECK(ctx, hipFuncSetAttribute(reinterpret_cast<const void*>(&pack_bricks_kernel<1>),
                                               hipFuncAttributeMaxDynamicSharedMemorySize, (int)lds));
      attr_lds = lds;
    }
    hipLaunchKernelGGL(pack_bricks_kernel<1>, dim3((unsigned)tiles), dim3(256), lds, st, bt, (char*)packed_t);
    NERAF_HIP_CHECK(ctx, hipGetLastError());
  }
  return NERAF_OK;
}

static int resnet3d_bwd_body(neraf_ctx* ctx, const Arch& A, const Layout& L, const BwdLayout& B, const void* packed_t,
                             const float* const* conv_w, const float* const* bn, char* ws, char* bws, const float* dfeat,
                             float* const* w_grads, float* const* bn_grads, int n_cells, int n_ch, float* dgrid_cells, hipStream_t st,
                             bool track) {
  float* scale = (float*)(bws + B.scale);
  neraf_zero_async(st, bws + B.sums_begin, B.sums_bytes);
  neraf_node(ctx, "neraf_zero_kernel | BatchNorm-backward accumulators", 0.0, 0.0, (double)B.sums_bytes);
  const int Mlast = (int)cube(A.final_edge);
  Ctx c{ctx, st, &A, &L, &B, (const char*)packed_t, ws, bws, bn, w_grads, bn_grads};
  c.track = track;
  half_t* g = (half_t*)(bws + B.g[0]);
  half_t* g_next = (half_t*)(bws + B.g[1]);
  ChainParents par{};
  int n_k = 0;
  auto new_k = [&](int parent) { par.p[n_k] = (unsigned char)parent; return n_k++; };
  int k_g = new_k(0);
  const int total_k = 1 + 3 * A.nblock + 1;
  if (total_k > kChainMax) return neraf_fail(ctx, NERAF_EINVAL, "resnet3d_bwd: chain table too small");
  {
    const int Mpad = (int)rows_pad(A.final_edge);
    const size_t n = (size_t)Mpad * A.n_features;
    unsigned blocks = (unsigned)((n + 255) / 256);
    if (blocks > 1024) blocks = 1024;
    ChainParents pp{};
    int k = 1, kg = 0;
    for (int b = A.nblock - 1; b >= 0; --b) { pp.p[k] = (unsigned char)kg; pp.p[k + 1] = (unsigned char)k; pp.p[k + 2] = (unsigned char)(k + 1); kg = k + 2; k += 3; }
    pp.p[k] = (unsigned char)kg;
    hipLaunchKernelGGL(bwd_prologue_kernel, dim3(blocks), dim3(256), 0, st, dfeat, scale, kChainTarget + (int)ceilf(log2f((float)Mlast)), Mlast, Mpad,
                       A.n_features, g, reinterpret_cast<ChainState*>(bws + B.chain), reinterpret_cast<unsigned*>(bws + B.amax), total_k, pp);
    neraf_node(ctx, "bwd_prologue_kernel | S0, scale groups, average-pool backward", 0.0, 4096.0 + (double)total_k * kAmaxRep * 4.0, (double)n * 2.0);
  }
  half_t* gm = (half_t*)(bws + B.gm); half_t* da = (half_t*)(bws + B.da);
  WgradItem items[64]; int n_items = 0;
  bool g_sums_done = false;
  for (int b = A.nblock - 1; b >= 0; --b) {
    const BlockSpec& Bk = A.block[b];
    const int i0 = Bk.conv[0], i1 = Bk.conv[1], i2 = Bk.conv[2];
    const half_t* out = (const half_t*)(ws + L.out[b]);
    const half_t* a1 = (const half_t*)(ws + L.a1[b]);
    const half_t* a2 = (const half_t*)(ws + L.a2[b]);
    const half_t* x_in = b == 0 ? (const half_t*)(ws + L.act_pool) : (const half_t*)(ws + L.out[b - 1]);
    half_t* dy0 = (half_t*)(bws + B.dy[i0]); half_t* dy1 = (half_t*)(bws + B.dy[i1]); half_t* dy2 = (half_t*)(bws + B.dy[i2]);
    half_t* dyds = Bk.ds >= 0 ? (half_t*)(bws + B.dy[Bk.ds]) : nullptr;
    const int k2 = new_k(k_g), k1 = new_k(k2), k0 = new_k(k1);
    if (int e = bn_backward(c, i2, g, nullptr, out, dy2, Bk.ds < 0 ? gm : nullptr, k_g, k2, k0, g_sums_done)) return e;
    g_sums_done = false;
    items[n_items++] = wgrad_item(c, i2, dy2, a2, k2);
    const bool f1 = fuse_bn_sums(A.conv[i1]);
    if (int e = conv_dgrad(c, i2, dy2, nullptr, da, f1 ? i1 : -1, f1 ? a2 : nullptr)) return e;
    if (int e = bn_backward(c, i1, da, nullptr, a2, dy1, nullptr, k2, k1, -1, f1)) return e;
    items[n_items++] = wgrad_item(c, i1, dy1, a1, k1);
    const bool f0 = fuse_bn_sums(A.conv[i0]) && A.conv[i1].stride == 1;
    if (int e = conv_dgrad(c, i1, dy1, nullptr, da, f0 ? i0 : -1, f0 ? a1 : nullptr)) return e;
    if (int e = bn_backward(c, i0, da, nullptr, a1, dy0, nullptr, k1, k0, -1, f0)) return e;
    items[n_items++] = wgrad_item(c, i0, dy0, x_in, k0);
    if (Bk.ds >= 0) {
      if (int e = bn_backward(c, Bk.ds, g, nullptr, out, dyds, nullptr, k_g, k0, -1)) return e;
      items[n_items++] = wgrad_item(c, Bk.ds, dyds, x_in, k0);
      if (int e = conv_dgrad(c, i0, dy0, nullptr, g_next)) return e;
      if (int e = conv_dgrad(c, Bk.ds, dyds, g_next, g_next)) return e;
    } else {
      const bool fg = b > 0 && A.block[b - 1].ds < 0 && fuse_bn_sums(A.conv[A.block[b - 1].conv[2]]);
      if (int e = conv_dgrad(c, i0, dy0, gm, g_next, fg ? A.block[b - 1].conv[2] : -1, fg ? (const half_t*)(ws + L.out[b - 1]) : nullptr)) return e;
      g_sums_done = fg;
    }
    half_t* t = g; g = g_next; g_next = t;
    k_g = k0;
  }
  {
    const ConvSpec& c0 = A.conv[0];
    half_t* dpost = (half_t*)(bws + B.dpost);
    const size_t rp = rows_pad(c0.dout);
    hipLaunchKernelGGL(maxpool_bwd_gather_kernel, dim3((unsigned)((rp * 8 + 255) / 256)), dim3(256), 0, st,
                       (const unsigned char*)(ws + L.pool_arg), c0.dout, A.pooled, g, dpost, rp);
    NERAF_HIP_CHECK(ctx, hipGetLastError());
    neraf_node(ctx, "maxpool_bwd_gather_kernel | max-pool routing", 0.0, (double)cube(A.pooled) * 64 * 3.0, (double)rp * 64 * 2.0);
    half_t* dy0 = (half_t*)(bws + B.dy[0]);
    const int k_s = new_k(k_g);
    if (int e = bn_backward(c, 0, dpost, nullptr, nullptr, dy0, nullptr, k_g, k_s, -1)) return e;
    items[n_items++] = wgrad_item(c, 0, dy0, (const half_t*)(ws + L.x0), k_s);
    if (n_cells > 0) {
      float* Wt = (float*)(bws + B.wtmp);
      hipLaunchKernelGGL(stem_w_relayout_kernel, dim3((125 * 8 * 64 + 255) / 256), dim3(256), 0, st, conv_w[0], Wt);
      hipLaunchKernelGGL(stem_dgrid_kernel, dim3((n_cells + 3) / 4), dim3(256), 0, st, dy0, Wt, A.S, c0.dout,
                         reinterpret_cast<const unsigned long long*>(bws + B.scale + 64), n_cells, n_ch, c.inv(k_s), dgrid_cells);
      NERAF_HIP_CHECK(ctx, hipGetLastError());
      neraf_node(ctx, "stem_w_relayout_kernel | W[co][c][tap] -> Wt[tap][c][co]", 0.0, 125.0 * 7 * 64 * 4, 125.0 * 8 * 64 * 4);
      neraf_node(ctx, "stem_dgrid_kernel | grid gradient of the refresh window", 2.0 * n_cells * (125.0 / 8.0) * 64 * n_ch, (double)n_cells * (125.0 / 8.0) * 128.0,
                 (double)n_cells * n_ch * 4.0);
    }
  }
  if (n_k != total_k) return neraf_fail(ctx, NERAF_EINVAL, "resnet3d_bwd: scale group count mismatch");
  (void)par;
  return launch_wgrad_grouped(ctx, items, n_items, (const half_t*)(ws + L.zero_page), (float*)(bws + B.splitk), B.splitk_bytes, c.inv_base(), st);
}

static std::mutex g_calib_mu;
static std::unordered_map<const void*, unsigned> g_calibrated;
constexpr int kMaxCalibrationPasses = 48;

__global__ void chain_set_kernel(ChainState* cs, int e0, int e1, int e2) {
  if (threadIdx.x != 0 || blockIdx.x != 0) return;
  const int e[3] = {e0, e1, e2};
  for (int t = 0; t < 3; ++t) { cs->e[t] = e[t]; cs->pow2[t] = exp2f((float)e[t]); cs->inv[t] = exp2f((float)-e[t]); }
  cs->magic = kChainMagic;
}

extern "C" int neraf_resnet3d_bwd_reset(neraf_ctx* ctx, void* bwd_workspace) {
  (void)ctx;
  std::lock_guard<std::mutex> lk(g_calib_mu);
  g_calibrated.erase(bwd_workspace);
  return NERAF_OK;
}

extern "C" int neraf_resnet3d_bwd(neraf_ctx* ctx, const neraf_resnet3d_desc* d, const void* packed_t, const float* const* conv_w,
                                  const float* const* bn, void* workspace, void* bwd_workspace, const float* dfeat,
                                  float* const* w_grads, float* const* bn_grads, size_t cell_start, int n_cells, int n_ch,
                                  float* dgrid_cells, neraf_stream_t stream) {
  Arch A; Layout L; BwdLayout B;
  if (make_arch(d, &A) || !packed_t || !conv_w || !bn || !workspace || !bwd_workspace || !dfeat || !w_grads || !bn_grads ||
      (n_cells > 0 && (!dgrid_cells || n_ch < 1 || n_ch > 7 || cell_start + (size_t)n_cells > cube(d->grid_size))))
    return neraf_fail(ctx, NERAF_EINVAL, "resnet3d_bwd: bad arguments");
  make_layout(A, &L);
  make_bwd_layout(A, &B);
  hipStream_t st = (hipStream_t)stream;
  char* bws = (char*)bwd_workspace;
  hipLaunchKernelGGL(set_u64_kernel, dim3(1), dim3(64), 0, st, reinterpret_cast<unsigned long long*>(bws + B.scale + 64),
                     (unsigned long long)cell_start);
  static const bool track_env = [] { const char* e = getenv("NERAF_CHAIN_AMAX"); return !(e && atoi(e) == 0); }();
  static const unsigned period = [] { const char* e = getenv("NERAF_CHAIN_AMAX_PERIOD"); const int v = e ? atoi(e) : 4; return (unsigned)(v < 1 ? 1 : v); }();
  auto run = [&](hipStream_t s2, bool track) {
    return resnet3d_bwd_body(ctx, A, L, B, packed_t, conv_w, bn, (char*)workspace, bws, dfeat, w_grads, bn_grads, n_cells, n_ch, dgrid_cells, s2,
                             track);
  };

  bool fresh;
  unsigned pass_no;
  {
    std::lock_guard<std::mutex> lk(g_calib_mu);
    auto it = g_calibrated.find(bwd_workspace);
    fresh = it == g_calibrated.end();
    if (fresh) it = g_calibrated.emplace(bwd_workspace, 0u).first;
    pass_no = it->second++;
  }
  const bool track = track_env && (pass_no % period) == 0;
  auto body = [&](hipStream_t s2) { return run(s2, track); };
  if (fresh) {
    struct ProfPause { neraf_ctx* c; bool was; ProfPause(neraf_ctx* c_) : c(c_), was(c_ && c_->prof) { if (c) c->prof = false; }
                       ~ProfPause() { if (c) c->prof = was; } } pause(ctx);
    auto forget = [&] { std::lock_guard<std::mutex> lk(g_calib_mu); g_calibrated.erase(bwd_workspace); };
    NERAF_HIP_CHECK(ctx, hipMemsetAsync(bws + B.chain, 0, sizeof(ChainState), st));
    bool settled = false, postponed = false;
    unsigned unsettled = 0;
    for (int i = 0; i < kMaxCalibrationPasses && !settled && !postponed; ++i) {
      if (int e = run(st, true)) { forget(); return e; }
      struct { unsigned unsettled, passes, dfeat_bad; } rd = {0u, 0u, 0u};
      static_assert(offsetof(ChainState, dfeat_bad) == offsetof(ChainState, unsettled) + 8, "read as one block");
      hipError_t he = hipMemcpyAsync(&rd, bws + B.chain + offsetof(ChainState, unsettled), sizeof(rd), hipMemcpyDeviceToHost, st);
      if (he == hipSuccess) he = hipStreamSynchronize(st);
      if (he != hipSuccess) { forget(); NERAF_HIP_CHECK(ctx, he); }
      unsettled = rd.unsettled;
      postponed = rd.dfeat_bad != 0;
      settled = i >= 1 && unsettled == 0;
    }
    if (postponed) forget();
    else if (!settled) {
      forget();
      char msg[200];
      snprintf(msg, sizeof(msg), "resnet3d_bwd: the fp16 gradient chain did not calibrate in %d passes (%u scale groups still overflow): "
               "non-finite activations or weights?", kMaxCalibrationPasses, unsettled);
      return neraf_fail(ctx, NERAF_ESTATE, msg);
    }
  }
  ArgHash k;
  k.add(0x62776432u); k.add(d->grid_size); k.add(packed_t); k.ptrs((const void* const*)conv_w, A.nconv);
  k.ptrs((const void* const*)bn, 4 * A.nconv); k.add(workspace); k.add(bwd_workspace); k.add(dfeat);
  k.ptrs((const void* const*)w_grads, A.nconv); k.ptrs((const void* const*)bn_grads, 2 * A.nconv);
  k.add(n_cells); k.add(n_ch); k.add(dgrid_cells); k.add(track);
  return neraf_run_graphed(ctx, st, k.h, body);
}

extern "C" int neraf_resnet3d_bwd_chain_state(neraf_ctx* ctx, const neraf_resnet3d_desc* d, const void* bwd_workspace, int32_t* e_out,
                                              float* amax_out, int n, int32_t* info2, neraf_stream_t stream) {
  Arch A; BwdLayout B;
  if (make_arch(d, &A) || !bwd_workspace || !e_out || !amax_out || n < 1 || n > kChainMax)
    return neraf_fail(ctx, NERAF_EINVAL, "resnet3d_bwd_chain_state: bad arguments");
  make_bwd_layout(A, &B);
  const char* bws = (const char*)bwd_workspace;
  NERAF_HIP_CHECK(ctx, hipStreamSynchronize((hipStream_t)stream));
  ChainState cs;
  NERAF_HIP_CHECK(ctx, hipMemcpy(&cs, bws + B.chain, sizeof(cs), hipMemcpyDeviceToHost));
  std::vector<unsigned> am((size_t)n * kAmaxRep * kAmaxStride);
  NERAF_HIP_CHECK(ctx, hipMemcpy(am.data(), bws + B.amax, am.size() * 4, hipMemcpyDeviceToHost));
  for (int t = 0; t < n; ++t) {
    unsigned mx = 0;
    for (int r = 0; r < kAmaxRep; ++r) mx = std::max(mx, am[((size_t)t * kAmaxRep + r) * kAmaxStride]);
    float f; memcpy(&f, &mx, 4);
    e_out[t] = cs.magic == kChainMagic ? cs.e[t] : 0;
    amax_out[t] = f;
  }
  if (info2) { info2[0] = (int32_t)cs.unsettled; info2[1] = (int32_t)cs.passes; }
  return NERAF_OK;
}

extern "C" int neraf_debug_conv_bn_relu_stage(neraf_ctx* ctx, int cin, int cin_real, int cout, int k, int stride, int pad, int din,
                                              const void* x_f16, const float* w, const float* gamma, const float* beta, const float* g,
                                              void* y_f16, float* dx, float* dw, float* dgamma, float* dbeta, neraf_stream_t stream) {
  hipStream_t st = (hipStream_t)stream;
  Arch A{};
  A.S = din; A.nconv = 1; A.nblock = 0; A.pooled = din; A.final_edge = din; A.n_features = 1024;
  const int dout = (din + 2 * pad - k) / stride + 1;
  A.conv[0] = ConvSpec{cin, cout, k, stride, pad, din, dout, cin_real};
  Layout L{}; BwdLayout B{};
  make_layout(A, &L);
  make_bwd_layout(A, &B);
  const size_t act = std::max(rows_pad(dout) * (size_t)cout, rows_pad(din) * (size_t)cin) * 2 + 256;
  char *ws = nullptr, *bws = nullptr, *packed = nullptr, *packed_t = nullptr, *extra = nullptr;
  NERAF_HIP_CHECK(ctx, hipMalloc(&ws, L.total));
  NERAF_HIP_CHECK(ctx, hipMalloc(&bws, B.total));
  NERAF_HIP_CHECK(ctx, hipMalloc(&packed, L.packed_total));
  NERAF_HIP_CHECK(ctx, hipMalloc(&packed_t, B.packed_total + 256));
  NERAF_HIP_CHECK(ctx, hipMalloc(&extra, 5 * act));
  NERAF_HIP_CHECK(ctx, hipMemsetAsync(ws, 0, L.total, st));
  NERAF_HIP_CHECK(ctx, hipMemsetAsync(bws, 0, B.total, st));
  NERAF_HIP_CHECK(ctx, hipMemsetAsync(extra, 0, 5 * act, st));
  const float* wl[1] = {w};
  {
    PackTable t{};
    t.n = 1; t.src[0] = w; t.begin[0] = 0; t.dst_off[0] = L.w[0]; t.cout[0] = cout; t.cin_real[0] = cin_real; t.cin[0] = cin;
    t.taps[0] = k * k * k; t.kpad[0] = conv_kpad(A.conv[0]); t.begin[1] = (unsigned long long)conv_npad(A.conv[0]) * conv_kpad(A.conv[0]);
    hipLaunchKernelGGL(pack_all_conv_weights_kernel, dim3((unsigned)((t.begin[1] + 255) / 256)), dim3(256), 0, st, t, packed);
  }
  half_t* xin = (half_t*)extra;
  NERAF_HIP_CHECK(ctx, hipMemcpyAsync(xin, x_f16, cube(din) * cin * 2, hipMemcpyDeviceToDevice, st));
  if (int e = run_conv(ctx, st, A, L, 0, packed, ws, xin)) return e;
  const float* bnp[4] = {gamma, beta, gamma, gamma};
  half_t* yact = (half_t*)(extra + act);
  {
    BnApplyArgs a{};
    a.a = bn_src_fwd(A, L, ws, bnp, 0, 1);
// ... 31 lines not shown
```

Measured before the change: 258.8 million field-samples/s.

## Fold small setup kernels into neighbouring kernels to cut launch count

Several tiny single-purpose kernels are removed by merging their work into adjacent kernels. Scale-from-amax computation moves into the field backward and NaCF cvt kernels, and amax clearing moves into finalize. The NaCF outer-product and dfeat reductions share one launch, bias pad-copies join the grouped cvt kernel, and zero-fills plus the stem weight relayout fold into the window conversion and backward prologue kernels. This is meant to reduce launch and serialization overhead, at the cost of redundant per-block scale computation and more complex kernels whose correctness depends on ordering (amax must be cleared after every consumer has read it).

After: 259.7 million field-samples/s, median of 6. No clear change (+0.3%).

```diff
diff --git a/neraf_amd/csrc/field_bwd.hip b/neraf_amd/csrc/field_bwd.hip
--- a/neraf_amd/csrc/field_bwd.hip
+++ b/neraf_amd/csrc/field_bwd.hip
@@ -390,7 +390,7 @@
   const float* origins; const float* dirs; const float* e_bins; const int* cam_idx;
   int R, S; int mode; float aabb[6]; float avg_density; int avg_row;
   const float* d_rgb; const float* d_density;
-  const float* scale;
+  float* scale;
   float* emb_grad;
   half_t* dump; long npad;
   unsigned* d_enc;
@@ -409,6 +409,17 @@
   for (int r = 0; r < 4; ++r) base[(long)(row0 + r) * npad + n] = (half_t)(v[r] * m);
 }
 
+__device__ __forceinline__ float field_scale_from_amax(unsigned amax_bits) {
+  const float amax = __uint_as_float(amax_bits);
+  float S = 1.f;
+  if (amax > 0.f && amax < 3.0e38f) {
+    int e = 6 - (int)floorf(log2f(amax));
+    e = e > 100 ? 100 : (e < -100 ? -100 : e);
+    S = exp2f((float)e);
+  }
+  return S;
+}
+
 template <bool RAYGRAD, bool SAVED>
 __global__ __launch_bounds__(256) void field_backward_kernel(FieldBwdArgs a) {
   __shared__ float l_scale[MAX_LEVELS];
@@ -423,11 +434,15 @@
   __shared__ float t_sum[4][16];
   __shared__ float e_acc[32];
   __shared__ int e_blk_s;
+  __shared__ float gscale_s[2];
   if (threadIdx.x < 32) e_acc[threadIdx.x] = 0.f;
   if (threadIdx.x == 0) {
     long n0 = (long)blockIdx.x * 64; const long Nn = (long)a.R * a.S;
     if (n0 >= Nn) n0 = Nn - 1;
     e_blk_s = (a.avg_row < 0 && a.cam_idx) ? a.cam_idx[n0 / a.S] : -1;
+    const float S = field_scale_from_amax(reinterpret_cast<const unsigned*>(a.scale)[2]);
+    gscale_s[0] = S; gscale_s[1] = 1.f / S;
+    if (blockIdx.x == 0) { a.scale[0] = S; a.scale[1] = 1.f / S; }
   }
   __syncthreads();
   const int e_blk = e_blk_s;
@@ -441,7 +456,7 @@
   for (int i = threadIdx.x; i < NFRAG_B * 64; i += 256) wb_s[i] = a.wfrag_b[i];
   __syncthreads();
   const half8* wb = wb_s + lane;
-  const float gscale = a.scale[0], inv_gscale = a.scale[1];
+  const float gscale = gscale_s[0], inv_gscale = gscale_s[1];
   float tl[4] = {0.f, 0.f, 0.f, 0.f};
   const f32x4 zero = {0.f, 0.f, 0.f, 0.f};
   const long N = (long)a.R * a.S;
@@ -717,8 +732,9 @@
 
 __global__ __launch_bounds__(256) void field_finalize_kernel(const float* __restrict__ t_part, int nblocks, float* __restrict__ lvl,
                                                             const float* __restrict__ e_part, const int* __restrict__ e_part_row,
-                                                            float* __restrict__ emb_grad) {
+                                                            float* __restrict__ emb_grad, unsigned* __restrict__ amax_clear) {
   __shared__ float red[4];
+  if (amax_clear && blockIdx.x == 0 && threadIdx.x == 0) *amax_clear = 0u;
   if (blockIdx.x < 16) {
     const int l = blockIdx.x;
     float v = 0.f;
@@ -1103,20 +1119,6 @@
   if (threadIdx.x == 0) atomicMax(amax_bits, __float_as_uint(fmaxf(fmaxf(sh[0], sh[1]), fmaxf(sh[2], sh[3]))));
 }
 
-__global__ void field_make_scale_kernel(float* __restrict__ scale) {
-  if (threadIdx.x == 0 && blockIdx.x == 0) {
-    const float amax = __uint_as_float(reinterpret_cast<unsigned*>(scale)[2]);
-    reinterpret_cast<unsigned*>(scale)[2] = 0u;
-    float S = 1.f;
-    if (amax > 0.f && amax < 3.0e38f) {
-      int e = 6 - (int)floorf(log2f(amax));
-      e = e > 100 ? 100 : (e < -100 ? -100 : e);
-      S = exp2f((float)e);
-    }
-    scale[0] = S; scale[1] = 1.f / S;
-  }
-}
-
 }
 
 extern "C" int neraf_render_loss(neraf_ctx* ctx, const float* density, const float* rgb_s, const float* e_bins,
@@ -1216,7 +1218,7 @@
     hipLaunchKernelGGL(proposal_backward_kernel, dim3((unsigned)blocks), dim3(256), 0, st, a);
     if (a.g6_out) hipLaunchKernelGGL(ray_fold_kernel, dim3((R + 3) / 4), dim3(256), 0, st, a.g6_out, R, S, d_rays);
     if (a.d32) {
-      hipLaunchKernelGGL(field_finalize_kernel, dim3(16), dim3(256), 0, st, a.t_part, (int)blocks, lvl, nullptr, nullptr, nullptr);
+      hipLaunchKernelGGL(field_finalize_kernel, dim3(16), dim3(256), 0, st, a.t_part, (int)blocks, lvl, nullptr, nullptr, nullptr, nullptr);
       FieldScatterArgs sa{};
       sa.g = a.g; sa.origins = origins; sa.dirs = dirs; sa.e_bins = e_bins; sa.R = R; sa.S = S; sa.mode = 0;
       sa.npad = npad; sa.lvl = lvl; sa.acc = reinterpret_cast<unsigned long long*>(acc_scratch ? acc_scratch : (void*)table_grad);
@@ -1361,7 +1363,6 @@
     const bool zero_emb = acc_scratch && !accumulate && emb_grad && avg_row < 0 && emb_rows > 0;
     hipLaunchKernelGGL(field_amax_kernel, dim3((unsigned)blocks), dim3(256), 0, st, d_rgb, d_density, density, N, avg_density,
                        reinterpret_cast<unsigned*>(scale) + 2, zero_emb ? emb_grad : nullptr, zero_emb ? (long)emb_rows * 32 : 0l);
-    hipLaunchKernelGGL(field_make_scale_kernel, dim3(1), dim3(64), 0, st, scale);
   }
   {
     const long groups = npad / 16;
@@ -1383,7 +1384,7 @@
     if (a.emb_det)
       hipLaunchKernelGGL(field_emb_fold_det_kernel, dim3((unsigned)emb_rows), dim3(256), 0, st, a.e_part, a.e_part_row, npad / 16, emb_grad, 1);
     hipLaunchKernelGGL(field_finalize_kernel, dim3(16 + (fold_emb ? (unsigned)((blocks + 63) / 64) : 0u)), dim3(256), 0, st, a.t_part,
-                       (int)blocks, lvl, a.e_part, a.e_part_row, fold_emb ? emb_grad : nullptr);
+                       (int)blocks, lvl, a.e_part, a.e_part_row, fold_emb ? emb_grad : nullptr, reinterpret_cast<unsigned*>(scale) + 2);
     FieldScatterArgs sa{};
     sa.g = a.g; sa.origins = origins; sa.dirs = dirs; sa.e_bins = e_bins; sa.R = R; sa.S = S; sa.mode = mode;
     for (int i = 0; i < 6; ++i) sa.aabb[i] = a.aabb[i];
diff --git a/neraf_amd/csrc/nacf.hip b/neraf_amd/csrc/nacf.hip
--- a/neraf_amd/csrc/nacf.hip
+++ b/neraf_amd/csrc/nacf.hip
@@ -101,14 +101,29 @@
 }
 
 
+__device__ __forceinline__ float nacf_scale_from_amax(unsigned amax_bits) {
+  const float amax = __uint_as_float(amax_bits);
+  float S = 1.f;
+  if (amax > 0.f && amax < 3.0e38f) {
+    int e = 8 - (int)floorf(log2f(amax));
+    e = e > 100 ? 100 : (e < -100 ? -100 : e);
+    S = exp2f((float)e);
+  }
+  return S;
+}
+
 __global__ __launch_bounds__(256) void cvt_pad_transpose_kernel(
-    const float* __restrict__ src, const float* __restrict__ aux, const float* __restrict__ scale, int ld, int R, int Cc,
+    const float* __restrict__ src, const float* __restrict__ aux, float* scale, int ld, int R, int Cc,
     int mode, half_t* __restrict__ dst, int ld_dst, int Rpad, int Cpad,
     half_t* __restrict__ dstT, int ld_dstT, int RpadT, int CpadT, float* __restrict__ colsum, int colsum_slot_stride) {
   __shared__ float tile[32][33];
   const int tx = threadIdx.x & 31, ty = threadIdx.x >> 5;
   const int c0 = blockIdx.x * 32, r0 = blockIdx.y * 32;
-  const float sc = scale ? scale[0] : 1.f;
+  float sc = 1.f;
+  if (mode == 1 && scale) {
+    sc = nacf_scale_from_amax(reinterpret_cast<const unsigned*>(scale)[2]);
+    if (threadIdx.x == 0 && blockIdx.x == 0 && blockIdx.y == 0) { scale[0] = sc; scale[1] = 1.f / sc; }
+  }
 #pragma unroll
   for (int i = 0; i < 4; ++i) {
     const int r = r0 + ty + i * 8, c = c0 + tx;
@@ -154,10 +169,21 @@
   int tiles_x, tile_begin;
 };
 constexpr int kMaxCvtJobs = 10;
-struct CvtTable { int n; int total; CvtJob j[kMaxCvtJobs]; };
+struct PadCopyJob { const float* src; float* dst; int n, npad, blk_begin; };
+constexpr int kMaxPadCopyJobs = 13;
+struct CvtTable { int n; int total; CvtJob j[kMaxCvtJobs]; int nv; int vtotal; PadCopyJob v[kMaxPadCopyJobs]; };
 
 __global__ __launch_bounds__(256) void cvt_pad_transpose_grouped_kernel(CvtTable t) {
   __shared__ float tile[32][33];
+  if ((int)blockIdx.x >= t.total) {
+    const int vb = blockIdx.x - t.total;
+    int vi = 0;
+    while (vi + 1 < t.nv && vb >= t.v[vi + 1].blk_begin) ++vi;
+    const PadCopyJob& V = t.v[vi];
+    const int i = (vb - V.blk_begin) * 256 + threadIdx.x;
+    if (i < V.npad) V.dst[i] = (i < V.n) ? V.src[i] : 0.f;
+    return;
+  }
   int ji = 0;
   while (ji + 1 < t.n && (int)blockIdx.x >= t.j[ji + 1].tile_begin) ++ji;
   const CvtJob& J = t.j[ji];
@@ -231,12 +257,20 @@
   if (lane == 0) out[n] = (n < N) ? s + b0[n] : 0.f;
 }
 
-__global__ __launch_bounds__(256) void dfeat_kernel(const float* __restrict__ W0, int ldw, const float* __restrict__ db0,
-                                                   int N, int n_feat, float* __restrict__ dfeat, float* __restrict__ part) {
+__global__ __launch_bounds__(256) void outer_dfeat_kernel(const float* __restrict__ W0, const float* __restrict__ db0,
+                                                         const float* __restrict__ feat, int N, int n_feat, int nsplit,
+                                                         float* __restrict__ dW0, int ldw, float* __restrict__ dfeat,
+                                                         float* __restrict__ part) {
   const int k = blockIdx.x * 256 + threadIdx.x;
-  const int per = (N + gridDim.y - 1) / gridDim.y;
-  const int n0 = blockIdx.y * per, n1 = min(N, n0 + per);
   if (k >= n_feat) return;
+  if ((int)blockIdx.y < N) {
+    const int n = blockIdx.y;
+    dW0[(size_t)n * ldw + k] = db0[n] * feat[k];
+    return;
+  }
+  const int sy = blockIdx.y - N;
+  const int per = (N + nsplit - 1) / nsplit;
+  const int n0 = sy * per, n1 = min(N, n0 + per);
   float s = 0.f, s1 = 0.f, s2 = 0.f, s3 = 0.f;
   int n = n0;
   for (; n + 8 <= n1; n += 8) {
@@ -247,7 +281,7 @@
     s2 += db0[n + 2] * w[2] + db0[n + 6] * w[6]; s3 += db0[n + 3] * w[3] + db0[n + 7] * w[7];
   }
   for (; n < n1; ++n) s += db0[n] * W0[(size_t)n * ldw + k];
-  if (part) part[(size_t)blockIdx.y * n_feat + k] = (s + s1) + (s2 + s3);
+  if (part) part[(size_t)sy * n_feat + k] = (s + s1) + (s2 + s3);
   else atomicAdd(dfeat + k, (s + s1) + (s2 + s3));
 }
 
@@ -262,14 +296,6 @@
   }
   for (; sl < nsplit; ++sl) a += part[(size_t)sl * n_feat + k];
   dfeat[k] = (a + b) + (c + e);
-}
-
-__global__ __launch_bounds__(256) void outer_kernel(const float* __restrict__ db0, const float* __restrict__ feat, int N,
-                                                   int n_feat, float* __restrict__ dW0, int ldw, float* __restrict__ zero_nfeat) {
-  const int k = blockIdx.x * 256 + threadIdx.x;
-  const int n = blockIdx.y;
-  if (k < n_feat && n < N) dW0[(size_t)n * ldw + k] = db0[n] * feat[k];
-  if (zero_nfeat && n == 0 && k < n_feat) zero_nfeat[k] = 0.f;
 }
 
 struct EncodeArgs {
@@ -366,20 +392,6 @@
   if (threadIdx.x == 0) atomicMax(amax_bits, __float_as_uint(fmaxf(fmaxf(sh[0], sh[1]), fmaxf(sh[2], sh[3]))));
 }
 
-__global__ void make_scale_kernel(float* __restrict__ scale) {
-  if (threadIdx.x == 0 && blockIdx.x == 0) {
-    const float amax = __uint_as_float(reinterpret_cast<unsigned*>(scale)[2]);
-    float S = 1.f;
-    if (amax > 0.f && amax < 3.0e38f) {
-      int e = 8 - (int)floorf(log2f(amax));
-      e = e > 100 ? 100 : (e < -100 ? -100 : e);
-      S = exp2f((float)e);
-    }
-    scale[0] = S;
-    scale[1] = 1.f / S;
-  }
-}
-
 __global__ void scale_copy_kernel(float* __restrict__ dst, const float* __restrict__ src, int n, const float* __restrict__ mul) {
   const int i = blockIdx.x * blockDim.x + threadIdx.x;
   if (i < n) dst[i] = src[i] * mul[0];
@@ -446,7 +458,7 @@
   }
 }
 
-int cvt_pad_transpose(neraf_ctx* ctx, hipStream_t st, const float* src, const float* aux, const float* scale, int ld, int R,
+int cvt_pad_transpose(neraf_ctx* ctx, hipStream_t st, const float* src, const float* aux, float* scale, int ld, int R,
                       int Cc, int mode,
                       half_t* dst, int ld_dst, int Rpad, int Cpad, half_t* dstT, int ld_dstT, int RpadT, int CpadT,
                       float* colsum, int colsum_slot_stride = 0) {
@@ -484,7 +496,7 @@
 extern "C" int neraf_nacf_pack_weights(neraf_ctx* ctx, const neraf_nacf_desc* d, const float* const* w, void* packed,
                                        neraf_stream_t stream) {
   if (int e = check_desc(ctx, d)) return e;
-  if (d->C + 6 > kMaxCvtJobs || d->C + 5 > 16) return neraf_fail(ctx, NERAF_EINVAL, "nacf_pack_weights: too many heads");
+  if (d->C + 6 > kMaxCvtJobs || d->C + 5 > kMaxPadCopyJobs) return neraf_fail(ctx, NERAF_EINVAL, "nacf_pack_weights: too many heads");
   hipStream_t st = (hipStream_t)stream;
   const Dims D = make_dims(d);
   const PackLayout L = make_pack_layout(d, D);
@@ -515,14 +527,17 @@
     add(w[2 * (5 + c)], d->W, d->F, d->W, (half_t*)(P + L.w[5]) + (size_t)c * d->F * D.kp[5], D.kp[5], rows, D.kp[5],
         (half_t*)(P + L.wt[5]) + (size_t)c * d->F, D.np[5], rows, kt5);
   }
-  hipLaunchKernelGGL(cvt_pad_transpose_grouped_kernel, dim3(t.total), dim3(256), 0, st, t);
-  SegCopyTable sc{};
+  auto addv = [&](float* dst, const float* src, int n, int npad) {
+    PadCopyJob& V = t.v[t.nv++];
+    V.src = src; V.dst = dst; V.n = n; V.npad = npad; V.blk_begin = t.vtotal;
+    t.vtotal += (npad + 255) / 256;
+  };
   for (int c = 0; c < d->C; ++c) {
     const bool last = c == d->C - 1;
-    seg_copy_add(sc, (float*)(P + L.bias[5]) + (size_t)c * d->F, w[2 * (5 + c) + 1], d->F, last ? D.np[5] - c * d->F : d->F);
-  }
-  for (int l = 0; l < 5; ++l) seg_copy_add(sc, (float*)(P + L.bias[l]), Bptr(w, l), D.n[l], D.np[l]);
-  hipLaunchKernelGGL(seg_copy_kernel, dim3(sc.begin[sc.n]), dim3(256), 0, st, sc);
+    addv((float*)(P + L.bias[5]) + (size_t)c * d->F, w[2 * (5 + c) + 1], d->F, last ? D.np[5] - c * d->F : d->F);
+  }
+  for (int l = 0; l < 5; ++l) addv((float*)(P + L.bias[l]), Bptr(w, l), D.n[l], D.np[l]);
+  hipLaunchKernelGGL(cvt_pad_transpose_grouped_kernel, dim3(t.total + t.vtotal), dim3(256), 0, st, t);
   NERAF_HIP_CHECK(ctx, hipGetLastError());
   return NERAF_OK;
 }
@@ -637,7 +652,7 @@
 
 static int nacf_bwd_body(neraf_ctx* ctx, const neraf_nacf_desc* d, const Dims& D, const PackLayout& PL, const WsLayout& WL,
                          const char* P, char* ws, int B, const float* out, const float* dout, float* const* grads,
-                         int* slot0, hipStream_t st) {
+                         int* slot0, float* zero_nfeat, hipStream_t st) {
   const int M = WL.Mpad;
   neraf_zero_async(st, ws + WL.colsum[0], WL.scale + 256 - WL.colsum[0]);
   float* scale = (float*)(ws + WL.scale);
@@ -647,7 +662,6 @@
     int blocks = (int)((n + 1023) / 1024);
     if (blocks > 256) blocks = 256;
     hipLaunchKernelGGL(amax_dz5_kernel, dim3(blocks), dim3(256), 0, st, dout, out, n, reinterpret_cast<unsigned*>(scale) + 2);
-    hipLaunchKernelGGL(make_scale_kernel, dim3(1), dim3(64), 0, st, scale);
   }
   SegCopyTable outs{};
   outs.mul = inv_scale;
@@ -697,6 +711,7 @@
     }
   }
   copy_out(grads[1], (const float*)(ws + WL.colsum[0]), D.n[0], D.np[0]);
+  if (zero_nfeat && d->n_feat > 0) seg_copy_add(outs, zero_nfeat, nullptr, 0, d->n_feat);
   hipLaunchKernelGGL(seg_copy_kernel, dim3(outs.begin[outs.n]), dim3(256), 0, st, outs);
   NERAF_HIP_CHECK(ctx, hipGetLastError());
   *slot0 = cur;
@@ -715,7 +730,7 @@
   const char* P = (const char*)packed;
   char* ws = (char*)workspace;
   int s0 = 0;
-  if (int e = nacf_bwd_body(ctx, d, D, PL, WL, P, ws, B, out, dout, grads, &s0, st)) return e;
+  if (int e = nacf_bwd_body(ctx, d, D, PL, WL, P, ws, B, out, dout, grads, &s0, dfeat, st)) return e;
   const int M = WL.Mpad;
   GemmParams g{};
   g.A = (const half_t*)(ws + WL.dzT[s0]); g.lda = M;
@@ -726,14 +741,11 @@
   if (int e = launch_gemm_f16(ctx, g, st)) return e;
   const float* db0 = grads[1];
   if (d->n_feat > 0) {
-    hipLaunchKernelGGL(outer_kernel, dim3((d->n_feat + 255) / 256, D.n[0]), dim3(256), 0, st, db0, feat, D.n[0], d->n_feat,
-                       grads[0], D.kdense, dfeat);
-    if (dfeat) {
-      float* part = WL.col_slots > 1 ? (float*)(ws + WL.dfeat_part) : nullptr;
-      hipLaunchKernelGGL(dfeat_kernel, dim3((d->n_feat + 255) / 256, 64), dim3(256), 0, st, Wptr(w, 0), D.kdense, db0,
-                         D.n[0], d->n_feat, dfeat, part);
-      if (part) hipLaunchKernelGGL(dfeat_fold_kernel, dim3((d->n_feat + 255) / 256), dim3(256), 0, st, part, 64, d->n_feat, dfeat);
-    }
+    float* part = (dfeat && WL.col_slots > 1) ? (float*)(ws + WL.dfeat_part) : nullptr;
+    const int nsplit = dfeat ? 64 : 0;
+    hipLaunchKernelGGL(outer_dfeat_kernel, dim3((d->n_feat + 255) / 256, D.n[0] + nsplit), dim3(256), 0, st, Wptr(w, 0), db0, feat,
+                       D.n[0], d->n_feat, nsplit, grads[0], D.kdense, dfeat, part);
+    if (part) hipLaunchKernelGGL(dfeat_fold_kernel, dim3((d->n_feat + 255) / 256), dim3(256), 0, st, part, 64, d->n_feat, dfeat);
   }
   NERAF_HIP_CHECK(ctx, hipGetLastError());
   return NERAF_OK;
@@ -752,7 +764,7 @@
   const char* P = (const char*)packed;
   char* ws = (char*)workspace;
   int s0 = 0;
-  if (int e = nacf_bwd_body(ctx, d, D, PL, WL, P, ws, B, out, dout, grads, &s0, st)) return e;
+  if (int e = nacf_bwd_body(ctx, d, D, PL, WL, P, ws, B, out, dout, grads, &s0, nullptr, st)) return e;
   const int M = WL.Mpad;
   GemmParams g{};
   g.A = (const half_t*)(ws + WL.dzT[s0]); g.lda = M;
diff --git a/neraf_amd/csrc/resnet3d.hip b/neraf_amd/csrc/resnet3d.hip
--- a/neraf_amd/csrc/resnet3d.hip
+++ b/neraf_amd/csrc/resnet3d.hip
@@ -13,17 +13,29 @@
   reinterpret_cast<half8*>(out)[v] = h;
 }
 
-__global__ __launch_bounds__(256) void grid_window_to_ndhwc8_kernel(const float* __restrict__ grid, size_t nvox, const unsigned long long* start,
-                                                                   int n, half_t* __restrict__ out) {
-  const int t = blockIdx.x * 256 + threadIdx.x;
-  if (t >= n) return;
-  const size_t v = (size_t)*start + t;
-  if (v >= nvox) return;
-  half8 h;
-#pragma unroll
-  for (int c = 0; c < 7; ++c) h[c] = (half_t)grid[c * nvox + v];
-  h[7] = (half_t)0.f;
-  reinterpret_cast<half8*>(out)[v] = h;
+__global__ __launch_bounds__(256) void zero3_grid_window_kernel(const float* __restrict__ grid, size_t nvox, const unsigned long long* start,
+                                                               int n, half_t* __restrict__ out, unsigned win_blocks,
+                                                               unsigned* __restrict__ p0, size_t n0, unsigned* __restrict__ p1, size_t n1,
+                                                               unsigned* __restrict__ p2, size_t n2) {
+  if (blockIdx.x < win_blocks) {
+    const int t = blockIdx.x * 256 + threadIdx.x;
+    if (t >= n) return;
+    const size_t v = (size_t)*start + t;
+    if (v >= nvox) return;
+    half8 h;
+#pragma unroll
+    for (int c = 0; c < 7; ++c) h[c] = (half_t)grid[c * nvox + v];
+    h[7] = (half_t)0.f;
+    reinterpret_cast<half8*>(out)[v] = h;
+    return;
+  }
+  const size_t total = n0 + n1 + n2;
+  const size_t zb = gridDim.x - win_blocks;
+  for (size_t i = (size_t)(blockIdx.x - win_blocks) * 256 + threadIdx.x; i < total; i += zb * 256) {
+    if (i < n0) p0[i] = 0u;
+    else if (i < n0 + n1) p1[i - n0] = 0u;
+    else p2[i - n0 - n1] = 0u;
+  }
 }
 
 __global__ void set_u64_fwd_kernel(unsigned long long* p, unsigned long long v) { if (threadIdx.x == 0 && blockIdx.x == 0) p[0] = v; }
@@ -222,15 +234,21 @@
 
 static int resnet3d_fwd_body(neraf_ctx* ctx, const Arch& A, const Layout& L, const char* packed, const float* const* bn, const float* grid,
                              char* ws, float* feat, int use_batch_stats, int win_cells, hipStream_t st) {
-  neraf_zero3_async(st, ws + L.zero_page, 256, ws + L.stats_begin, L.stats_bytes, feat, (size_t)A.n_features * sizeof(float));
-  neraf_node(ctx, "neraf_zero3_kernel | statistics accumulators", 0.0, 0.0, 256.0 + (double)L.stats_bytes + 4096.0);
   const size_t nvox = cube(A.S);
   const bool training = use_batch_stats != 0;
   if (win_cells > 0) {
-    hipLaunchKernelGGL(grid_window_to_ndhwc8_kernel, dim3((unsigned)((win_cells + 255) / 256)), dim3(256), 0, st, grid, nvox,
-                       reinterpret_cast<const unsigned long long*>(ws + L.win), win_cells, (half_t*)(ws + L.x0));
-    neraf_node(ctx, "grid_window_to_ndhwc8_kernel | refresh window -> fp16 channels-last", 0.0, win_cells * 28.0, win_cells * 16.0);
+    const size_t w0 = 256 / 4, w1 = L.stats_bytes / 4, w2 = (size_t)A.n_features;
+    size_t zblocks = (w0 + w1 + w2 + 255) / 256;
+    if (zblocks > 4096) zblocks = 4096;
+    const unsigned win_blocks = (unsigned)((win_cells + 255) / 256);
+    hipLaunchKernelGGL(zero3_grid_window_kernel, dim3(win_blocks + (unsigned)zblocks), dim3(256), 0, st, grid, nvox,
+                       reinterpret_cast<const unsigned long long*>(ws + L.win), win_cells, (half_t*)(ws + L.x0), win_blocks,
+                       (unsigned*)(ws + L.zero_page), w0, (unsigned*)(ws + L.stats_begin), w1, (unsigned*)feat, w2);
+    neraf_node(ctx, "zero3_grid_window_kernel | statistics accumulators + refresh window -> fp16 channels-last", 0.0, win_cells * 28.0,
+               win_cells * 16.0 + 256.0 + (double)L.stats_bytes + 4096.0);
   } else {
+    neraf_zero3_async(st, ws + L.zero_page, 256, ws + L.stats_begin, L.stats_bytes, feat, (size_t)A.n_features * sizeof(float));
+    neraf_node(ctx, "neraf_zero3_kernel | statistics accumulators", 0.0, 0.0, 256.0 + (double)L.stats_bytes + 4096.0);
     hipLaunchKernelGGL(grid_to_ndhwc8_kernel, dim3((unsigned)((nvox + 255) / 256)), dim3(256), 0, st, grid, nvox, (half_t*)(ws + L.x0));
     neraf_node(ctx, "grid_to_ndhwc8_kernel | grid -> fp16 channels-last", 0.0, (double)nvox * 28.0, (double)nvox * 16.0);
   }
diff --git a/neraf_amd/csrc/resnet3d_bwd.hip b/neraf_amd/csrc/resnet3d_bwd.hip
--- a/neraf_amd/csrc/resnet3d_bwd.hip
+++ b/neraf_amd/csrc/resnet3d_bwd.hip
@@ -243,7 +243,9 @@
 
 __global__ __launch_bounds__(256) void bwd_prologue_kernel(const float* __restrict__ dfeat, float* __restrict__ scale, int target_log2, int M,
                                                           int Mpad, int C, half_t* __restrict__ g, ChainState* __restrict__ cs,
-                                                          unsigned* __restrict__ amax, int n_groups, ChainParents par) {
+                                                          unsigned* __restrict__ amax, int n_groups, ChainParents par,
+                                                          unsigned* __restrict__ zero_p, size_t zero_words,
+                                                          const float* __restrict__ stem_w, float* __restrict__ stem_wt) {
   __shared__ float red[4];
   __shared__ unsigned s_am[kChainMax];
   __shared__ ChainParents s_par;
@@ -331,6 +333,18 @@
   for (size_t idx = (size_t)blockIdx.x * 256 + threadIdx.x; idx < total; idx += (size_t)gridDim.x * 256) {
     const int row = (int)(idx / C), c = (int)(idx % C);
     g[idx] = (half_t)(row < M ? dfeat[c] * k : 0.f);
+  }
+  {
+    const size_t n4 = zero_words / 4;
+    typedef unsigned u4 __attribute__((ext_vector_type(4)));
+    for (size_t i = (size_t)blockIdx.x * 256 + threadIdx.x; i < n4; i += (size_t)gridDim.x * 256) reinterpret_cast<u4*>(zero_p)[i] = u4{0u, 0u, 0u, 0u};
+    if (blockIdx.x == 0 && threadIdx.x < (zero_words & 3)) zero_p[n4 * 4 + threadIdx.x] = 0u;
+  }
+  if (stem_wt) {
+    for (int idx = blockIdx.x * 256 + threadIdx.x; idx < 125 * 8 * 64; idx += gridDim.x * 256) {
+      const int co = idx & 63, c = (idx >> 6) & 7, tap = idx >> 9;
+      stem_wt[idx] = c < 7 ? stem_w[((size_t)co * 7 + c) * 125 + tap] : 0.f;
+    }
   }
 }
 
@@ -372,13 +386,6 @@
 
 __global__ void set_f32x2_kernel(float* p, float a, float b) { if (threadIdx.x == 0 && blockIdx.x == 0) { p[0] = a; p[1] = b; } }
 __global__ void set_u64_kernel(unsigned long long* p, unsigned long long v) { if (threadIdx.x == 0 && blockIdx.x == 0) p[0] = v; }
-
-__global__ __launch_bounds__(256) void stem_w_relayout_kernel(const float* __restrict__ W, float* __restrict__ Wt) {
-  const int idx = blockIdx.x * 256 + threadIdx.x;
-  if (idx >= 125 * 8 * 64) return;
-  const int co = idx & 63, c = (idx >> 6) & 7, tap = idx >> 9;
-  Wt[idx] = c < 7 ? W[((size_t)co * 7 + c) * 125 + tap] : 0.f;
-}
 
 __global__ __launch_bounds__(256) void stem_dgrid_kernel(const half_t* __restrict__ dy, const float* __restrict__ Wt, int S, int dout,
                                                         const unsigned long long* __restrict__ start_dev, int n, int nch,
@@ -659,8 +666,6 @@
                              float* const* w_grads, float* const* bn_grads, int n_cells, int n_ch, float* dgrid_cells, hipStream_t st,
                              bool track) {
   float* scale = (float*)(bws + B.scale);
-  neraf_zero_async(st, bws + B.sums_begin, B.sums_bytes);
-  neraf_node(ctx, "neraf_zero_kernel | BatchNorm-backward accumulators", 0.0, 0.0, (double)B.sums_bytes);
   const int Mlast = (int)cube(A.final_edge);
   Ctx c{ctx, st, &A, &L, &B, (const char*)packed_t, ws, bws, bn, w_grads, bn_grads};
   c.track = track;
@@ -682,8 +687,12 @@
     for (int b = A.nblock - 1; b >= 0; --b) { pp.p[k] = (unsigned char)kg; pp.p[k + 1] = (unsigned char)k; pp.p[k + 2] = (unsigned char)(k + 1); kg = k + 2; k += 3; }
     pp.p[k] = (unsigned char)kg;
     hipLaunchKernelGGL(bwd_prologue_kernel, dim3(blocks), dim3(256), 0, st, dfeat, scale, kChainTarget + (int)ceilf(log2f((float)Mlast)), Mlast, Mpad,
-                       A.n_features, g, reinterpret_cast<ChainState*>(bws + B.chain), reinterpret_cast<unsigned*>(bws + B.amax), total_k, pp);
-    neraf_node(ctx, "bwd_prologue_kernel | S0, scale groups, average-pool backward", 0.0, 4096.0 + (double)total_k * kAmaxRep * 4.0, (double)n * 2.0);
+                       A.n_features, g, reinterpret_cast<ChainState*>(bws + B.chain), reinterpret_cast<unsigned*>(bws + B.amax), total_k, pp,
+                       reinterpret_cast<unsigned*>(bws + B.sums_begin), B.sums_bytes / 4, n_cells > 0 ? conv_w[0] : nullptr,
+                       n_cells > 0 ? (float*)(bws + B.wtmp) : nullptr);
+    neraf_node(ctx, "bwd_prologue_kernel | S0, scale groups, average-pool backward, accumulators = 0, stem W -> Wt[tap][c][co]", 0.0,
+               4096.0 + (double)total_k * kAmaxRep * 4.0 + (n_cells > 0 ? 125.0 * 7 * 64 * 4 : 0.0),
+               (double)n * 2.0 + (double)B.sums_bytes + (n_cells > 0 ? 125.0 * 8 * 64 * 4 : 0.0));
   }
   half_t* gm = (half_t*)(bws + B.gm); half_t* da = (half_t*)(bws + B.da);
   WgradItem items[64]; int n_items = 0;
@@ -736,11 +745,9 @@
     items[n_items++] = wgrad_item(c, 0, dy0, (const half_t*)(ws + L.x0), k_s);
     if (n_cells > 0) {
       float* Wt = (float*)(bws + B.wtmp);
-      hipLaunchKernelGGL(stem_w_relayout_kernel, dim3((125 * 8 * 64 + 255) / 256), dim3(256), 0, st, conv_w[0], Wt);
       hipLaunchKernelGGL(stem_dgrid_kernel, dim3((n_cells + 3) / 4), dim3(256), 0, st, dy0, Wt, A.S, c0.dout,
                          reinterpret_cast<const unsigned long long*>(bws + B.scale + 64), n_cells, n_ch, c.inv(k_s), dgrid_cells);
       NERAF_HIP_CHECK(ctx, hipGetLastError());
-      neraf_node(ctx, "stem_w_relayout_kernel | W[co][c][tap] -> Wt[tap][c][co]", 0.0, 125.0 * 7 * 64 * 4, 125.0 * 8 * 64 * 4);
       neraf_node(ctx, "stem_dgrid_kernel | grid gradient of the refresh window", 2.0 * n_cells * (125.0 / 8.0) * 64 * n_ch, (double)n_cells * (125.0 / 8.0) * 128.0,
                  (double)n_cells * n_ch * 4.0);
     }
```
